# icrdr/3D-UNet-Renal-Anatomy-Extraction

Measured on AMD Instinct MI355X. Metric: train voxels/sec (128^3 patch, bs=2 per GPU), whole job, higher is better.
Workload: dtype bf16; 1 GPU; ResUnet3D(num_pool=4, num_features=32, in=1, out=3) train step (fwd+HybirdLoss+bwd+Adam), 2x1x128^3 per GPU, dropout on; global_batch=2, parallelism=dp1, optimizer=optim.Adam (fused multi-tensor)

## Files before the change

3d-unet-renal-anatomy-extraction_amd/_native.py:

```python
import ctypes
import os
import threading

import torch

_HERE = os.path.dirname(os.path.abspath(__file__))
LIB_PATH = os.environ.get("RU3D_LIB", os.path.join(_HERE, "libru3d.so"))

F32, BF16, F16 = 0, 1, 2
PREDICT_MAX_BATCH = 16
LABEL_I64, LABEL_U8 = 0, 1
ROLE_CONV_FWD, ROLE_CONV_DGRAD, ROLE_CONVT_FWD, ROLE_CONVT_DGRAD, ROLE_BIAS = 0, 1, 2, 3, 4
LOSS_HYBIRD, LOSS_DICELOSS, LOSS_FOCAL, LOSS_DICE = 0, 1, 2, 3
MAX_CLASSES = 8


class Tensor(ctypes.Structure):
    _fields_ = [("ptr", ctypes.c_void_p), ("n", ctypes.c_int32), ("d", ctypes.c_int32), ("h", ctypes.c_int32),
                ("w", ctypes.c_int32), ("c", ctypes.c_int32), ("ld", ctypes.c_int32), ("cseg", ctypes.c_int32),
                ("seg_stride", ctypes.c_int64)]


class PackItem(ctypes.Structure):
    _fields_ = [("src", ctypes.c_void_p), ("dst", ctypes.c_void_p), ("cout", ctypes.c_int32), ("cin", ctypes.c_int32),
                ("k", ctypes.c_int32), ("stride", ctypes.c_int32), ("role", ctypes.c_int32),
                ("cout_seg", ctypes.c_int32), ("cin_seg", ctypes.c_int32)]


class PatchParams(ctypes.Structure):
    _fields_ = [("lo", ctypes.c_int32 * 3), ("before", ctypes.c_int32 * 3), ("patch", ctypes.c_int32 * 3),
                ("flip", ctypes.c_int32 * 3), ("image_cval", ctypes.c_float), ("label_cval", ctypes.c_int32),
                ("do_contrast", ctypes.c_int32), ("do_brightness", ctypes.c_int32), ("do_gamma", ctypes.c_int32),
                ("contrast", ctypes.c_float), ("brightness", ctypes.c_float), ("gamma", ctypes.c_float),
                ("gamma_eps", ctypes.c_float)]


class SpatialParams(ctypes.Structure):
    _fields_ = [("centre", ctypes.c_double * 3), ("matrix", ctypes.c_double * 9), ("lattice", ctypes.c_int32 * 3),
                ("spacing", ctypes.c_int32 * 3)]


class DegradeParams(ctypes.Structure):
    _fields_ = [("do_noise", ctypes.c_int32), ("do_blur", ctypes.c_int32), ("do_low_res", ctypes.c_int32),
                ("noise_key", ctypes.c_uint32 * 2), ("reserved", ctypes.c_int32), ("noise_variance", ctypes.c_double),
                ("blur_sigma", ctypes.c_double), ("low_res_zoom", ctypes.c_double)]


class MorphRow(ctypes.Structure):
    _fields_ = [("dx", ctypes.c_int8), ("dy", ctypes.c_int8), ("zmask", ctypes.c_uint16)]


class RenderTile(ctypes.Structure):
    _fields_ = [("volume", ctypes.c_void_p), ("table", ctypes.c_void_p), ("overlay", ctypes.c_void_p * 2),
                ("overlay_table", ctypes.c_void_p * 2), ("vmin", ctypes.c_double), ("vmax", ctypes.c_double),
                ("origin", ctypes.c_double * 2), ("step", ctypes.c_double * 2), ("x0", ctypes.c_int32),
                ("y0", ctypes.c_int32), ("w", ctypes.c_int32), ("h", ctypes.c_int32), ("X", ctypes.c_int32),
                ("Y", ctypes.c_int32), ("Z", ctypes.c_int32), ("C", ctypes.c_int32), ("channel", ctypes.c_int32),
                ("kind", ctypes.c_int32), ("axis", ctypes.c_int32), ("index", ctypes.c_int32),
                ("overlay_mode", ctypes.c_int32 * 2)]


class RenderView(ctypes.Structure):
    _fields_ = [("o", ctypes.c_double * 3), ("du", ctypes.c_double * 3), ("dv", ctypes.c_double * 3),
                ("dw", ctypes.c_double * 3), ("spacing", ctypes.c_double * 3), ("light", ctypes.c_double * 3),
                ("ambient", ctypes.c_double), ("diffuse", ctypes.c_double), ("background", ctypes.c_double * 3),
                ("num_steps", ctypes.c_int32), ("reserved", ctypes.c_int32)]


class DsLevel(ctypes.Structure):
    _fields_ = [("logits", ctypes.c_void_p), ("stride_n", ctypes.c_int64), ("stride_c", ctypes.c_int64),
                ("stride_v", ctypes.c_int64), ("d", ctypes.c_int32), ("h", ctypes.c_int32), ("w", ctypes.c_int32),
                ("shift", ctypes.c_int32)]


DS_MAX_LEVELS = 8
MASK_NE, MASK_EQ, MASK_GT, MASK_GE = 0, 1, 2, 3
TILE_F32, TILE_U8 = 0, 1
OVERLAY_FILL, OVERLAY_OUTLINE = 0, 1
RENDER_MAX_TILES = 256
MORPH_ERODE, MORPH_DILATE = 0, 1
MORPH_MAX_EXTENT, MORPH_MAX_ROWS = 15, 225
CONFUSION_MAX_CLASSES = 32
ORDER_STATS_MAX_RANKS = 8
EDT_MAX_AXIS = 4096
SPATIAL_MAX_YZ = 2560
BOUNDARY_MAX_AXIS = 2048
DEGRADE_MAX_RADIUS = 16
PACK_MAX = 40
_P = ctypes.POINTER(Tensor)
_vp, _i, _i64, _f, _sz, _u64 = (ctypes.c_void_p, ctypes.c_int, ctypes.c_int64, ctypes.c_float, ctypes.c_size_t,
                                ctypes.c_uint64)
_dbl = ctypes.c_double

_LOSS_VIEW = [_vp, _i64, _i64, _i64, _vp, _i, _i]

SIGNATURES = {
    "ru3d_version": (_i, []),
    "ru3d_last_error": (ctypes.c_char_p, []),
    "ru3d_launch_log_begin": (None, []),
    "ru3d_launch_log_end": (ctypes.c_char_p, []),
    "ru3d_packed_weight_bytes": (_sz, [_i, _i, _i, _i, _i, _i]),
    "ru3d_pack_weight": (_i, [_vp, _vp, _i, _i, _i, _i, _i, _i, _vp]),
    "ru3d_pack_weights": (_i, [ctypes.POINTER(PackItem), _i, _i, _vp]),
    "ru3d_unpad_weight_grad": (_i, [_vp, _vp, _i, _i, _i, _i, _i, _vp]),
    "ru3d_conv3d_workspace_bytes": (_sz, [_P, _P, _i, _i, _i]),
    "ru3d_conv3d_fwd": (_i, [_P, _vp, _vp, _P, _P, _i, _i, _i, _i, _vp, _sz, _vp]),
    "ru3d_conv3d_fwd_in_workspace_bytes": (_sz, [_P, _P, _i, _i, _i]),
    "ru3d_conv3d_fwd_in": (_i, [_P, _vp, _vp, _P, _i, _i, _i, _vp, _vp, _vp, _vp, _sz, _f, _vp]),
    "ru3d_conv3d_fwd_in_lrelu_workspace_bytes": (_sz, [_P, _P, _i, _i, _i]),
    "ru3d_conv3d_fwd_in_lrelu": (_i, [_P, _vp, _vp, _P, _i, _i, _i, _vp, _vp, _vp, _P, _P, _f, _vp, _sz, _f, _vp]),
    "ru3d_planar_concat_supported": (_i, [_i, _i, _i, _i, _i, _i, _i]),
    "ru3d_conv3d_dgrad": (_i, [_P, _vp, _P, _P, _i, _i, _i, _vp, _sz, _vp]),
    "ru3d_conv3d_s2_pair_fwd_in_supported": (_i, [_P, _P, _P, _i]),
    "ru3d_conv3d_s2_pair_fwd_in_workspace_bytes": (_sz, [_P, _P, _i]),
    "ru3d_conv3d_s2_pair_fwd_in": (_i, [_P, _vp, _vp, _P, _vp, _vp, _P, _vp, _vp, _vp, _vp, _sz, _f, _i, _vp]),
    "ru3d_conv3d_s1_dgrad_pair_supported": (_i, [_P, _P, _P, _i]),
    "ru3d_conv3d_s1_dgrad_pair": (_i, [_P, _vp, _P, _vp, _P, _i, _vp]),
    "ru3d_conv3d_s2_dgrad_pair_supported": (_i, [_P, _P, _P, _P, _i]),
    "ru3d_conv3d_s2_dgrad_pair": (_i, [_P, _vp, _P, _vp, _P, _P, _i, _vp]),
    "ru3d_conv3d_wgrad_workspace_bytes": (_sz, [_P, _P, _i, _i, _i]),
    "ru3d_conv3d_wgrad": (_i, [_P, _P, _vp, _vp, _sz, _i, _i, _i, _vp]),
    "ru3d_conv3d_wgrad_bias_workspace_bytes": (_sz, [_P, _P, _i, _i, _i]),
    "ru3d_conv3d_wgrad_bias": (_i, [_P, _P, _vp, _vp, _vp, _sz, _i, _i, _i, _vp]),
    "ru3d_conv3d_wgrad_pair_supported": (_i, [_P, _P, _P, _i, _i]),
    "ru3d_conv3d_wgrad_pair_workspace_bytes": (_sz, [_P, _P, _P, _i, _i]),
    "ru3d_conv3d_wgrad_pair": (_i, [_P, _P, _P, _vp, _vp, _vp, _sz, _i, _i, _vp]),
    "ru3d_head_bwd_supported": (_i, [_P, _P, _P, _i]),
    "ru3d_head_bwd_workspace_bytes": (_sz, [_P, _i]),
    "ru3d_head_bwd": (_i, [_P, _P, _vp, _i, _P, _vp, _vp, _vp, _sz, _i, _vp]),
    "ru3d_convtranspose3d_k3s2p1_fwd": (_i, [_P, _vp, _vp, _P, _i, _vp]),
    "ru3d_convtranspose3d_k3s2p1_fwd_in_workspace_bytes": (_sz, [_P, _P, _i]),
    "ru3d_convtranspose3d_k3s2p1_fwd_in": (_i, [_P, _vp, _vp, _P, _vp, _vp, _vp, _sz, _f, _i, _vp]),
    "ru3d_convtranspose3d_k3s2p1_dgrad": (_i, [_P, _vp, _P, _i, _vp]),
    "ru3d_convtranspose3d_k3s2p1_wgrad_workspace_bytes": (_sz, [_P, _P, _i]),
    "ru3d_convtranspose3d_k3s2p1_wgrad": (_i, [_P, _P, _vp, _vp, _sz, _i, _vp]),
    "ru3d_reduce_workspace_bytes": (_sz, [_P]),
    "ru3d_instnorm_stats": (_i, [_P, _vp, _vp, _vp, _vp, _sz, _f, _i, _vp]),
    "ru3d_in_lrelu_fwd": (_i, [_P, _vp, _vp, _P, _P, _f, _i, _vp]),
    "ru3d_skip1x1_in_lrelu_fwd_supported": (_i, [_P, _P, _P, _i]),
    "ru3d_skip1x1_in_lrelu_fwd": (_i, [_P, _vp, _vp, _P, _vp, _vp, _P, _f, _i, _vp]),
    "ru3d_skip1x1_in_lrelu_head_fwd_supported": (_i, [_P, _P, _P, _P, _i]),
    "ru3d_skip1x1_in_lrelu_head_fwd": (_i, [_P, _vp, _vp, _P, _vp, _vp, _P, _vp, _vp, _P, _f, _i, _vp]),
    "ru3d_head_in_bwd_supported": (_i, [_P, _P, _P, _P, _P, _i]),
    "ru3d_head_in_bwd_workspace_bytes": (_sz, [_P, _i]),
    "ru3d_head_in_bwd": (_i, [_P, _P, _vp, _i, _P, _vp, _vp, _P, _P, _vp, _vp, _vp, _vp, _sz, _f, _i, _vp]),
    "ru3d_in_lrelu_bwd": (_i, [_P, _P, _P, _vp, _vp, _P, _P, _vp, _sz, _f, _i, _vp, _vp, _i, _vp]),
    "ru3d_in_lrelu_bwd_apply": (_i, [_P, _P, _vp, _vp, _vp, _P, _f, _i, _i, _vp]),
    "ru3d_conv3d_dgrad_in_bwd_workspace_bytes": (_sz, [_P, _P, _i, _i, _i]),
    "ru3d_conv3d_dgrad_in_bwd": (_i, [_P, _vp, _P, _vp, _vp, _P, _P, _i, _i, _f, _i, _vp, _sz, _vp]),
    "ru3d_channel_sum": (_i, [_P, _vp, _vp, _sz, _i, _vp]),
    "ru3d_batchnorm_stats_pool": (_i, [_P, _vp, _vp, _vp, _sz, _i, _vp]),
    "ru3d_batchnorm_stats_finalize": (_i, [_vp, _i, _i, _i, _dbl, _vp, _vp, _vp, _f, _f, _vp, _vp, _vp, _vp, _vp, _vp, _vp]),
    "ru3d_affine_lrelu_fwd": (_i, [_P, _vp, _vp, _P, _P, _f, _i, _vp]),
    "ru3d_batchnorm_bwd_pool": (_i, [_P, _P, _P, _vp, _vp, _P, _vp, _vp, _sz, _f, _i, _vp]),
    "ru3d_batchnorm_bwd_apply": (_i, [_P, _P, _vp, _vp, _vp, _vp, _dbl, _P, _vp, _sz, _i, _i, _vp]),
    "ru3d_dropout3d_scale": (_i, [_vp, _i, _f, _u64, _u64, _vp]),
    "ru3d_dropout3d_scale_dev": (_i, [_vp, _i, _f, _u64, _u64, _vp, _vp]),
    "ru3d_pointwise": (_i, [_i, _P, _P, _P, _P, _P, _f, _i, _vp]),
    "ru3d_copy_channels": (_i, [_P, _P, _i, _vp]),
    "ru3d_add": (_i, [_P, _P, _P, _i, _vp]),
    "ru3d_cast_f32": (_i, [_P, _P, _i, _vp]),
    "ru3d_ncdhw_to_ndhwc": (_i, [_vp, _P, _i, _vp]),
    "ru3d_ndhwc_to_ncdhw": (_i, [_P, _vp, _i, _vp]),
    "ru3d_loss_state_bytes": (_sz, [_i]),
    "ru3d_loss_state_bad_labels_offset": (_sz, []),
    "ru3d_loss_workspace_bytes": (_sz, [_i, _i64, _i]),
    "ru3d_loss_fwd": (_i, _LOSS_VIEW + [_i64, _i, _i, _f, _vp, _f, _f, _f, _vp, _vp, _vp, _sz, _vp]),
    "ru3d_loss_bwd": (_i, _LOSS_VIEW + [_i64, _i, _f, _vp, _vp, _vp, _i, _vp]),
    "ru3d_tversky": (_i, [_vp, _vp, _i64, _f, _f, _f, _vp, _vp, _sz, _vp]),
    "ru3d_predict_accumulate": (_i, [_P, _i, _i, _vp, _vp, _i, _i, _i, _i, _i, _i, _vp]),
    "ru3d_predict_merge": (_i, [_vp, _vp, _i, _i, _i, _i, _i, _i, _i, _i, _i, _i, _i, _vp, _vp]),
    "ru3d_predict_gather": (_i, [_vp, _i, _i, _i, _i, _vp, _i, _P, _vp]),
    "ru3d_predict_accumulate_weighted": (_i, [_P, _i, _i, _i, _vp, _vp, _vp, _vp, _vp, _i, _i, _i, _i, _i, _i, _vp]),
    "ru3d_group_loss_state_bytes": (_sz, []),
    "ru3d_group_loss_workspace_bytes": (_sz, [_i, _i64, _i]),
    "ru3d_group_loss_fwd": (_i, _LOSS_VIEW + [_i64, _i, _vp, _i, _i, _i, _i, _f, _vp, _f, _f, _f, _vp, _vp, _vp, _sz,
                                              _vp]),
    "ru3d_group_loss_bwd": (_i, _LOSS_VIEW + [_i64, _i, _vp, _i, _i, _i, _f, _vp, _vp, _vp, _i, _vp]),
    "ru3d_topk_select_workspace_bytes": (_sz, [_i64]),
    "ru3d_topk_select_trip_elements": (_i64, []),
    "ru3d_topk_select": (_i, [_vp, _i64, _i64, _vp, _vp, _sz, _vp]),
    "ru3d_topk_loss_state_bytes": (_sz, []),
    "ru3d_topk_loss_workspace_bytes": (_sz, [_i, _i64, _i]),
    "ru3d_topk_loss_fwd": (_i, _LOSS_VIEW + [_i64, _i, _i64, _i, _vp, _f, _f, _f, _f, _vp, _vp, _vp, _vp, _sz, _vp]),
    "ru3d_topk_loss_fwd_launches": (_i, []),
    "ru3d_topk_loss_fwd_timed": (_i, _LOSS_VIEW + [_i64, _i, _i64, _i, _vp, _f, _f, _f, _f, _vp, _vp, _vp, _vp, _sz,
                                                   _vp, _vp]),
    "ru3d_topk_loss_bwd": (_i, _LOSS_VIEW + [_i64, _i, _i, _vp, _vp, _vp, _vp, _i, _vp]),
    "ru3d_predict_accumulate_groups": (_i, [_P, _i, _i, _i, _vp, _vp, _vp, _vp, _vp, _i, _i, _i, _i, _i, _i, _vp]),
    "ru3d_predict_merge_groups": (_i, [_vp, _vp, _i, _i, _i, _i, _vp, _vp, _i, _i, _i, _i, _i, _i, _vp, _vp]),
    "ru3d_components_workspace_bytes": (_sz, [_i, _i, _i]),
    "ru3d_label_components": (_i, [_vp, _i, _i, _i, _vp, _vp, _vp, _sz, _vp]),
    "ru3d_component_stats": (_i, [_vp, _i, _i, _i, _i, _vp, _vp, _vp]),
    "ru3d_filter_components_workspace_bytes": (_sz, [_i]),
    "ru3d_filter_components": (_i, [_vp, _i, _i, _i, _i, _vp, _i, _vp, _vp, _vp, _vp, _sz, _vp]),
    "ru3d_region_accumulate": (_i, [_vp, _i, _i, _i, _i, _i, _i, _i, _vp, _vp, _i, _i, _i, _vp]),
    "ru3d_cascade_merge": (_i, [_vp, _vp, _i, _i, _i, _i, _vp, _vp]),
    "ru3d_mask_bytes": (_sz, [_i, _i, _i]),
    "ru3d_mask_pack": (_i, [_vp, _i, _i, _i, _i, _i, _vp, _vp]),
    "ru3d_mask_unpack": (_i, [_vp, _i, _i, _i, _i, _i, _vp, _vp]),
    "ru3d_binary_morph": (_i, [_vp, _vp, _i, _i, _i, _i, ctypes.POINTER(MorphRow), _i, _i, _vp]),
    "ru3d_confusion_counts": (_i, [_vp, _vp, _i64, _i, _vp, _vp]),
    "ru3d_threshold_bbox": (_i, [_vp, _i, _i, _i, _i, _f, _vp, _vp, _vp]),
    "ru3d_masked_sample_workspace_bytes": (_sz, [_i, _i, _i]),
    "ru3d_masked_sample": (_i, [_vp, _i, _i, _i, _i, _i, _vp, _i, _i, _vp, _i64, _vp, _vp, _sz, _vp]),
    "ru3d_order_stats_workspace_bytes": (_sz, []),
    "ru3d_order_stats": (_i, [_vp, _i64, ctypes.POINTER(ctypes.c_int64), _i, _vp, _vp, _sz, _vp]),
    "ru3d_moments_workspace_bytes": (_sz, []),
    "ru3d_moments": (_i, [_vp, _i64, _vp, _vp, _sz, _vp]),
    "ru3d_edt_workspace_bytes": (_sz, [_i, _i, _i]),
    "ru3d_edt_squared": (_i, [_vp, _i, _i, _i, ctypes.POINTER(_dbl), _vp, _vp, _sz, _vp]),
    "ru3d_mask_surface": (_i, [_vp, _vp, _i, _i, _i, _vp]),
    "ru3d_edt_gather_workspace_bytes": (_sz, [_i, _i, _i]),
    "ru3d_edt_gather": (_i, [_vp, _vp, _i, _i, _i, _vp, _i64, _vp, _vp, _sz, _vp]),
    "ru3d_edt_reduce_workspace_bytes": (_sz, [_i64]),
    "ru3d_edt_reduce": (_i, [_vp, _vp, _i64, _dbl, _vp, _vp, _sz, _vp]),
    "ru3d_skeleton_workspace_bytes": (_sz, [_i, _i, _i]),
    "ru3d_skeleton_thin": (_i, [_vp, _i, _i, _i, _i, _vp, _sz, _vp]),
    "ru3d_skeleton_classify": (_i, [_vp, _i, _i, _i, _vp, _vp, _vp, _vp]),
    "ru3d_skeleton_length": (_i, [_vp, _i, _i, _i, ctypes.POINTER(_dbl), _vp, _vp, _sz, _vp]),
    "ru3d_skeleton_overlap": (_i, [_vp, _vp, _i, _i, _i, _vp, _vp]),
    "ru3d_skeleton_radius_stats": (_i, [_vp, _i64, _vp, _vp]),
    "ru3d_cldice_workspace_bytes": (_sz, [_i, _i, _i, _i, _i]),
    "ru3d_cldice_state_bytes": (_sz, []),
    "ru3d_soft_skeleton_fwd": (_i, [_vp, _i, _i, _i, _i, _i, _vp, _vp, _vp, _vp, _vp, _sz, _vp]),
    "ru3d_soft_skeleton_bwd": (_i, [_vp, _i, _i, _i, _i, _i, _vp, _vp, _vp, _vp, _vp, _vp, _sz, _vp]),
    "ru3d_cldice_fwd": (_i, _LOSS_VIEW + [_i, _i, _i, _i, _vp, _i, _i, _vp, _f, _vp, _vp, _vp, _vp, _vp, _vp, _vp, _vp,
                                          _sz, _vp]),
    "ru3d_cldice_bwd": (_i, _LOSS_VIEW + [_i, _i, _i, _i, _vp, _i, _i, _vp, _vp, _vp, _vp, _vp, _vp, _vp, _f, _i, _vp,
                                          _vp, _sz, _vp]),
    "ru3d_boundary_workspace_bytes": (_sz, [_i, _i, _i, _i]),
    "ru3d_boundary_state_bytes": (_sz, []),
    "ru3d_signed_distance": (_i, [_vp, _i, _i, _i, _i, _i, _i, _vp, _i, _vp, _vp, _vp, _sz, _vp]),
    "ru3d_boundary_fwd": (_i, _LOSS_VIEW + [_i, _i, _i, _i, _vp, _i, _vp, _vp, _vp, _vp, _vp, _sz, _vp]),
    "ru3d_boundary_bwd": (_i, [_vp, _i64, _i64, _i64, _i, _i, _i, _i, _i, _vp, _i, _vp, _vp, _vp, _f, _i, _vp, _vp]),
    "ru3d_ds_state_bytes": (_sz, []),
    "ru3d_ds_state_bad_labels_offset": (_sz, []),
    "ru3d_ds_block_bytes": (_sz, []),
    "ru3d_ds_loss_workspace_bytes": (_sz, [ctypes.POINTER(DsLevel), _i, _i]),
    "ru3d_ds_loss_fwd": (_i, [ctypes.POINTER(DsLevel), _i, _vp, _i, _i, _i, _i, _i, _i, _i, _f, _vp, _f, _f, _f, _vp, _vp,
                              _vp, _vp, _sz, _vp]),
    "ru3d_ds_loss_bwd": (_i, [ctypes.POINTER(DsLevel), ctypes.POINTER(_vp), _i, _vp, _i, _i, _i, _i, _i, _i, _f, _vp, _vp,
                              _vp]),
    "ru3d_mesh_workspace_bytes": (_sz, [_i, _i, _i]),
    "ru3d_mesh_count": (_i, [_vp, _i, _i, _i, _vp, _vp, _sz, _vp]),
    "ru3d_mesh_emit": (_i, [_vp, _i, _i, _i, _vp, _vp, _i64, _vp, _i64, _vp, _vp, _sz, _vp]),
    "ru3d_mesh_smooth": (_i, [_vp, _vp, _vp, _i64, _dbl, _vp]),
    "ru3d_mesh_measure_workspace_bytes": (_sz, [_i64]),
    "ru3d_mesh_measure": (_i, [_vp, _i64, _vp, _i64, _vp, _vp, _sz, _vp]),
    "ru3d_render_tiles": (_i, [_vp, _i, _vp, _i, _i, _vp]),
    "ru3d_render_surface_workspace_bytes": (_sz, [_i, _i, _i]),
    "ru3d_render_surface_prepare": (_i, [_vp, _i, _i, _i, _vp, _vp, _sz, _vp]),
    "ru3d_render_surface": (_i, [_vp, _i, _i, _i, _vp, ctypes.POINTER(RenderView), _vp, _vp, _i, _i, _vp, _sz, _vp]),
    "ru3d_adam_multi": (_i, [_vp, _vp, _i, _i, _f, _f, _f, _f, _f, _f, _f, _vp]),
    "ru3d_adam_multi_dev": (_i, [_vp, _vp, _i, _i, _vp, _vp]),
    "ru3d_adam_multi_amp": (_i, [_vp, _vp, _i, _i, _vp, _vp, _vp]),
    "ru3d_amp_update": (_i, [_vp, _f, _f, _i, _f, _f, _vp]),
    "ru3d_grad_sumsq": (_i, [_vp, _vp, _i, _i, _vp, _vp]),
    "ru3d_grad_norm_finish": (_i, [_vp, _i, _f, _vp, _f, _vp, _vp]),
    "ru3d_grad_norm": (_i, [_vp, _vp, _i, _i, _vp, _f, _f, _vp, _vp]),
    "ru3d_grad_scale_dev": (_i, [_vp, _vp, _i, _i, _vp, _vp]),
    "ru3d_sgd_multi": (_i, [_vp, _vp, _i, _i, _f, _f, _f, _i, _f, _vp, _vp]),
    "ru3d_sgd_multi_dev": (_i, [_vp, _vp, _i, _i, _vp, _vp, _vp]),
    "ru3d_adamw_multi": (_i, [_vp, _vp, _i, _i, _f, _f, _f, _f, _f, _f, _f, _f, _vp, _vp]),
    "ru3d_adamw_multi_dev": (_i, [_vp, _vp, _i, _i, _vp, _vp, _vp]),
    "ru3d_adam_multi_clip": (_i, [_vp, _vp, _i, _i, _f, _f, _f, _f, _f, _f, _f, _vp, _vp]),
    "ru3d_adam_multi_clip_dev": (_i, [_vp, _vp, _i, _i, _vp, _vp, _vp]),
    "ru3d_adam_step": (_i, [_vp, _vp, _vp, _vp, _i64, _f, _f, _f, _f, _f, _f, _f, _vp]),
    "ru3d_augment_workspace_bytes": (_sz, [_i, _i, _i]),
    "ru3d_augment_label_presence": (_i, [_vp, _i, _i, _i, _i, ctypes.POINTER(ctypes.c_int32),
                                        ctypes.POINTER(ctypes.c_int32), _i, _vp, _vp]),
    "ru3d_augment_patch": (_i, [_vp, _vp, _i, _i, _i, _i, _i, ctypes.POINTER(PatchParams), _vp, _vp, _vp, _vp, _sz,
                               _vp]),
    "ru3d_augment_patch_spatial": (_i, [_vp, _vp, _i, _i, _i, _i, _i, ctypes.POINTER(PatchParams),
                                       ctypes.POINTER(SpatialParams), _vp, _vp, _vp, _vp, _vp, _sz, _vp]),
    "ru3d_augment_degrade_workspace_bytes": (_sz, [_i, _i, _i, _i]),
    "ru3d_augment_degrade": (_i, [_vp, _i, _i, _i, _i, ctypes.POINTER(DegradeParams), _vp, _sz, _vp, _vp]),
    "ru3d_augment_intensity": (_i, [_vp, _i64, _vp, _i, ctypes.POINTER(PatchParams), _vp]),
    "ru3d_grad_scale_check": (_i, [_vp, _vp, _i, _i, _f, _vp, _vp]),
    "ru3d_comm_unique_id": (_i, [_vp]),
    "ru3d_comm_init": (_i, [ctypes.POINTER(_vp), _vp, _i, _i, _i]),
    "ru3d_comm_allreduce": (_i, [_vp, _vp, _i64, _i, _i, _vp]),
    "ru3d_comm_reduce_scatter": (_i, [_vp, _vp, _i64, _i, _i, _vp]),
    "ru3d_comm_all_gather": (_i, [_vp, _vp, _i64, _i, _vp]),
    "ru3d_comm_available": (_i, []),
    "ru3d_comm_destroy": (_i, [_vp]),
    "ru3d_probe_begin": (_i, [_i, _i, _i, _i, _i, _i]),
    "ru3d_probe_end": (_i, [ctypes.POINTER(ctypes.c_int), ctypes.POINTER(ctypes.c_double)]),
# ... 172 lines not shown
```

3d-unet-renal-anatomy-extraction_amd/_ops.py:

```python
import ctypes
import os
import threading
import weakref

import torch

import _native as N
from _native import check, desc, ptr, ref, stream

LRELU_SLOPE = 0.01
IN_EPS = 1e-5


def pack_weight(w, role, dtype, stride=1):
    N.require_device(w, "weight")
    w = w.detach()
    if w.dtype != torch.float32 or not w.is_contiguous():
        w = w.float().contiguous()
    k = w.shape[2]
    if role in (N.ROLE_CONVT_FWD, N.ROLE_CONVT_DGRAD):
        cin, cout = w.shape[0], w.shape[1]
    else:
        cout, cin = w.shape[0], w.shape[1]
    code = N.dtype_code(dtype)
# ... 164 lines not shown
    return b if (b.dtype == torch.float32 and b.is_contiguous()) else b.float().contiguous()


def _conv_out(size, k, s):
    return (size + 2 * (k // 2) - k) // s + 1


class Probe:

    def __init__(self, n, cin, cout, extent):
        self.key = (int(n),) + tuple(int(e) for e in extent) + (int(cin), int(cout))
        self.count = 0
        self.total_ms = 0.0
        self.active = False

    def start(self):
        check(N.lib.ru3d_probe_begin(*self.key), "probe_begin")
        self.active = True

    def stop(self):
        if not self.active:
            return
        n = ctypes.c_int(0)
        ms = ctypes.c_double(0.0)
        check(N.lib.ru3d_probe_end(ctypes.byref(n), ctypes.byref(ms)), "probe_end")
        self.count += n.value
        self.total_ms += ms.value
        self.active = False

    def result(self):
        self.stop()
        return self.count, (self.total_ms / self.count if self.count else 0.0)


def set_probe(p):
    cur = _PROBE[0]
    if cur is not None and cur is not p:
        cur.stop()
    _PROBE[0] = p
    if p is not None:
        p.start()


_PROBE = [None]


class launch_log:

    def __init__(self):
        self.names = []

    def __enter__(self):
        N.lib.ru3d_launch_log_begin()
        return self

    def __exit__(self, *exc):
        s = N.lib.ru3d_launch_log_end().decode("utf-8", "replace")
        self.names = s.split(";") if s else []
        return False


def _conv_ws(dsrc, ddst, k, stride, dtype, device):
    if k != 3 or stride != 1 or dtype == torch.float32:
        return None, 0
    need = N.lib.ru3d_conv3d_workspace_bytes(ref(dsrc), ref(ddst), k, stride, N.dtype_code(dtype))
    if need == 0:
        return None, 0
    buf = N.workspace(need, device)
    return ptr(buf), buf.numel()


def conv_fwd(x, pw, bias, cout, k, stride, res=None, out_dtype=None):
    n, _, d, h, w = x.shape
    out_dtype = out_dtype or x.dtype
    y = N.new_act(n, cout, _conv_out(d, k, stride), _conv_out(h, k, stride), _conv_out(w, k, stride), out_dtype,
                  x.device)
    b = _bias(bias)
    dx, dyy = desc(x), desc(y)
    dr = desc(res) if res is not None else None
    ws, wsn = _conv_ws(dx, dyy, k, stride, x.dtype, x.device)
    check(N.lib.ru3d_conv3d_fwd(ref(dx), ptr(pw), ptr(b), ref(dr), ref(dyy), k, stride, N.dtype_code(x.dtype),
                                N.dtype_code(out_dtype), ws, wsn, stream()), "conv3d_fwd")
    return y


def conv_fwd_in(x, pw, bias, cout, k, stride, drop_scale=None):
    n, _, d, h, w = x.shape
    y = N.new_act(n, cout, _conv_out(d, k, stride), _conv_out(h, k, stride), _conv_out(w, k, stride), x.dtype, x.device)
    mean = torch.empty(n * cout, dtype=torch.float32, device=x.device)
    scale = torch.empty(n * cout, dtype=torch.float32, device=x.device)
    b = _bias(bias)
    dx, dyy = desc(x), desc(y)
    code = N.dtype_code(x.dtype)
    ws = N.workspace(N.lib.ru3d_conv3d_fwd_in_workspace_bytes(ref(dx), ref(dyy), k, stride, code), x.device)
    check(N.lib.ru3d_conv3d_fwd_in(ref(dx), ptr(pw), ptr(b), ref(dyy), k, stride, code, ptr(drop_scale), ptr(mean),
                                   ptr(scale), ptr(ws), ws.numel(), IN_EPS, stream()), "conv3d_fwd_in")
    return y, mean, scale


def conv_fwd_in_act(x, pw, bias, cout, k, stride, drop_scale=None, res=None, out=None):
    n, _, d, h, w = x.shape
    od, oh, ow = _conv_out(d, k, stride), _conv_out(h, k, stride), _conv_out(w, k, stride)
    y = N.new_act(n, cout, od, oh, ow, x.dtype, x.device)
    if out is None:
        out = N.new_act(n, cout, od, oh, ow, x.dtype, x.device)
    mean = torch.empty(n * cout, dtype=torch.float32, device=x.device)
    scale = torch.empty(n * cout, dtype=torch.float32, device=x.device)
    b = _bias(bias)
    dx, dyy, do = desc(x), desc(y), desc(out)
    dr = desc(res) if res is not None else None
    code = N.dtype_code(x.dtype)
    ws = N.workspace(N.lib.ru3d_conv3d_fwd_in_lrelu_workspace_bytes(ref(dx), ref(dyy), k, stride, code), x.device)
    check(N.lib.ru3d_conv3d_fwd_in_lrelu(ref(dx), ptr(pw), ptr(b), ref(dyy), k, stride, code, ptr(drop_scale), ptr(mean),
                                         ptr(scale), ref(dr), ref(do), LRELU_SLOPE, ptr(ws), ws.numel(), IN_EPS, stream()),
          "conv3d_fwd_in_lrelu")
    return y, mean, scale, out


def conv_dgrad(dy, pw, in_shape, k, stride, res=None):
    n, cin, d, h, w = in_shape
    dx = N.new_act(n, cin, d, h, w, dy.dtype, dy.device)
    ddy, ddx = desc(dy), desc(dx)
    dr = desc(res) if res is not None else None
    ws, wsn = _conv_ws(ddy, ddx, k, stride, dy.dtype, dy.device)
    check(N.lib.ru3d_conv3d_dgrad(ref(ddy), ptr(pw), ref(dr), ref(ddx), k, stride, N.dtype_code(dy.dtype), ws, wsn,
                                  stream()), "conv3d_dgrad")
    return dx


def conv_dgrad_in_bwd(dy, pw, act, mean, scale, k=3, stride=1):
    n, c, d, h, w = act.shape
    da = N.new_act(n, c, d, h, w, dy.dtype, dy.device)
    dyn = N.new_act(n, c, d, h, w, dy.dtype, dy.device)
    ddy, dact, dda, ddyn = desc(dy), desc(act), desc(da), desc(dyn)
    code = N.dtype_code(dy.dtype)
    need = N.lib.ru3d_conv3d_dgrad_in_bwd_workspace_bytes(ref(ddy), ref(dda), k, stride, code)
    ws = N.workspace(need, dy.device)
    check(N.lib.ru3d_conv3d_dgrad_in_bwd(ref(ddy), ptr(pw), ref(dact), ptr(mean), ptr(scale), ref(dda), ref(ddyn), k,
                                         stride, LRELU_SLOPE, code, ptr(ws), ws.numel(), stream()),
          "conv3d_dgrad_in_bwd")
    return dyn


GRAD_ARENA = {}


def _grad_out(key, shape, device):
    t = GRAD_ARENA.get(key) if key is not None else None
    if t is not None and tuple(t.shape) == tuple(shape) and t.device == device:
        return t.view(t.shape)
    return torch.empty(shape, dtype=torch.float32, device=device)


def conv_wgrad(x, dy, k, stride, key=None):
    cout, cin = dy.shape[1], x.shape[1]
    dw = _grad_out(key, (cout, cin, k, k, k), x.device)
    dx, ddy = desc(x), desc(dy)
    code = N.dtype_code(x.dtype)
    nbytes = N.lib.ru3d_conv3d_wgrad_workspace_bytes(ref(dx), ref(ddy), k, stride, code)
    ws = N.workspace(nbytes, x.device)
    check(N.lib.ru3d_conv3d_wgrad(ref(dx), ref(ddy), ptr(dw), ptr(ws), ws.numel(), k, stride, code, stream()),
          "conv3d_wgrad")
    return dw


def _wgrad_pair_ok(x, dy, stride=1):
    if x.dtype == torch.float32:
        return False
    dx, ddy = desc(x), desc(dy)
    return bool(N.lib.ru3d_conv3d_wgrad_pair_supported(ref(dx), ref(ddy), ref(ddy), stride, N.dtype_code(x.dtype)))


def conv_wgrad_pair(x, dy, dy2, stride=1, key=None, key2=None):
    if x.dtype == torch.float32 or tuple(dy.shape) != tuple(dy2.shape):
        return None
    dx, ddy, ddy2 = desc(x), desc(dy), desc(dy2)
    code = N.dtype_code(x.dtype)
    if not N.lib.ru3d_conv3d_wgrad_pair_supported(ref(dx), ref(ddy), ref(ddy2), stride, code):
        return None
    cout, cin = dy.shape[1], x.shape[1]
    dw = _grad_out(key, (cout, cin, 3, 3, 3), x.device)
    dw2 = _grad_out(key2, (cout, cin, 1, 1, 1), x.device)
    ws = N.workspace(N.lib.ru3d_conv3d_wgrad_pair_workspace_bytes(ref(dx), ref(ddy), ref(ddy2), stride, code), x.device)
    check(N.lib.ru3d_conv3d_wgrad_pair(ref(dx), ref(ddy), ref(ddy2), ptr(dw), ptr(dw2), ptr(ws), ws.numel(), stride, code,
                                       stream()), "conv3d_wgrad_pair")
    return dw, dw2


def conv_wgrad_bias(x, dy, k, stride, key=None):
    cout, cin = dy.shape[1], x.shape[1]
    dw = _grad_out(key, (cout, cin, k, k, k), x.device)
    db = torch.empty(cout, dtype=torch.float32, device=x.device)
    dx, ddy = desc(x), desc(dy)
    code = N.dtype_code(x.dtype)
    ws = N.workspace(N.lib.ru3d_conv3d_wgrad_bias_workspace_bytes(ref(dx), ref(ddy), k, stride, code), x.device)
    check(N.lib.ru3d_conv3d_wgrad_bias(ref(dx), ref(ddy), ptr(dw), ptr(db), ptr(ws), ws.numel(), k, stride, code, stream()),
          "conv3d_wgrad_bias")
    return dw, db


def head_bwd(x, gy, weight, want_bias, key=None):
    if gy.dtype != torch.float32 or x.dtype == torch.float32 or not N.is_ndhwc(gy) or weight.dtype != torch.float32:
        return None
    n, c, d, h, w = x.shape
    dx = N.new_act(n, c, d, h, w, x.dtype, x.device)
    ddx, dg, dxx = desc(x), desc(gy), desc(dx)
    code = N.dtype_code(x.dtype)
    if not N.lib.ru3d_head_bwd_supported(ref(ddx), ref(dg), ref(dxx), code):
        return None
    cout, cin = weight.shape[0], weight.shape[1]
    dw = _grad_out(key, (cout, cin, 1, 1, 1), x.device)
    db = torch.empty(cout, dtype=torch.float32, device=x.device) if want_bias else None
    ws = N.workspace(N.lib.ru3d_head_bwd_workspace_bytes(ref(ddx), code), x.device)
    wd = weight.detach()
    check(N.lib.ru3d_head_bwd(ref(ddx), ref(dg), ptr(wd if wd.is_contiguous() else wd.contiguous()), cin, ref(dxx), ptr(dw),
                              ptr(db), ptr(ws), ws.numel(), code, stream()), "head_bwd")
    return dx, dw, db


def convt_fwd(x, pw, bias, cout):
    n, _, d, h, w = x.shape
    y = N.new_act(n, cout, 2 * d, 2 * h, 2 * w, x.dtype, x.device)
    b = _bias(bias)
    dx, dyy = desc(x), desc(y)
    check(N.lib.ru3d_convtranspose3d_k3s2p1_fwd(ref(dx), ptr(pw), ptr(b), ref(dyy), N.dtype_code(x.dtype), stream()),
          "convtranspose3d_fwd")
    return y


def convt_fwd_in(x, pw, bias, cout):
    n, _, d, h, w = x.shape
    y = N.new_act(n, cout, 2 * d, 2 * h, 2 * w, x.dtype, x.device)
    mean = torch.empty(n * cout, dtype=torch.float32, device=x.device)
    scale = torch.empty(n * cout, dtype=torch.float32, device=x.device)
    b = _bias(bias)
    dx, dyy = desc(x), desc(y)
    code = N.dtype_code(x.dtype)
    ws = N.workspace(N.lib.ru3d_convtranspose3d_k3s2p1_fwd_in_workspace_bytes(ref(dx), ref(dyy), code), x.device)
    check(N.lib.ru3d_convtranspose3d_k3s2p1_fwd_in(ref(dx), ptr(pw), ptr(b), ref(dyy), ptr(mean), ptr(scale), ptr(ws),
                                                   ws.numel(), IN_EPS, code, stream()), "convtranspose3d_fwd_in")
    return y, mean, scale


def conv_s2_pair_fwd_in(x, pw3, b3, pw1, b1, cout, drop_scale=None):
    code = N.dtype_code(x.dtype)
    if code == N.F32:
        return None
    n, _, d, h, w = x.shape
    od, oh, ow = _conv_out(d, 3, 2), _conv_out(h, 3, 2), _conv_out(w, 3, 2)
    y3 = N.new_act(n, cout, od, oh, ow, x.dtype, x.device)
    y1 = N.new_act(n, cout, od, oh, ow, x.dtype, x.device)
    dx, d3, d1 = desc(x), desc(y3), desc(y1)
    if not N.lib.ru3d_conv3d_s2_pair_fwd_in_supported(ref(dx), ref(d3), ref(d1), code):
        return None
    mean = torch.empty(n * cout, dtype=torch.float32, device=x.device)
    scale = torch.empty(n * cout, dtype=torch.float32, device=x.device)
    ws = N.workspace(N.lib.ru3d_conv3d_s2_pair_fwd_in_workspace_bytes(ref(dx), ref(d3), code), x.device)
    check(N.lib.ru3d_conv3d_s2_pair_fwd_in(ref(dx), ptr(pw3), ptr(_bias(b3)), ref(d3), ptr(pw1), ptr(_bias(b1)), ref(d1),
                                           ptr(drop_scale), ptr(mean), ptr(scale), ptr(ws), ws.numel(), IN_EPS, code,
                                           stream()), "conv3d_s2_pair_fwd_in")
    return y3, mean, scale, y1


def conv_s1_dgrad_pair(dy, pw3, dy2, pw1, in_shape, planar=False):
    n, cin, d, h, w = in_shape
    code = N.dtype_code(dy.dtype)
    if code == N.F32:
        return None
    dx = N.new_act(2 * n, cin // 2, d, h, w, dy.dtype, dy.device) if planar else N.new_act(n, cin, d, h, w, dy.dtype, dy.device)
    ddy, ddy2, ddx = desc(dy), desc(dy2), desc(N.Split(dx) if planar else dx)
    if not N.lib.ru3d_conv3d_s1_dgrad_pair_supported(ref(ddy), ref(ddy2), ref(ddx), code):
        return None
    check(N.lib.ru3d_conv3d_s1_dgrad_pair(ref(ddy), ptr(pw3), ref(ddy2), ptr(pw1), ref(ddx), code, stream()),
          "conv3d_s1_dgrad_pair")
    return dx


def conv_s2_dgrad_pair(dy, pw3, dy2, pw1, in_shape, res=None):
    n, cin, d, h, w = in_shape
    code = N.dtype_code(dy.dtype)
    if code == N.F32:
        return None
    dx = N.new_act(n, cin, d, h, w, dy.dtype, dy.device)
    ddy, ddy2, ddx = desc(dy), desc(dy2), desc(dx)
    dr = desc(res) if res is not None else None
    if not N.lib.ru3d_conv3d_s2_dgrad_pair_supported(ref(ddy), ref(ddy2), ref(dr), ref(ddx), code):
        return None
    check(N.lib.ru3d_conv3d_s2_dgrad_pair(ref(ddy), ptr(pw3), ref(ddy2), ptr(pw1), ref(dr), ref(ddx), code, stream()),
          "conv3d_s2_dgrad_pair")
    return dx


def convt_dgrad(dy, pw, in_shape):
    n, cin, d, h, w = in_shape
    dx = N.new_act(n, cin, d, h, w, dy.dtype, dy.device)
    ddy, ddx = desc(dy), desc(dx)
    check(N.lib.ru3d_convtranspose3d_k3s2p1_dgrad(ref(ddy), ptr(pw), ref(ddx), N.dtype_code(dy.dtype), stream()),
          "convtranspose3d_dgrad")
    return dx


def convt_wgrad(x, dy, key=None):
    cin, cout = x.shape[1], dy.shape[1]
    dw = _grad_out(key, (cin, cout, 3, 3, 3), x.device)
    dx, ddy = desc(x), desc(dy)
    code = N.dtype_code(x.dtype)
    nbytes = N.lib.ru3d_convtranspose3d_k3s2p1_wgrad_workspace_bytes(ref(dx), ref(ddy), code)
    ws = N.workspace(nbytes, x.device)
    check(N.lib.ru3d_convtranspose3d_k3s2p1_wgrad(ref(dx), ref(ddy), ptr(dw), ptr(ws), ws.numel(), code, stream()),
          "convtranspose3d_wgrad")
    return dw


def in_stats(y, drop_scale=None):
    n, c = y.shape[0], y.shape[1]
    mean = torch.empty(n * c, dtype=torch.float32, device=y.device)
    scale = torch.empty(n * c, dtype=torch.float32, device=y.device)
    dy = desc(y)
    ws = N.workspace(N.lib.ru3d_reduce_workspace_bytes(ref(dy)), y.device)
    check(N.lib.ru3d_instnorm_stats(ref(dy), ptr(drop_scale), ptr(mean), ptr(scale), ptr(ws), ws.numel(), IN_EPS,
                                    N.dtype_code(y.dtype), stream()), "instnorm_stats")
    return mean, scale


def in_lrelu_fwd(y, mean, scale, res=None, out=None):
    if out is None:
        n, c, d, h, w = y.shape
        out = N.new_act(n, c, d, h, w, y.dtype, y.device)
    dy, do = desc(y), desc(out)
    dr = desc(res) if res is not None else None
    check(N.lib.ru3d_in_lrelu_fwd(ref(dy), ptr(mean), ptr(scale), ref(dr), ref(do), LRELU_SLOPE,
                                  N.dtype_code(y.dtype), stream()), "in_lrelu_fwd")
    return out


def skip1x1_in_lrelu_fwd(x, pw, bias, y, mean, scale, out=None):
    code = N.dtype_code(y.dtype)
    if code == N.F32:
        return None
    if out is None:
        n, c, d, h, w = y.shape
        out = N.new_act(n, c, d, h, w, y.dtype, y.device)
    dx, dy, do = desc(x), desc(y), desc(out)
    if not N.lib.ru3d_skip1x1_in_lrelu_fwd_supported(ref(dx), ref(dy), ref(do), code):
        return None
    check(N.lib.ru3d_skip1x1_in_lrelu_fwd(ref(dx), ptr(pw), ptr(_bias(bias)), ref(dy), ptr(mean), ptr(scale), ref(do),
                                          LRELU_SLOPE, code, stream()), "skip1x1_in_lrelu_fwd")
    return out


def head_tail_mode():
    return os.environ.get("RU3D_HEAD_TAIL", "1")


def skip1x1_in_lrelu_head_fwd(x, pw, bias, y, mean, scale, head_pw, head_bias, head_cout):
    code = N.dtype_code(y.dtype)
    if code == N.F32 or head_cout > 4:
        return None
    n, c, d, h, w = y.shape
    out = N.new_act(n, c, d, h, w, y.dtype, y.device)
    logits = N.new_act(n, head_cout, d, h, w, torch.float32, y.device)
    dx, dy, do, dl = desc(x), desc(y), desc(out), desc(logits)
    if not N.lib.ru3d_skip1x1_in_lrelu_head_fwd_supported(ref(dx), ref(dy), ref(do), ref(dl), code):
        return None
    check(N.lib.ru3d_skip1x1_in_lrelu_head_fwd(ref(dx), ptr(pw), ptr(_bias(bias)), ref(dy), ptr(mean), ptr(scale), ref(do),
                                               ptr(head_pw), ptr(_bias(head_bias)), ref(dl), LRELU_SLOPE, code, stream()),
          "skip1x1_in_lrelu_head_fwd")
    return out, logits


def head_in_bwd(z, gy, weight, want_bias, y, mean, scale, key=None):
    if gy.dtype != torch.float32 or z.dtype == torch.float32 or not N.is_ndhwc(gy) or weight.dtype != torch.float32:
        return None
    n, c, d, h, w = z.shape
    dy = N.new_act(n, c, d, h, w, z.dtype, z.device)
    gpre = N.new_act(n, c, d, h, w, z.dtype, z.device)
    dz, dg, dyy, dp, ddy = desc(z), desc(gy), desc(y), desc(gpre), desc(dy)
    code = N.dtype_code(z.dtype)
    if not N.lib.ru3d_head_in_bwd_supported(ref(dz), ref(dg), ref(dyy), ref(dp), ref(ddy), code):
        return None
    cout, cin = weight.shape[0], weight.shape[1]
    dw = _grad_out(key, (cout, cin, 1, 1, 1), z.device)
    db = torch.empty(cout, dtype=torch.float32, device=z.device) if want_bias else None
    gsum = torch.empty(c, dtype=torch.float32, device=z.device)
    ws = N.workspace(N.lib.ru3d_head_in_bwd_workspace_bytes(ref(dz), code), z.device)
    wd = weight.detach()
    check(N.lib.ru3d_head_in_bwd(ref(dz), ref(dg), ptr(wd if wd.is_contiguous() else wd.contiguous()), cin, ref(dyy),
                                 ptr(mean), ptr(scale), ref(dp), ref(ddy), ptr(dw), ptr(db), ptr(gsum), ptr(ws), ws.numel(),
                                 LRELU_SLOPE, code, stream()), "head_in_bwd")
    return dy, gpre, gsum, dw, db


def in_lrelu_bwd(gout, out, y, mean, scale, want_gpre=False, zero_far=False, want_gpre_sum=False, dy_sum=None):
    n, c, d, h, w = y.shape
    dy = N.new_act(n, c, d, h, w, y.dtype, y.device)
    gpre = N.new_act(n, c, d, h, w, y.dtype, y.device) if want_gpre else None
    dg, do, dyy, ddy = desc(gout), desc(out), desc(y), desc(dy)
    dp = desc(gpre) if want_gpre else None
    ws = N.workspace(N.lib.ru3d_reduce_workspace_bytes(ref(dyy)), y.device)
    gsum = torch.empty(c, dtype=torch.float32, device=y.device) if (want_gpre and want_gpre_sum) else None
    check(N.lib.ru3d_in_lrelu_bwd(ref(dg), ref(do), ref(dyy), ptr(mean), ptr(scale), ref(ddy), ref(dp), ptr(ws),
                                  ws.numel(), LRELU_SLOPE, 1 if zero_far else 0, ptr(gsum), ptr(dy_sum),
                                  N.dtype_code(y.dtype), stream()), "in_lrelu_bwd")
    if want_gpre_sum:
        return dy, gpre, gsum
    return dy, gpre


_BN_SYNC = [None, 1]


def set_bn_sync(group=None, enable=True):
    import torch.distributed as dist
    if enable and dist.is_available() and dist.is_initialized() and dist.get_world_size(group) > 1:
        _BN_SYNC[0], _BN_SYNC[1] = (group if group is not None else dist.group.WORLD), dist.get_world_size(group)
    else:
        _BN_SYNC[0], _BN_SYNC[1] = None, 1


def _bn_allreduce(pooled):
    if _BN_SYNC[0] is not None:
        import torch.distributed as dist
        dist.all_reduce(pooled, group=_BN_SYNC[0])
    return pooled


def bn_train_stats(y, drop_scale, norm, c_real):
    n, c = y.shape[0], y.shape[1]
    dev = y.device
    dy = desc(y)
    pooled = torch.empty(2 * c, dtype=torch.float64, device=dev)
    ws = N.workspace(N.lib.ru3d_reduce_workspace_bytes(ref(dy)), dev)
    check(N.lib.ru3d_batchnorm_stats_pool(ref(dy), ptr(drop_scale), ptr(pooled), ptr(ws), ws.numel(),
                                          N.dtype_code(y.dtype), stream()), "batchnorm_stats_pool")
    _bn_allreduce(pooled)
    count = float(n * y.shape[2] * y.shape[3] * y.shape[4]) * _BN_SYNC[1]
    track = norm.track_running_stats and norm.running_mean is not None
    momentum = 0.0
    if track:
        norm.num_batches_tracked.add_(1)
        momentum = (1.0 / float(norm.num_batches_tracked)) if norm.momentum is None else float(norm.momentum)
    out = torch.empty(4, n * c, dtype=torch.float32, device=dev)
    gamma = norm.weight.detach() if norm.weight is not None else None
    beta = norm.bias.detach() if norm.bias is not None else None
    for t in (gamma, beta, norm.running_mean if track else None, norm.running_var if track else None):
        if t is not None and (t.dtype != torch.float32 or not t.is_contiguous() or t.device != dev):
            raise N.Ru3dError("BatchNorm3d: parameters / running statistics must be contiguous fp32 on %s" % dev)
    check(N.lib.ru3d_batchnorm_stats_finalize(ptr(pooled), n, c, c_real, count, ptr(drop_scale), ptr(gamma), ptr(beta),
                                              float(norm.eps), momentum, ptr(norm.running_mean if track else None),
                                              ptr(norm.running_var if track else None), ptr(out[0]), ptr(out[1]),
                                              ptr(out[2]), ptr(out[3]), stream()), "batchnorm_stats_finalize")
    return out[0], out[1], out[2], out[3], count


def affine_lrelu_fwd(y, scale, shift, res=None, out=None):
    if out is None:
        n, c, d, h, w = y.shape
        out = N.new_act(n, c, d, h, w, y.dtype, y.device)
    dy, do = desc(y), desc(out)
    dr = desc(res) if res is not None else None
# ... 120 lines not shown
    else:
        check(N.lib.ru3d_dropout3d_scale(ptr(out), n * c, float(p), ctypes.c_uint64(seed), ctypes.c_uint64(offset),
                                         stream()), "dropout3d_scale")
    return out


_DROP_POOL = []


def prefill_dropout(specs, device):
    _DROP_POOL.clear()
    if len(specs) < 2 or any(sp[2] != specs[0][2] for sp in specs):
        return
    flat = dropout_scale(1, sum(n * c for n, c, _ in specs), specs[0][2], device)
    off = 0
    for n, c, p in specs:
        _DROP_POOL.append((flat[off:off + n * c], n, c, p))
        off += n * c


def take_dropout(n, c, p):
    if not _DROP_POOL:
        return None
    t, n0, c0, p0 = _DROP_POOL[0]
    if (n0, c0, p0) != (n, c, p):
        _DROP_POOL.clear()
        return None
    _DROP_POOL.pop(0)
    return t


def as_input(x, dtype):
    N.require_device(x, "input")
    if x.dim() != 5:
        raise N.Ru3dError("ru3d: expected a 5-D [N,C,D,H,W] tensor, got %s" % (tuple(x.shape),))
    if x.dtype == dtype and N.is_ndhwc(x):
        return x
    if N.is_ndhwc(x) and x.dtype == torch.float32:
        return cast_f32(x, dtype)
    if x.is_contiguous() or x.dtype != torch.float32:
        return ncdhw_to_ndhwc(x, dtype)
    return ncdhw_to_ndhwc(x.contiguous(), dtype)


def as_grad(g, like_dtype):
    if g.dtype != like_dtype:
        if g.dtype == torch.float32 and N.is_ndhwc(g):
            return cast_f32(g, like_dtype)
        g = g.to(like_dtype)
    return N.to_ndhwc(g)


_SIDE_MODE = os.environ.get("RU3D_WGRAD_STREAM", "0")
_SIDE_MAXVOX = int(os.environ.get("RU3D_SIDE_MAXVOX", "65536"))
_SIDE = {}
_SIDE_BUSY = {}


def _side_stream(device):
    s = _SIDE.get(device)
    if s is None:
        s = _SIDE[device] = torch.cuda.Stream(device=device)
    return s


class _OnSide:

    def __init__(self, device, nvox=0, keep=()):
        self.device = device
        self.ctx = None
        self.on = _SIDE_MODE == "1" or (_SIDE_MODE == "auto" and 0 < nvox <= _SIDE_MAXVOX)
        self.keep = keep

    def __enter__(self):
        if self.on:
            side = _side_stream(self.device)
            side.wait_stream(torch.cuda.current_stream(self.device))
            _SIDE_BUSY.setdefault(self.device, []).extend(t for t in self.keep if t is not None)
            self.ctx = torch.cuda.stream(side)
            self.ctx.__enter__()
        return self

    def __exit__(self, *exc):
        if self.ctx is not None:
            self.ctx.__exit__(*exc)
            self.ctx = None
        return False


def _join(device, *outs):
    busy = _SIDE_BUSY.get(device)
    if busy is None:
        return
    cur = torch.cuda.current_stream(device)
    cur.wait_stream(_side_stream(device))
    for t in outs:
        if t is not None:
            t.record_stream(cur)
    del _SIDE_BUSY[device]


class SkipLink:

    def __init__(self, up_channels, dec_channels=0):
        self.up_channels = up_channels
        self.dec_channels = dec_channels
        self.buf = None
        self.grad = None
        self.planar = False

    def skip_view(self, n, c, d, h, w, dtype, device):
        self.planar = False
        self.buf = N.new_act(n, self.up_channels + c, d, h, w, dtype, device)
        return self.buf[:, self.up_channels:]

    def planar_view(self, n, c, d, h, w, dtype, device):
        if (c != self.up_channels or dtype == torch.float32 or not self.dec_channels
                or not N.lib.ru3d_planar_concat_supported(n, d, h, w, c, self.dec_channels, N.dtype_code(dtype))):
            return None
        self.planar = True
        self.buf = N.new_act(2 * n, c, d, h, w, dtype, device)
        return self.buf[n:]


def _f32_view(pack, count):
    return pack[:4 * count].view(torch.float32)


class ConvFn(torch.autograd.Function):

    @staticmethod
    def forward(ctx, x, weight, bias, stride, storage_dtype, out_dtype, pad_in=False, pad_out=False):
        xin = as_input(x, storage_dtype)
        k = weight.shape[2]
        cout, cin = weight.shape[0], weight.shape[1]
        cin_seg = seg_of(cin, xin.shape[1]) if pad_in else 0
        cout_seg = cout if pad_out else 0
        if not pad_in and xin.shape[1] != cin:
            raise N.Ru3dError("conv: input has %d channels, weight expects %d" % (xin.shape[1], cin))
        cout_p = padded_dim(cout, cout_seg)
        specs = [(weight, N.ROLE_CONV_FWD, stride, cout_seg, cin_seg)]
        if ctx.needs_input_grad[0]:
            specs.append((weight, N.ROLE_CONV_DGRAD, stride, cout_seg, cin_seg))
        if cout_seg and bias is not None:
            specs.append((bias, N.ROLE_BIAS, 1, cout_seg, 0))
        packs = pack_weights(specs, storage_dtype)
        b = _f32_view(packs[-1], cout_p) if (cout_seg and bias is not None) else bias
        y = conv_fwd(xin, packs[0], b, cout_p, k, stride, out_dtype=out_dtype)
        ctx.save_for_backward(xin, packs[1] if ctx.needs_input_grad[0] else None)
        ctx.dims = (cout, cin, cout_seg, cin_seg)
        ctx.stride, ctx.k, ctx.has_bias = stride, k, bias is not None
        ctx.storage_dtype = storage_dtype
        ctx.in_dtype = x.dtype
        ctx.wkey = weight.data_ptr() if not (cout_seg or cin_seg) else None
        ctx.weight_ref = weight if (k == 1 and cout <= 4) else None
        return y

    @staticmethod
    def backward(ctx, gy):
        xin, pwd = ctx.saved_tensors
        sd = ctx.storage_dtype
        cout, cin, cout_seg, cin_seg = ctx.dims
        if (ctx.k == 1 and ctx.stride == 1 and cout <= 4 and not cout_seg and all(ctx.needs_input_grad[:2])
                and ctx.weight_ref is not None):
            fused = head_bwd(xin, gy, ctx.weight_ref, ctx.has_bias and ctx.needs_input_grad[2],
                             key=None if cin_seg else ctx.wkey)
            if fused is not None:
                gx, gw, gb = fused
                if gx.dtype != ctx.in_dtype:
                    gx = gx.to(ctx.in_dtype)
                return gx, gw, gb, None, None, None, None, None
        gy = as_grad(gy, sd)
        gx = gw = gb = None
        with _OnSide(gy.device):
            if ctx.needs_input_grad[1] and ctx.has_bias and ctx.needs_input_grad[2] and not (cout_seg or cin_seg) \
                    and sd != torch.float32:
                gw, gb = conv_wgrad_bias(xin, gy, ctx.k, ctx.stride, key=ctx.wkey)
            elif ctx.needs_input_grad[1]:
                gw = unpad_wgrad(conv_wgrad(xin, gy, ctx.k, ctx.stride, key=ctx.wkey), cout, cin, cout_seg, cin_seg)
            if gb is None and ctx.has_bias and ctx.needs_input_grad[2]:
                gb = channel_sum(gy)[:cout]
        if ctx.needs_input_grad[0]:
            gx = conv_dgrad(gy, pwd, tuple(xin.shape), ctx.k, ctx.stride)
            if gx.dtype != ctx.in_dtype:
                gx = gx.to(ctx.in_dtype)
        _join(gy.device, gw, gb)
        return gx, gw, gb, None, None, None, None, None


class ResBlockFn(torch.autograd.Function):

    @staticmethod
    def forward(ctx, x, w1, b1, w2, b2, ws, bs, stride, drop_scale, pad=0, checkpoint=False, in_link=None,
                out_link=None, planar=False, head_w=None, head_b=None):
        sd = x.dtype
        x = N.to_ndhwc(x)
        xt = x
        if planar:
            x = N.Split(x)
        cout, cin = w1.shape[0], w1.shape[1]
        cin_seg = seg_of(cin, x.shape[1], int(pad)) if pad else 0
        cout_seg = cout if pad else 0
        if not pad and x.shape[1] != cin:
            raise N.Ru3dError("ResBlock: input has %d channels, conv1 expects %d" % (x.shape[1], cin))
        cout_p = padded_dim(cout, cout_seg)
        train = any(ctx.needs_input_grad)
        need_gx = ctx.needs_input_grad[0]
        specs = [(w1, N.ROLE_CONV_FWD, stride, cout_seg, cin_seg), (w2, N.ROLE_CONV_FWD, 1, cout_seg, cout_seg)]
        if ws is not None:
            specs.append((ws, N.ROLE_CONV_FWD, stride, cout_seg, cin_seg))
        nfwd = len(specs)
        if train:
            specs.append((w2, N.ROLE_CONV_DGRAD, 1, cout_seg, cout_seg))
            if need_gx:
                specs.append((w1, N.ROLE_CONV_DGRAD, stride, cout_seg, cin_seg))
                if ws is not None:
                    specs.append((ws, N.ROLE_CONV_DGRAD, stride, cout_seg, cin_seg))
        nw = len(specs)
        if cout_seg:
            specs += [(b, N.ROLE_BIAS, 1, cout_seg, 0) for b in (b1, b2, bs) if b is not None]
        packs = pack_weights(specs, sd)
        if cout_seg:
            it = iter(packs[nw:])
            b1, b2, bs = [(_f32_view(next(it), cout_p) if b is not None else None) for b in (b1, b2, bs)]
        pw1, pw2 = packs[0], packs[1]
        fused = conv_s2_pair_fwd_in(x, pw1, b1, packs[2], bs, cout_p, drop_scale) if (ws is not None and stride == 2) else None
        if fused is not None:
            y1, mean1, scale1, skip = fused
            a1 = in_lrelu_fwd(y1, mean1, scale1)
        else:
            y1, mean1, scale1, a1 = conv_fwd_in_act(x, pw1, b1, cout_p, 3, stride, drop_scale)
        n_, _, d_, h_, w_ = a1.shape
        zout = None
        if out_link is not None and cout_p * a1.element_size() >= 128:
            zout = out_link.skip_view(n_, cout_p, d_, h_, w_, sd, x.device)
        elif out_link is not None:
            zout = out_link.planar_view(n_, cout_p, d_, h_, w_, sd, x.device)
        z = None
        tail = (fused is None and ws is not None and stride == 1 and out_link is None and sd != torch.float32
                and (x.shape[1], cout_p) in ((64, 32), (128, 64)) and n_ * d_ * h_ * w_ >= 65536)
        logits = head_pack = None
        if head_w is not None:
            if head_w.shape[1] != cout or head_w.shape[2] != 1 or out_link is not None:
                raise N.Ru3dError("ResBlock: the head must be a 1x1x1 conv on the block's %d output channels" % cout)
            head_pack = pack_weights([(head_w, N.ROLE_CONV_FWD, 1, 0, cout_seg)], sd)[0]
        if tail:
            y2, mean2, scale2 = conv_fwd_in(a1, pw2, b2, cout_p, 3, 1)
            both = (skip1x1_in_lrelu_head_fwd(x, packs[2], bs, y2, mean2, scale2, head_pack, head_b, head_w.shape[0])
                    if (head_w is not None and head_tail_mode() != "bwd") else None)
            if both is not None:
                z, logits = both
            else:
                z = skip1x1_in_lrelu_fwd(x, packs[2], bs, y2, mean2, scale2)
            if z is None:
                z = in_lrelu_fwd(y2, mean2, scale2, res=conv_fwd(x, packs[2], bs, cout_p, 1, stride), out=zout)
        else:
            if fused is not None:
                pass
            elif ws is not None:
                skip = conv_fwd(x, packs[2], bs, cout_p, 1, stride)
            else:
                skip = x
            y2, mean2, scale2, z = conv_fwd_in_act(a1, pw2, b2, cout_p, 3, 1, res=skip, out=zout)
        if head_w is not None and logits is None:
            logits = conv_fwd(z, head_pack, head_b, head_w.shape[0], 1, 1, out_dtype=torch.float32)
        bwd = packs[nfwd:nw] + [None] * 3
        hsave = head_w if train else None
        if checkpoint and train:
            ctx.save_for_backward(xt, None, None, None, z, mean1, scale1, mean2, scale2, bwd[0], bwd[1], bwd[2],
                                  pw1, pw2, b1, b2, hsave)
        else:
            ctx.save_for_backward(xt, y1, a1, y2, z, mean1, scale1, mean2, scale2, bwd[0], bwd[1], bwd[2],
                                  None, None, None, None, hsave)
        ctx.head = head_w is not None
        ctx.head_bias = head_b is not None
        ctx.hkey = head_w.data_ptr() if (head_w is not None and not cout_seg) else None
        ctx.planar = bool(planar)
        ctx.dims = (cout, cin, cout_seg, cin_seg)
        ctx.stride = stride
        plain = not (cout_seg or cin_seg)
        ctx.wkeys = (w1.data_ptr() if plain else None, w2.data_ptr() if plain else None,
                     ws.data_ptr() if (plain and ws is not None) else None)
        ctx.has_skip_conv = ws is not None
        ctx.in_link = in_link if (in_link is not None and ws is not None) else None
        if in_link is not None:
            in_link.fused_grad = ctx.in_link is not None and need_gx
        return logits if head_w is not None else z

    @staticmethod
    def _head_backward(ctx, gy, z, head_w, y2, mean2, scale2):
        cout, cin, cout_seg, cin_seg = ctx.dims
        sd = z.dtype
        want_b = ctx.head_bias and ctx.needs_input_grad[15]
        fused = head_in_bwd(z, gy, head_w, want_b, y2, mean2, scale2, key=ctx.hkey) if head_tail_mode() != "fwd" else None
        if fused is not None:
            return fused
        hb = head_bwd(z, gy, head_w, want_b, key=ctx.hkey)
        if hb is not None:
            gz, ghw, ghb = hb
        else:
            gy = as_grad(gy, sd)
            hcout = head_w.shape[0]
            ghw = unpad_wgrad(conv_wgrad(z, gy, 1, 1, key=ctx.hkey), hcout, cout, 0, cout_seg)
            ghb = channel_sum(gy)[:hcout] if want_b else None
            pwd = pack_weights([(head_w, N.ROLE_CONV_DGRAD, 1, 0, cout_seg)], sd)[0]
            gz = conv_dgrad(gy, pwd, tuple(z.shape), 1, 1)
        dy2, gpre, gbs_sum = in_lrelu_bwd(gz, z, y2, mean2, scale2, want_gpre=True, want_gpre_sum=True)
        return dy2, gpre, gbs_sum, ghw, ghb

    @staticmethod
    def backward(ctx, gz):
        (x, y1, a1, y2, z, mean1, scale1, mean2, scale2, pw2d, pw1d, pwsd, pw1, pw2, b1, b2, head_w) = ctx.saved_tensors
        cout, cin, cout_seg, cin_seg = ctx.dims
        cout_p = padded_dim(cout, cout_seg)
        sd = x.dtype
        dev = x.device
        stride = ctx.stride
        if not ctx.head:
            gz = as_grad(gz, sd)
        if ctx.planar:
            x = N.Split(x)
        if y1 is None:
            y1 = conv_fwd(x, pw1, b1, cout_p, 3, stride)
            a1 = in_lrelu_fwd(y1, mean1, scale1)
            y2 = conv_fwd(a1, pw2, b2, cout_p, 3, 1)
        ghw = ghb = None
        if ctx.head:
            dy2, gpre, gbs_sum, ghw, ghb = ResBlockFn._head_backward(ctx, gz, z, head_w, y2, mean2, scale2)
        else:
            dy2, gpre, gbs_sum = in_lrelu_bwd(gz, z, y2, mean2, scale2, want_gpre=True, want_gpre_sum=True)
        del y2
        return ResBlockFn._backward_tail(ctx, x, a1, y1, dy2, gpre, gbs_sum, mean1, scale1, pw2d, pw1d, pwsd) + (ghw, ghb)

    @staticmethod
    def _backward_tail(ctx, x, a1, y1, dy2, gpre, gbs_sum, mean1, scale1, pw2d, pw1d, pwsd):
        cout, cin, cout_seg, cin_seg = ctx.dims
        dev = x.device
        stride = ctx.stride
        gws = gbs = None
        nvox = dy2.shape[0] * dy2.shape[2] * dy2.shape[3] * dy2.shape[4]
        xk = x.t if ctx.planar else x
        pair_later = ctx.has_skip_conv and _wgrad_pair_ok(x, gpre, stride)
        with _OnSide(dev, nvox, (a1, dy2, xk, gpre)):
            gw2 = unpad_wgrad(conv_wgrad(a1, dy2, 3, 1, key=ctx.wkeys[1]), cout, cout, cout_seg, cout_seg)
            if ctx.has_skip_conv:
                if not pair_later:
                    gws = unpad_wgrad(conv_wgrad(x, gpre, 1, stride, key=ctx.wkeys[2]), cout, cin, cout_seg, cin_seg)
                gbs = gbs_sum[:cout]
        gb2 = None
        dy1 = conv_dgrad_in_bwd(dy2, pw2d, a1, mean1, scale1)
        del dy2, a1, y1
        with _OnSide(dev, nvox, (xk, dy1, gpre)):
            both = conv_wgrad_pair(x, dy1, gpre, stride, key=ctx.wkeys[0], key2=ctx.wkeys[2]) if pair_later else None
            if both is not None:
                gw1 = unpad_wgrad(both[0], cout, cin, cout_seg, cin_seg)
                gws = unpad_wgrad(both[1], cout, cin, cout_seg, cin_seg)
            else:
                gw1 = unpad_wgrad(conv_wgrad(x, dy1, 3, stride, key=ctx.wkeys[0]), cout, cin, cout_seg, cin_seg)
                if pair_later:
                    gws = unpad_wgrad(conv_wgrad(x, gpre, 1, stride, key=ctx.wkeys[2]), cout, cin, cout_seg, cin_seg)
        gb1 = None
        gx = None
        need_gx = ctx.needs_input_grad[0]
        if ctx.has_skip_conv:
            if need_gx:
                parked = None
                if ctx.in_link is not None:
                    parked, ctx.in_link.grad = ctx.in_link.grad, None
                if stride == 2:
                    gx = conv_s2_dgrad_pair(dy1, pw1d, gpre, pwsd, tuple(x.shape), res=parked)
                elif parked is None:
                    gx = conv_s1_dgrad_pair(dy1, pw1d, gpre, pwsd, tuple(x.shape), planar=ctx.planar)
                if gx is None and ctx.planar:
                    raise N.Ru3dError("ResBlock: the split concat input has no fused input-gradient kernel for this shape")
                if gx is None:
                    gx0 = conv_dgrad(gpre, pwsd, tuple(x.shape), 1, stride, res=parked)
                    gx = conv_dgrad(dy1, pw1d, tuple(x.shape), 3, stride, res=gx0)
        elif need_gx:
            gx = conv_dgrad(dy1, pw1d, tuple(x.shape), 3, stride, res=gpre)
        _join(dev, gw1, gw2, gws, gbs)
        return gx, gw1, gb1, gw2, gb2, gws, gbs, None, None, None, None, None, None, None


class UpFn(torch.autograd.Function):

    @staticmethod
    def forward(ctx, x, wt, bt, skip, pad=False, link=None):
        sd = x.dtype
        x = N.to_ndhwc(x)
        cin, cout = wt.shape[0], wt.shape[1]
        cin_seg = seg_of(cin, x.shape[1]) if pad else 0
        cout_seg = cout if pad else 0
        if not pad and x.shape[1] != cin:
            raise N.Ru3dError("ConvTrans3D: input has %d channels, weight expects %d" % (x.shape[1], cin))
        cout_p = padded_dim(cout, cout_seg)
        specs = [(wt, N.ROLE_CONVT_FWD, 2, cout_seg, cin_seg)]
        if ctx.needs_input_grad[0]:
            specs.append((wt, N.ROLE_CONVT_DGRAD, 2, cout_seg, cin_seg))
        if cout_seg and bt is not None:
            specs.append((bt, N.ROLE_BIAS, 1, cout_seg, 0))
        packs = pack_weights(specs, sd)
        btp = _f32_view(packs[-1], cout_p) if (cout_seg and bt is not None) else bt
        y, mean, scale = convt_fwd_in(x, packs[0], btp, cout_p)
        n, _, d, h, w = y.shape
        if skip is not None:
            skip = as_grad(skip, sd)
            cs = skip.shape[1]
            if tuple(skip.shape[2:]) != (d, h, w) or skip.shape[0] != n:
                raise N.Ru3dError("UpConcat: skip %s does not match up-sampled %s" % (tuple(skip.shape), tuple(y.shape)))
            planar = (link is not None and link.planar and link.buf is not None and link.up_channels == cout_p == cs
                      and tuple(link.buf.shape) == (2 * n, cs, d, h, w) and link.buf.dtype == sd
                      and skip.data_ptr() == link.buf[n:].data_ptr())
            in_place = (not planar and link is not None and not link.planar and link.buf is not None
                        and link.up_channels == cout_p
                        and tuple(link.buf.shape) == (n, cout_p + cs, d, h, w) and link.buf.dtype == sd
                        and skip.data_ptr() == link.buf[:, cout_p:].data_ptr())
            if planar:
                buf = link.buf
                in_lrelu_fwd(y, mean, scale, out=buf[:n])
            else:
                buf = link.buf if in_place else N.new_act(n, cout_p + cs, d, h, w, sd, x.device)
                u = buf[:, :cout_p]
                in_lrelu_fwd(y, mean, scale, out=u)
                if not in_place:
                    copy_channels(skip, buf[:, cout_p:])
            if link is not None:
                link.buf = None
                link.planar_out = planar
            out = buf
        else:
            u = in_lrelu_fwd(y, mean, scale)
            out = u
        ctx.save_for_backward(x, y, out, mean, scale, packs[1] if ctx.needs_input_grad[0] else None)
        ctx.dims = (cout, cin, cout_seg, cin_seg)
        ctx.has_skip = skip is not None
        ctx.planar = bool(skip is not None and link is not None and getattr(link, "planar_out", False))
        ctx.wkey = wt.data_ptr() if not (cout_seg or cin_seg) else None
        ctx.link = link if (link is not None and getattr(link, "fused_grad", False)) else None
        return out

    @staticmethod
    def backward(ctx, g):
        x, y, out, mean, scale, pwd = ctx.saved_tensors
        cout, cin, cout_seg, cin_seg = ctx.dims
        cout_p = padded_dim(cout, cout_seg)
        sd = x.dtype
        g = as_grad(g, sd)
        if ctx.planar:
            n = out.shape[0] // 2
            u, gu, gskip = out[:n], g[:n], g[n:]
        else:
            u = out[:, :cout_p] if ctx.has_skip else out
            gu = g[:, :cout_p] if ctx.has_skip else g
            gskip = g[:, cout_p:] if ctx.has_skip else None
        gb = torch.empty(y.shape[1], dtype=torch.float32, device=y.device)
        dy, _ = in_lrelu_bwd(gu, u, y, mean, scale, zero_far=True, dy_sum=gb)
        gb = gb[:cout]
        nvox = x.shape[0] * x.shape[2] * x.shape[3] * x.shape[4]
        with _OnSide(x.device, nvox, (x, dy)):
            gw = unpad_wgrad(convt_wgrad(x, dy, key=ctx.wkey), cin, cout, cin_seg, cout_seg)
        gx = None
        if ctx.needs_input_grad[0]:
            gx = convt_dgrad(dy, pwd, tuple(x.shape))
        _join(x.device, gw, gb)
        if ctx.link is not None and gskip is not None:
            ctx.link.grad, gskip = gskip, None
        return gx, gw, gb, gskip, None, None


class ResBlockBNFn(torch.autograd.Function):

    @staticmethod
    def forward(ctx, x, w1, b1, w2, b2, ws, bs, gamma, beta, stride, drop_scale, pad, norm):
        sd = x.dtype
        x = N.to_ndhwc(x)
        cout, cin = w1.shape[0], w1.shape[1]
        cin_seg = seg_of(cin, x.shape[1], int(pad)) if pad else 0
        cout_seg = cout if pad else 0
        if not pad and x.shape[1] != cin:
            raise N.Ru3dError("ResBlock: input has %d channels, conv1 expects %d" % (x.shape[1], cin))
        cout_p = padded_dim(cout, cout_seg)
        need_gx = ctx.needs_input_grad[0]
        specs = [(w1, N.ROLE_CONV_FWD, stride, cout_seg, cin_seg), (w2, N.ROLE_CONV_FWD, 1, cout_seg, cout_seg)]
        if ws is not None:
            specs.append((ws, N.ROLE_CONV_FWD, stride, cout_seg, cin_seg))
        nfwd = len(specs)
        specs.append((w2, N.ROLE_CONV_DGRAD, 1, cout_seg, cout_seg))
        if need_gx:
            specs.append((w1, N.ROLE_CONV_DGRAD, stride, cout_seg, cin_seg))
            if ws is not None:
                specs.append((ws, N.ROLE_CONV_DGRAD, stride, cout_seg, cin_seg))
        nw = len(specs)
        if cout_seg:
            specs += [(b, N.ROLE_BIAS, 1, cout_seg, 0) for b in (b1, b2, bs) if b is not None]
        packs = pack_weights(specs, sd)
        has_b = (b1 is not None, b2 is not None, bs is not None)
        if cout_seg:
            it = iter(packs[nw:])
            b1, b2, bs = [(_f32_view(next(it), cout_p) if b is not None else None) for b in (b1, b2, bs)]
        y1 = conv_fwd(x, packs[0], b1, cout_p, 3, stride)
        fs1, fh1, a1s, b1s, cnt1 = bn_train_stats(y1, drop_scale, norm, cout)
        a1 = affine_lrelu_fwd(y1, fs1, fh1)
        y2 = conv_fwd(a1, packs[1], b2, cout_p, 3, 1)
        fs2, fh2, a2s, b2s, cnt2 = bn_train_stats(y2, None, norm, cout)
        skip = conv_fwd(x, packs[2], bs, cout_p, 1, stride) if ws is not None else x
        z = affine_lrelu_fwd(y2, fs2, fh2, res=skip)
        bwd = packs[nfwd:nw] + [None] * 3
        ctx.save_for_backward(x, y1, a1, y2, z, fs1, a1s, b1s, fs2, a2s, b2s, bwd[0], bwd[1], bwd[2])
        ctx.dims = (cout, cin, cout_seg, cin_seg)
        ctx.counts = (cnt1, cnt2)
        ctx.stride = stride
        ctx.has_skip_conv = ws is not None
        ctx.has_b = has_b
        return z

    @staticmethod
    def backward(ctx, gz):
        x, y1, a1, y2, z, fs1, a1s, b1s, fs2, a2s, b2s, pw2d, pw1d, pwsd = ctx.saved_tensors
        cout, cin, cout_seg, cin_seg = ctx.dims
        stride = ctx.stride
        gz = as_grad(gz, x.dtype)
        dy2, gpre, dg2, db2 = bn_lrelu_bwd(gz, z, y2, a2s, b2s, fs2, ctx.counts[1])
        gw2 = unpad_wgrad(conv_wgrad(a1, dy2, 3, 1), cout, cout, cout_seg, cout_seg)
        gb2 = channel_sum(dy2)[:cout] if ctx.has_b[1] else None
        gws = gbs = None
        if ctx.has_skip_conv:
            gws = unpad_wgrad(conv_wgrad(x, gpre, 1, stride), cout, cin, cout_seg, cin_seg)
            gbs = db2[:cout].clone() if ctx.has_b[2] else None
        da1 = conv_dgrad(dy2, pw2d, tuple(a1.shape), 3, 1)
        del dy2
        dy1, _, dg1, db1 = bn_lrelu_bwd(da1, a1, y1, a1s, b1s, fs1, ctx.counts[0])
        del da1
        gw1 = unpad_wgrad(conv_wgrad(x, dy1, 3, stride), cout, cin, cout_seg, cin_seg)
        gb1 = channel_sum(dy1)[:cout] if ctx.has_b[0] else None
        gx = None
        if ctx.needs_input_grad[0]:
            if ctx.has_skip_conv:
                gx0 = conv_dgrad(gpre, pwsd, tuple(x.shape), 1, stride)
                gx = conv_dgrad(dy1, pw1d, tuple(x.shape), 3, stride, res=gx0)
            else:
                gx = conv_dgrad(dy1, pw1d, tuple(x.shape), 3, stride, res=gpre)
        ggamma = (dg1 + dg2)[:cout] if ctx.needs_input_grad[7] else None
        gbeta = (db1 + db2)[:cout] if ctx.needs_input_grad[8] else None
        return gx, gw1, gb1, gw2, gb2, gws, gbs, ggamma, gbeta, None, None, None, None


class UpBNFn(torch.autograd.Function):

    @staticmethod
    def forward(ctx, x, wt, bt, gamma, beta, skip, pad, norm):
        sd = x.dtype
        x = N.to_ndhwc(x)
        cin, cout = wt.shape[0], wt.shape[1]
        cin_seg = seg_of(cin, x.shape[1]) if pad else 0
        cout_seg = cout if pad else 0
        if not pad and x.shape[1] != cin:
            raise N.Ru3dError("ConvTrans3D: input has %d channels, weight expects %d" % (x.shape[1], cin))
        cout_p = padded_dim(cout, cout_seg)
        specs = [(wt, N.ROLE_CONVT_FWD, 2, cout_seg, cin_seg)]
        if ctx.needs_input_grad[0]:
            specs.append((wt, N.ROLE_CONVT_DGRAD, 2, cout_seg, cin_seg))
        if cout_seg and bt is not None:
            specs.append((bt, N.ROLE_BIAS, 1, cout_seg, 0))
        packs = pack_weights(specs, sd)
        btp = _f32_view(packs[-1], cout_p) if (cout_seg and bt is not None) else bt
        y = convt_fwd(x, packs[0], btp, cout_p)
        fs, fh, a_s, b_s, cnt = bn_train_stats(y, None, norm, cout)
        n, _, d, h, w = y.shape
        if skip is not None:
            skip = as_grad(skip, sd)
            cs = skip.shape[1]
            if tuple(skip.shape[2:]) != (d, h, w) or skip.shape[0] != n:
                raise N.Ru3dError("UpConcat: skip %s does not match up-sampled %s" % (tuple(skip.shape), tuple(y.shape)))
            out = N.new_act(n, cout_p + cs, d, h, w, sd, x.device)
            affine_lrelu_fwd(y, fs, fh, out=out[:, :cout_p])
            copy_channels(skip, out[:, cout_p:])
        else:
            out = affine_lrelu_fwd(y, fs, fh)
        ctx.save_for_backward(x, y, out, fs, a_s, b_s, packs[1] if ctx.needs_input_grad[0] else None)
        ctx.dims = (cout, cin, cout_seg, cin_seg)
        ctx.count = cnt
        ctx.has_skip = skip is not None
        ctx.has_b = bt is not None
        return out

    @staticmethod
    def backward(ctx, g):
        x, y, out, fs, a_s, b_s, pwd = ctx.saved_tensors
        cout, cin, cout_seg, cin_seg = ctx.dims
        cout_p = padded_dim(cout, cout_seg)
# ... 62 lines not shown
```

3d-unet-renal-anatomy-extraction_amd/csrc/api.hip:

```cpp
#include "common.h"
#include "conv.h"
#include <string>

#ifndef RU3D_STORAGE_F16

static thread_local std::string g_last_error;

int ru3d_fail(int code, const char* fmt, ...) {
    char buf[512];
    va_list ap;
    va_start(ap, fmt);
    vsnprintf(buf, sizeof(buf), fmt, ap);
    va_end(ap);
    g_last_error = buf;
    return code;
}

static thread_local std::string g_launch_log;
static thread_local bool g_launch_log_armed = false;

int ru3d_check_launch(const char* what) {
    if (g_launch_log_armed) {
        if (!g_launch_log.empty()) g_launch_log += ';';
        g_launch_log += what;
    }
    hipError_t e = hipGetLastError();
    if (e != hipSuccess) {
        ru3d_fail((int)e, "%s: %s", what, hipGetErrorString(e));
        return (int)e > 0 ? (int)e : 1;
    }
    return 0;
}

extern "C" int ru3d_version(void) { return RU3D_VERSION; }
extern "C" const char* ru3d_last_error(void) { return g_last_error.c_str(); }
extern "C" void ru3d_launch_log_begin(void) {
    g_launch_log.clear();
    g_launch_log_armed = true;
}
extern "C" const char* ru3d_launch_log_end(void) {
    g_launch_log_armed = false;
    return g_launch_log.c_str();
}
#endif

namespace RU3D_NS {

static bool dtype_ok(int d) { return d == RU3D_F32 || d == RU3D_BF16; }
static int conv_out(int in, int k, int s) { return (in + 2 * (k / 2) - k) / s + 1; }

static void role_channels(int cout, int cin, int role, int* kin, int* kout, int64_t* s_o, int64_t* s_i, int taps) {
    switch (role) {
        case RU3D_ROLE_CONV_FWD:
            *kin = cin; *kout = cout; *s_o = (int64_t)cin * taps; *s_i = taps; break;
        case RU3D_ROLE_CONV_DGRAD:
            *kin = cout; *kout = cin; *s_o = taps; *s_i = (int64_t)cin * taps; break;
        case RU3D_ROLE_CONVT_FWD:
            *kin = cin; *kout = cout; *s_o = taps; *s_i = (int64_t)cout * taps; break;
        default:
            *kin = cout; *kout = cin; *s_o = (int64_t)cout * taps; *s_i = taps; break;
    }
}

static bool role_uses_mfma(int kin, int kout, int k, int stride, int role, int dtype) {
    (void)stride;
    (void)role;
    return mfma_conv_eligible(kin, kout, k, dtype, dtype);
}

extern "C" size_t ru3d_packed_weight_bytes(int cout, int cin, int k, int stride, int role, int dtype) {
    RU3D_FWD_F16(dtype, ru3d_packed_weight_bytes_f16(cout, cin, k, stride, role, dtype));
    if (cout <= 0 || cin <= 0 || (k != 1 && k != 3) || (stride != 1 && stride != 2) || role < 0 || role > 3 ||
        !dtype_ok(dtype))
        return 0;
    const int taps = k * k * k;
    int kin, kout;
    int64_t s_o, s_i;
    role_channels(cout, cin, role, &kin, &kout, &s_o, &s_i, taps);
    if (role_uses_mfma(kin, kout, k, stride, role, dtype)) return mfma_packed_bytes(kin, kout, taps);
    return (size_t)taps * kin * generic_cout_pad(kout) * (dtype == RU3D_F32 ? 4 : 2);
}

extern "C" int ru3d_pack_weight(const float* src, void* dst, int cout, int cin, int k, int stride, int role, int dtype,
                                void* stream) {
    RU3D_FWD_F16(dtype, ru3d_pack_weight_f16(src, dst, cout, cin, k, stride, role, dtype, stream));
    Ru3dDeviceGuard dev_guard(stream);
    RU3D_REQUIRE(src && dst, "pack_weight: null pointer");
    RU3D_REQUIRE(cout > 0 && cin > 0 && (k == 1 || k == 3) && (stride == 1 || stride == 2),
                 "pack_weight: bad shape cout=%d cin=%d k=%d stride=%d", cout, cin, k, stride);
    RU3D_REQUIRE(role >= 0 && role <= 3 && dtype_ok(dtype), "pack_weight: bad role/dtype");
    const int taps = k * k * k;
    int kin, kout;
    int64_t s_o, s_i;
    role_channels(cout, cin, role, &kin, &kout, &s_o, &s_i, taps);
    if (role_uses_mfma(kin, kout, k, stride, role, dtype))
        return pack_mfma_launch(src, dst, kin, kout, taps, s_o, s_i, 0, as_stream(stream));
    return pack_generic_launch(src, dst, kin, kout, taps, s_o, s_i, 0, dtype, as_stream(stream));
}

static int pad32(int c) { return (c + 31) / 32 * 32; }
static int padded_dim(int real, int seg) { return seg > 0 ? (real / seg) * pad32(seg) : real; }

extern "C" int ru3d_pack_weights(const ru3d_pack_item* items, int count, int dtype, void* stream) {
    RU3D_FWD_F16(dtype, ru3d_pack_weights_f16(items, count, dtype, stream));
    Ru3dDeviceGuard dev_guard(stream);
    RU3D_REQUIRE(items && count > 0 && count <= RU3D_PACK_MAX, "pack_weights: count must be 1..%d", RU3D_PACK_MAX);
    RU3D_REQUIRE(dtype_ok(dtype), "pack_weights: bad dtype");
    PackBatch b;
    b.count = count;
    for (int i = 0; i < count; i++) {
        const ru3d_pack_item& it = items[i];
        RU3D_REQUIRE(it.src && it.dst && it.cout > 0 && it.cin > 0 && (it.k == 1 || it.k == 3) &&
                         (it.stride == 1 || it.stride == 2) && it.role >= 0 && it.role <= RU3D_ROLE_BIAS,
                     "pack_weights: bad item %d", i);
        RU3D_REQUIRE(it.cout_seg >= 0 && it.cin_seg >= 0 && (it.cout_seg == 0 || it.cout % it.cout_seg == 0) &&
                         (it.cin_seg == 0 || it.cin % it.cin_seg == 0),
                     "pack_weights: item %d: segments (%d, %d) do not divide (%d, %d)", i, it.cout_seg, it.cin_seg,
                     it.cout, it.cin);
        PackOne& p = b.item[i];
        p.src = it.src;
        p.dst = it.dst;
        if (it.role == RU3D_ROLE_BIAS) {
            p.mfma = 2;
            p.cout = padded_dim(it.cout, it.cout_seg);
            p.cin = 1; p.taps = 1; p.cout_pad = p.cout; p.s_o = 1; p.s_i = 1;
            p.co_real = it.cout_seg; p.co_pad = it.cout_seg ? pad32(it.cout_seg) : 0;
            p.ci_real = 0; p.ci_pad = 0;
            p.total = p.cout;
            continue;
        }
        const int taps = it.k * it.k * it.k;
        int kin, kout;
        int64_t s_o, s_i;
        role_channels(it.cout, it.cin, it.role, &kin, &kout, &s_o, &s_i, taps);
        const bool in_is_cin = (it.role == RU3D_ROLE_CONV_FWD || it.role == RU3D_ROLE_CONVT_FWD);
        const int kin_seg = in_is_cin ? it.cin_seg : it.cout_seg, kout_seg = in_is_cin ? it.cout_seg : it.cin_seg;
        const int kin_p = padded_dim(kin, kin_seg), kout_p = padded_dim(kout, kout_seg);
        p.cin = kin_p; p.cout = kout_p; p.taps = taps; p.s_o = s_o; p.s_i = s_i;
        p.ci_real = kin_seg; p.ci_pad = kin_seg ? pad32(kin_seg) : 0;
        p.co_real = kout_seg; p.co_pad = kout_seg ? pad32(kout_seg) : 0;
        p.mfma = role_uses_mfma(kin_p, kout_p, it.k, it.stride, it.role, dtype) ? 1 : 0;
        p.cout_pad = generic_cout_pad(kout_p);
        p.total = p.mfma ? (int64_t)taps * kin_p * kout_p : (int64_t)taps * kin_p * p.cout_pad;
    }
    PackPairBatch pairs;
    pairs.count = 0;
    if (dtype == RU3D_BF16) {
        for (int i = 0; i < count; i++) {
            PackOne& p = b.item[i];
            const ru3d_pack_item& it = items[i];
            if (p.mfma != 1 || (p.cin % 32) || (p.cout % 32) || (p.taps != 27 && p.taps != 1)) continue;
            const bool is_t = it.role == RU3D_ROLE_CONVT_FWD || it.role == RU3D_ROLE_CONVT_DGRAD;
            const bool a_major = it.role == RU3D_ROLE_CONV_FWD || it.role == RU3D_ROLE_CONVT_DGRAD;
            const int a_seg = is_t ? it.cin_seg : it.cout_seg, b_seg = is_t ? it.cout_seg : it.cin_seg;
            const int a_realdim = is_t ? it.cin : it.cout, b_realdim = is_t ? it.cout : it.cin;
            int slot = -1;
            for (int j = 0; j < pairs.count; j++)
                if (pairs.item[j].src == it.src && pairs.item[j].taps == p.taps &&
                    pairs.item[j].adim == padded_dim(a_realdim, a_seg) && pairs.item[j].bdim == padded_dim(b_realdim, b_seg) &&
                    pairs.item[j].a_real == a_seg && pairs.item[j].b_real == b_seg &&
                    (a_major ? !pairs.item[j].dst_a : !pairs.item[j].dst_b))
                    slot = j;
            if (slot < 0) {
                slot = pairs.count++;
                PackPair& q = pairs.item[slot];
                q.src = it.src; q.dst_a = nullptr; q.dst_b = nullptr;
                q.adim = padded_dim(a_realdim, a_seg); q.bdim = padded_dim(b_realdim, b_seg); q.taps = p.taps;
                q.a_real = a_seg; q.a_pad = a_seg ? pad32(a_seg) : 0;
                q.b_real = b_seg; q.b_pad = b_seg ? pad32(b_seg) : 0;
                q.s_a = (int64_t)b_realdim * p.taps;
            }
            (a_major ? pairs.item[slot].dst_a : pairs.item[slot].dst_b) = p.dst;
            p.mfma = 3;
        }
    }
    bool rest = false;
    for (int i = 0; i < count; i++) rest = rest || b.item[i].mfma != 3;
    if (pairs.count) {
        int rc = pack_pair_launch(pairs, as_stream(stream));
        if (rc || !rest) return rc;
    }
    return pack_batch_launch(b, dtype, as_stream(stream));
}

// ... 469 lines not shown
    RU3D_REQUIRE(x && dy && dy2 && wgrad_pair_ok(x, dy, dy2, stride, dtype),
                 "conv3d_wgrad_pair: shapes have no fused kernel (ask ru3d_conv3d_wgrad_pair_supported first)");
    RU3D_REQUIRE(dw && dw2 && ws, "conv3d_wgrad_pair: null output / workspace");
    WgradGeom g = make_wgrad(x, dy, 3, stride);
    if (stride == 2) {
        RU3D_REQUIRE(ws_bytes >= wgrad_s2_pair_ws_bytes(g), "conv3d_wgrad_pair: workspace too small");
        return wgrad_s2_pair_launch(x->ptr, dy->ptr, dy2->ptr, dy2->ld, dw, dw2, ws, g, as_stream(stream));
    }
    RU3D_REQUIRE(ws_bytes >= wgrad_slide_pair_ws_bytes(g), "conv3d_wgrad_pair: workspace too small");
    return wgrad_slide_pair_launch(x->ptr, dy->ptr, dy2->ptr, dy2->ld, dw, dw2, ws, g, as_stream(stream));
}

extern "C" size_t ru3d_conv3d_wgrad_bias_workspace_bytes(const ru3d_tensor* x, const ru3d_tensor* dy, int k, int stride,
                                                         int dtype) {
    RU3D_FWD_F16(dtype, ru3d_conv3d_wgrad_bias_workspace_bytes_f16(x, dy, k, stride, dtype));
    if (!wgrad_shapes_ok(x, dy, k, stride)) return 0;
    const size_t a = ru3d_conv3d_wgrad_workspace_bytes(x, dy, k, stride, dtype), b = ru3d_reduce_workspace_bytes(dy);
    return a > b ? a : b;
}

extern "C" int ru3d_conv3d_wgrad_bias(const ru3d_tensor* x, const ru3d_tensor* dy, float* dw, float* db, void* ws,
                                      size_t ws_bytes, int k, int stride, int dtype, void* stream) {
    RU3D_FWD_F16(dtype, ru3d_conv3d_wgrad_bias_f16(x, dy, dw, db, ws, ws_bytes, k, stride, dtype, stream));
    Ru3dDeviceGuard dev_guard(stream);
    RU3D_REQUIRE((k == 1 || k == 3) && (stride == 1 || stride == 2), "conv3d_wgrad_bias: k=%d stride=%d unsupported", k, stride);
    RU3D_REQUIRE(wgrad_shapes_ok(x, dy, k, stride) && tensor_ok(x), "conv3d_wgrad_bias: x/dy shape mismatch");
    RU3D_REQUIRE(dw && db && dtype_ok(dtype), "conv3d_wgrad_bias: bad argument");
    RU3D_REQUIRE(ws && ws_bytes >= ru3d_conv3d_wgrad_bias_workspace_bytes(x, dy, k, stride, dtype),
                 "conv3d_wgrad_bias: workspace too small");
    WgradGeom g = make_wgrad(x, dy, k, stride);
    if (stem_wgrad_gives_bias(g, dtype))
        return stem_wgrad_launch(x->ptr, dy->ptr, dw, ws, ws_bytes, g, dtype, as_stream(stream), db);
    int rc = ru3d_conv3d_wgrad(x, dy, dw, ws, ws_bytes, k, stride, dtype, stream);
    if (rc) return rc;
    return ru3d_channel_sum(dy, db, ws, ws_bytes, dtype, stream);
}

extern "C" int ru3d_head_bwd_supported(const ru3d_tensor* x, const ru3d_tensor* dlogits, const ru3d_tensor* dx, int dtype) {
    RU3D_FWD_F16(dtype, ru3d_head_bwd_supported_f16(x, dlogits, dx, dtype));
    if (!tensor_ok(x) || !tensor_ok(dlogits) || !tensor_ok(dx)) return 0;
    if (x->n != dlogits->n || x->d != dlogits->d || x->h != dlogits->h || x->w != dlogits->w) return 0;
    if (dx->n != x->n || dx->d != x->d || dx->h != x->h || dx->w != x->w || dx->c != x->c) return 0;
    if ((x->ld % 8) || (dx->ld % 8) || ((((uintptr_t)x->ptr) | ((uintptr_t)dx->ptr)) % 16) || (((uintptr_t)dlogits->ptr) % 4)) return 0;
    return head_bwd_eligible(x->c, dlogits->c, dtype) ? 1 : 0;
}

extern "C" size_t ru3d_head_bwd_workspace_bytes(const ru3d_tensor* x, int dtype) {
    RU3D_FWD_F16(dtype, ru3d_head_bwd_workspace_bytes_f16(x, dtype));
    return tensor_ok(x) ? head_bwd_ws_bytes(nvox(x), x->c) : 0;
}

extern "C" int ru3d_head_bwd(const ru3d_tensor* x, const ru3d_tensor* dlogits, const float* weight, int cin_real,
                             const ru3d_tensor* dx, float* dw, float* db, void* ws, size_t ws_bytes, int dtype, void* stream) {
    RU3D_FWD_F16(dtype, ru3d_head_bwd_f16(x, dlogits, weight, cin_real, dx, dw, db, ws, ws_bytes, dtype, stream));
    Ru3dDeviceGuard dev_guard(stream);
    RU3D_REQUIRE(ru3d_head_bwd_supported(x, dlogits, dx, dtype), "head_bwd: shapes have no fused kernel (ask ru3d_head_bwd_supported first)");
    RU3D_REQUIRE(weight && dw && ws && cin_real > 0 && cin_real <= x->c, "head_bwd: bad argument");
    RU3D_REQUIRE(ws_bytes >= head_bwd_ws_bytes(nvox(x), x->c), "head_bwd: workspace too small");
    return head_bwd_launch(x->ptr, x->ld, (const float*)dlogits->ptr, dlogits->ld, weight, cin_real, x->c, dlogits->c, dx->ptr,
                           dx->ld, dw, db, ws, nvox(x), as_stream(stream));
}

static bool convt_shapes_ok(const ru3d_tensor* x, const ru3d_tensor* y) {
    return tensor_ok(x) && tensor_ok(y) && x->n == y->n && y->d == 2 * x->d && y->h == 2 * x->h && y->w == 2 * x->w;
}

extern "C" int ru3d_convtranspose3d_k3s2p1_fwd(const ru3d_tensor* x, const void* w_packed, const float* bias,
                                               const ru3d_tensor* y, int dtype, void* stream) {
    RU3D_FWD_F16(dtype, ru3d_convtranspose3d_k3s2p1_fwd_f16(x, w_packed, bias, y, dtype, stream));
    Ru3dDeviceGuard dev_guard(stream);
    RU3D_REQUIRE(convt_shapes_ok(x, y) && w_packed, "convtranspose3d_fwd: y must have extents 2*x");
    RU3D_REQUIRE(dtype_ok(dtype), "convtranspose3d_fwd: bad dtype");
    return run_conv(x, w_packed, bias, nullptr, y, 3, 2, 1, 0, 1, dtype, dtype, as_stream(stream));
}

static ConvGeom convt_fwd_geom(const ru3d_tensor* x, const ru3d_tensor* y) {
    return conv_geom(x, y, nullptr, 3, 2, 1, 0, 1);
}

static bool convt_fwd_in_fused(const ru3d_tensor* x, const ru3d_tensor* y, int dtype) {
    return dtype == RU3D_BF16 && convt_shapes_ok(x, y) && mfma_conv_eligible(x->c, y->c, 3, dtype, dtype) &&
           ((((uintptr_t)x->ptr) | ((uintptr_t)y->ptr)) % 16) == 0 && convt_s2_tile_eligible(convt_fwd_geom(x, y));
}

extern "C" size_t ru3d_convtranspose3d_k3s2p1_fwd_in_workspace_bytes(const ru3d_tensor* x, const ru3d_tensor* y, int dtype) {
    RU3D_FWD_F16(dtype, ru3d_convtranspose3d_k3s2p1_fwd_in_workspace_bytes_f16(x, y, dtype));
    if (!tensor_ok(x) || !tensor_ok(y)) return 0;
    size_t need = ru3d_reduce_workspace_bytes(y);
    if (convt_fwd_in_fused(x, y, dtype)) {
        const size_t slab = convt_s2_tile_slab_bytes(convt_fwd_geom(x, y));
        if (slab > need) need = slab;
    }
    return need;
}

extern "C" int ru3d_convtranspose3d_k3s2p1_fwd_in(const ru3d_tensor* x, const void* w_packed, const float* bias,
                                                  const ru3d_tensor* y, float* mean, float* scale, void* ws,
                                                  size_t ws_bytes, float eps, int dtype, void* stream) {
    RU3D_FWD_F16(dtype, ru3d_convtranspose3d_k3s2p1_fwd_in_f16(x, w_packed, bias, y, mean, scale, ws, ws_bytes, eps, dtype, stream));
    Ru3dDeviceGuard dev_guard(stream);
    RU3D_REQUIRE(convt_shapes_ok(x, y) && w_packed && mean && scale && ws, "convtranspose3d_fwd_in: bad argument");
    RU3D_REQUIRE(ws_bytes >= ru3d_convtranspose3d_k3s2p1_fwd_in_workspace_bytes(x, y, dtype),
                 "convtranspose3d_fwd_in: workspace too small");
    if (convt_fwd_in_fused(x, y, dtype)) {
        const ConvGeom g = convt_fwd_geom(x, y);
        int rc = convt_s2_tile_launch(x->ptr, w_packed, bias, nullptr, y->ptr, g, (float*)ws, nullptr, 0, nullptr, as_stream(stream));
        if (rc) return rc;
        int gx, cb;
        if (convt_s2_tile_slab_geom(g, &gx, &cb)) return ru3d_fail(-1, "convtranspose3d_fwd_in: no slab geometry");
        return stats_slab_finalize_launch((const float*)ws, gx, cb, g.N, g.Cout, 1.0 / ((double)g.Do * g.Ho * g.Wo), nullptr, eps,
                                          mean, scale, as_stream(stream));
    }
    int rc = ru3d_convtranspose3d_k3s2p1_fwd(x, w_packed, bias, y, dtype, stream);
    if (rc) return rc;
    return ru3d_instnorm_stats(y, nullptr, mean, scale, ws, ws_bytes, eps, dtype, stream);
}

extern "C" int ru3d_convtranspose3d_k3s2p1_dgrad(const ru3d_tensor* dy, const void* w_packed, const ru3d_tensor* dx,
                                                 int dtype, void* stream) {
    RU3D_FWD_F16(dtype, ru3d_convtranspose3d_k3s2p1_dgrad_f16(dy, w_packed, dx, dtype, stream));
    Ru3dDeviceGuard dev_guard(stream);
    RU3D_REQUIRE(convt_shapes_ok(dx, dy) && w_packed, "convtranspose3d_dgrad: dy must have extents 2*dx");
    RU3D_REQUIRE(dtype_ok(dtype), "convtranspose3d_dgrad: bad dtype");
    return run_conv(dy, w_packed, nullptr, nullptr, dx, 3, 2, 0, 0, 0, dtype, dtype, as_stream(stream));
}

static WgradGeom make_convt_wgrad(const ru3d_tensor* x, const ru3d_tensor* dy) {
    WgradGeom g = make_wgrad(dy, x, 3, 2);
    g.s_o = (int64_t)dy->c * 27;
    g.s_i = 27;
    return g;
}

extern "C" size_t ru3d_convtranspose3d_k3s2p1_wgrad_workspace_bytes(const ru3d_tensor* x, const ru3d_tensor* dy,
                                                                    int dtype) {
    RU3D_FWD_F16(dtype, ru3d_convtranspose3d_k3s2p1_wgrad_workspace_bytes_f16(x, dy, dtype));
    if (!convt_shapes_ok(x, dy)) return 0;
    WgradGeom g = make_convt_wgrad(x, dy);
    if (mfma_wgrad_eligible(g, dtype)) return wgrad_mfma_ws_bytes(g);
    return wgrad_generic_ws_bytes(g);
}

extern "C" int ru3d_convtranspose3d_k3s2p1_wgrad(const ru3d_tensor* x, const ru3d_tensor* dy, float* dw, void* ws,
                                                 size_t ws_bytes, int dtype, void* stream) {
    RU3D_FWD_F16(dtype, ru3d_convtranspose3d_k3s2p1_wgrad_f16(x, dy, dw, ws, ws_bytes, dtype, stream));
    Ru3dDeviceGuard dev_guard(stream);
    RU3D_REQUIRE(convt_shapes_ok(x, dy), "convtranspose3d_wgrad: dy must have extents 2*x");
    RU3D_REQUIRE(dw && dtype_ok(dtype), "convtranspose3d_wgrad: bad argument");
    WgradGeom g = make_convt_wgrad(x, dy);
    if (mfma_wgrad_eligible(g, dtype)) return wgrad_mfma_launch(dy->ptr, x->ptr, dw, ws, ws_bytes, g, as_stream(stream));
    return wgrad_generic_launch(dy->ptr, x->ptr, dw, ws, ws_bytes, g, dtype, as_stream(stream));
}

}
```

3d-unet-renal-anatomy-extraction_amd/csrc/common.h:

```cpp
#pragma once
#include <hip/hip_runtime.h>
#include <stdint.h>
#include <stdio.h>
#include <stdarg.h>
#include <stdlib.h>
#include "f16_names.h"
#include "../../include/ru3d.h"

#ifdef RU3D_STORAGE_F16
typedef _Float16 bf16;
#define RU3D_BF16 RU3D_F16
#define RU3D_NS ru3d_f16
#define RU3D_MFMA_32X32X16 __builtin_amdgcn_mfma_f32_32x32x16_f16
#define RU3D_MFMA_ASM "v_mfma_f32_32x32x16_f16"
#define RU3D_FWD_F16(dt, call)
#else
typedef __bf16 bf16;
#define RU3D_NS ru3d_bf16
#define RU3D_MFMA_32X32X16 __builtin_amdgcn_mfma_f32_32x32x16_bf16
#define RU3D_MFMA_ASM "v_mfma_f32_32x32x16_bf16"
#define RU3D_DECL_F16(name) extern "C" decltype(name) name##_f16;
RU3D_F16_APIS(RU3D_DECL_F16)
#define RU3D_FWD_F16(dt, call) \
    if ((dt) == RU3D_F16) return call
#endif
typedef __attribute__((ext_vector_type(8))) bf16 bf16x8;
typedef __attribute__((ext_vector_type(4))) bf16 bf16x4;
typedef __attribute__((ext_vector_type(4))) short i16x4;
typedef __attribute__((address_space(3))) i16x4 lds_i16x4;
#define RU3D_DS_READ_TR16(p) __builtin_bit_cast(bf16x4, __builtin_amdgcn_ds_read_tr16_b64_v4i16((lds_i16x4*)(p)))
typedef __attribute__((ext_vector_type(4))) float f32x4;
typedef __attribute__((ext_vector_type(16))) float f32x16;

#define RU3D_WAVE 64

typedef __attribute__((ext_vector_type(4))) int ru3d_i32x4;
__device__ __forceinline__ ru3d_i32x4 ru3d_buffer_rsrc(const void* base, int num_bytes) {
    const uint64_t p = (uint64_t)base;
    ru3d_i32x4 r = {(int)(uint32_t)p, (int)((uint32_t)(p >> 32) & 0xffffu), num_bytes, 0x00020000};
    return r;
}
__device__ __forceinline__ void ru3d_lds_dma16(const ru3d_i32x4& rsrc, const void* lds_dst, int byte_offset) {
    const uint32_t dst = (uint32_t)(uintptr_t)lds_dst;
    asm volatile("s_mov_b32 m0, %0\n\ts_nop 0\n\tbuffer_load_dwordx4 %1, %2, 0 offen lds"
                 :
                 : "s"(dst), "v"(byte_offset), "s"(rsrc)
                 : "memory", "m0");
}
__device__ __forceinline__ void ru3d_dma_landed_barrier() {
    asm volatile("s_waitcnt vmcnt(0) lgkmcnt(0)\n\ts_barrier" ::: "memory");
}

int ru3d_fail(int code, const char* fmt, ...);
int ru3d_check_launch(const char* what);

static inline hipStream_t as_stream(void* s) { return (hipStream_t)s; }

static inline int ru3d_env_int(const char* name, int dflt) {
    const char* v = getenv(name);
    return v ? atoi(v) : dflt;
}

void* ru3d_probe_start(int n, int d, int h, int w, int cin, int cout, hipStream_t st);
void ru3d_probe_stop(void* ev, hipStream_t st);

struct Ru3dDeviceGuard {
    int prev, want;
    explicit Ru3dDeviceGuard(void* stream) : prev(-1), want(-1) {
        if (!stream) return;
        hipDevice_t dev;
        if (hipStreamGetDevice((hipStream_t)stream, &dev) != hipSuccess) { (void)hipGetLastError(); return; }
        want = (int)dev;
        if (hipGetDevice(&prev) != hipSuccess) { prev = -1; return; }
        if (prev != want) (void)hipSetDevice(want);
    }
    ~Ru3dDeviceGuard() {
        if (prev >= 0 && want >= 0 && prev != want) (void)hipSetDevice(prev);
    }
};

static inline int64_t nvox(const ru3d_tensor* t) { return (int64_t)t->n * t->d * t->h * t->w; }

static inline int tensor_ok(const ru3d_tensor* t) {
    return t && t->ptr && t->n > 0 && t->d > 0 && t->h > 0 && t->w > 0 && t->c > 0 && t->ld >= t->c && t->cseg == 0;
}
static inline int tensor_ok_split(const ru3d_tensor* t) {
    if (t && t->cseg == 0) return tensor_ok(t);
    return t && t->ptr && t->n > 0 && t->d > 0 && t->h > 0 && t->w > 0 && t->c > 0 && t->cseg > 0 && (t->c % t->cseg) == 0 &&
           t->ld >= t->cseg && t->seg_stride >= (int64_t)t->n * t->d * t->h * t->w * t->ld;
}

#define RU3D_REQUIRE(cond, ...)                        \
    do {                                               \
        if (!(cond)) return ru3d_fail(-1, __VA_ARGS__); \
    } while (0)

template <typename T> __device__ __forceinline__ float to_f32(T v);
template <> __device__ __forceinline__ float to_f32<float>(float v) { return v; }
template <> __device__ __forceinline__ float to_f32<bf16>(bf16 v) { return (float)v; }

template <typename T> __device__ __forceinline__ T from_f32(float v);
template <> __device__ __forceinline__ float from_f32<float>(float v) { return v; }
template <> __device__ __forceinline__ bf16 from_f32<bf16>(float v) { return (bf16)v; }

template <typename T, int VEC> struct vec_t {
    T v[VEC];
};
template <typename T, int VEC>
__device__ __forceinline__ void load_vec(const T* p, float (&out)[VEC]) {
    typedef __attribute__((ext_vector_type(VEC))) T VT;
    VT x = *reinterpret_cast<const VT*>(p);
#pragma unroll
    for (int i = 0; i < VEC; i++) out[i] = to_f32<T>(x[i]);
}
template <typename T, int VEC>
__device__ __forceinline__ void store_vec(T* p, const float (&in)[VEC]) {
    typedef __attribute__((ext_vector_type(VEC))) T VT;
    VT x;
#pragma unroll
    for (int i = 0; i < VEC; i++) x[i] = from_f32<T>(in[i]);
    *reinterpret_cast<VT*>(p) = x;
}

__device__ __forceinline__ void ru3d_clear_own_slab_rows(float* slab, int64_t wave_row, int N, int row_floats) {
    float* base = slab + wave_row * (int64_t)N * row_floats;
    for (int i = threadIdx.x & 63; i < N * row_floats; i += 64) base[i] = 0.f;
    __builtin_amdgcn_s_waitcnt(0x0f70);
}

__device__ __forceinline__ float wave_sum(float v) {
#pragma unroll
    for (int o = 32; o > 0; o >>= 1) v += __shfl_xor(v, o, 64);
    return v;
}
__device__ __forceinline__ double wave_sum_d(double v) {
#pragma unroll
    for (int o = 32; o > 0; o >>= 1) v += __shfl_xor(v, o, 64);
    return v;
}

__device__ __forceinline__ float lrelu_f(float x, float slope) { return x > 0.f ? x : x * slope; }
```

3d-unet-renal-anatomy-extraction_amd/csrc/conv.h:

```cpp
#pragma once
#include "common.h"

namespace RU3D_NS {

struct ConvGeom {
    int N;
    int Di, Hi, Wi, Cin, ldx;
    int Do, Ho, Wo, Cout, ldy;
    int CoutPad;
    int ldr;
    int k, stride, pad;
    int transposed;
    int zero_far;
    int flip;
    int x_cseg = 0, y_cseg = 0;
    int64_t x_segstride = 0, y_segstride = 0;
};

struct WgradGeom {
    int N;
    int Di, Hi, Wi, Cin, ldx;
    int Do, Ho, Wo, Cout, lddy;
    int k, taps, stride, pad;
    int64_t s_o, s_i;
    int64_t chunk_len;
    int x_cseg = 0;
    int64_t x_segstride = 0;
};

struct PackOne {
    const float* src;
    void* dst;
    int cin, cout, taps, mfma, cout_pad;
    int co_real, co_pad, ci_real, ci_pad;
    int64_t s_o, s_i, total;
};
struct PackBatch {
    int count;
    PackOne item[RU3D_PACK_MAX];
};
int pack_batch_launch(const PackBatch& b, int dtype, hipStream_t st);

struct PackPair {
    const float* src;
    void* dst_a;
    void* dst_b;
    int adim, bdim, taps;
    int a_real, a_pad, b_real, b_pad;
    int64_t s_a;
};
struct PackPairBatch {
    int count;
    PackPair item[RU3D_PACK_MAX];
};
int pack_pair_launch(const PackPairBatch& b, hipStream_t st);
int unpad_weight_launch(const float* src, float* dst, int cout, int cin, int taps, int co_real, int co_pad, int ci_real,
                        int ci_pad, int cin_p, hipStream_t st);

int generic_cot(int cout);
int generic_cout_pad(int cout);
int conv_generic_launch(const void* x, const void* w, const float* bias, const void* res, void* y,
                        const ConvGeom& g, int dtype, int y_dtype, hipStream_t st);
int pack_generic_launch(const float* src, void* dst, int cin, int cout, int taps, int64_t s_o, int64_t s_i,
                        int flip, int dtype, hipStream_t st);
size_t wgrad_generic_ws_bytes(const WgradGeom& g);
int wgrad_reduce_launch(const float* part, float* dw, int chunks, int taps, int cin, int cout, int64_t s_o, int64_t s_i,
                        hipStream_t st);
int wgrad_generic_launch(const void* x, const void* dy, float* dw, void* ws, size_t ws_bytes, WgradGeom g, int dtype,
                         hipStream_t st);

bool mfma_conv_eligible(int cin, int cout, int k, int dtype, int y_dtype);
bool mfma_conv_geometry_ok(const ConvGeom& g);
size_t mfma_packed_bytes(int cin, int cout, int taps);
int pack_mfma_launch(const float* src, void* dst, int cin, int cout, int taps, int64_t s_o, int64_t s_i, int flip,
                     hipStream_t st);
enum { S1_SLIDE32 = 1, S1_SLIDE64, S1_WS, S1_PC4, S1_PC, S1_SK, S1_TILE };
struct SlidePlan {
    int dsplit, DL, tiles_h, tiles_w, units, grid, ny;
};
struct Conv3S1Choice {
    int family;
    int td, th, tw, mt, nt;
    int ks;
    char name[40];
};
struct Conv3S1Plan {
    int count = 0;
    Conv3S1Choice choice[5];
    SlidePlan slide;
    int pc_gx = 0, pc_gy = 0;
    size_t ws_bytes = 0;
    bool can_stats = false, can_bwd_sums = false, can_partner = false;
    int gx = 0, gy = 0, cb = 0;
    size_t slab_bytes = 0;
};
Conv3S1Plan conv3_s1_plan(const ConvGeom& g);
int conv_mfma_launch(const void* x, const void* w, const float* bias, const void* res, void* y, const ConvGeom& g,
                     hipStream_t st, float* stat_slab = nullptr, void* ws = nullptr, size_t ws_bytes = 0,
                     const void* bst_act = nullptr, int bst_ld = 0, float slope = 0.f, const void* x2 = nullptr,
                     int ldx2 = 0, const void* w2 = nullptr, int* defer_ks = nullptr, const Conv3S1Plan* plan = nullptr);
int stats_slab_finalize_launch(const float* slab, int gx, int cb, int N, int C, double invV, const float* drop, float eps,
                               float* mean, float* scale, hipStream_t st);
bool mfma_wgrad_eligible(const WgradGeom& g, int dtype);
size_t wgrad_mfma_ws_bytes(const WgradGeom& g);
int wgrad_mfma_launch(const void* x, const void* dy, float* dw, void* ws, size_t ws_bytes, WgradGeom g,
                      hipStream_t st);

bool slide_conv_plan(int N, int D, int H, int W, int Cin, int Cout, SlidePlan* out);
int conv_slide_launch(const void* x, const void* w, const float* bias, const void* res, void* y, const ConvGeom& g,
                      const SlidePlan& p, float* stat_slab, hipStream_t st, const void* bst_act = nullptr, int bst_ld = 0,
                      float slope = 0.f, const void* x2 = nullptr, int ldx2 = 0, const void* w2 = nullptr);

bool slide64_conv_plan(int N, int D, int H, int W, int Cin, int Cout, bool edge, SlidePlan* out);
int conv_ws_slices(int N, int D, int H, int W, int Cin, int Cout, int mode);
int conv_ws_launch(const void* x, const void* w, float* part, int N, int D, int H, int W, int Cin, int Cout, int ldx,
                   int flip, int slices, hipStream_t st);
int conv_slide64_launch(const void* x, const void* w, const float* bias, const void* res, void* y, const ConvGeom& g,
                        const SlidePlan& p, float* stat_slab, hipStream_t st);

bool convt_s2_tile_eligible(const ConvGeom& g);
size_t convt_s2_tile_slab_bytes(const ConvGeom& g);
int convt_s2_tile_slab_geom(const ConvGeom& g, int* gx, int* cb);
int convt_s2_tile_launch(const void* x, const void* w, const float* bias, const void* res, void* y, const ConvGeom& g,
                         float* stat_slab, const void* x2, int ldx2, const void* w2, hipStream_t st);

bool conv_s2_tile_eligible(const ConvGeom& g);
size_t conv_s2_tile_slab_bytes(const ConvGeom& g);
int conv_s2_tile_slab_geom(const ConvGeom& g, int* gx, int* cb);
int conv_s2_tile_launch(const void* x, const void* w, const float* bias, void* y, const ConvGeom& g, float* stat_slab,
                        const void* w2, const float* bias2, void* y2, int ldy2, hipStream_t st);

bool skip1x1_fused_eligible(const ru3d_tensor* x, const ru3d_tensor* y2, const ru3d_tensor* out, int dtype);
bool skip1x1_head_fused_eligible(const ru3d_tensor* x, const ru3d_tensor* y2, const ru3d_tensor* out,
                                 const ru3d_tensor* logits, int dtype);
int skip1x1_fused_launch(const ru3d_tensor* x, const void* w, const float* bias, const ru3d_tensor* y2, const float* mean,
                         const float* scale, const ru3d_tensor* out, float slope, hipStream_t st,
                         const void* head_w = nullptr, const float* head_bias = nullptr, const ru3d_tensor* logits = nullptr);

int in_small_mode(const ru3d_tensor* y, bool all_samples, const ru3d_tensor* a = nullptr, const ru3d_tensor* b = nullptr,
                  const ru3d_tensor* c = nullptr, const ru3d_tensor* d = nullptr);
size_t in_small_ws_bytes(const ru3d_tensor* y);
int in_small_fwd_launch(const ru3d_tensor* y, const float* part, int ksplit, const float* bias, const float* drop,
                        float* mean, float* scale, const ru3d_tensor* res, const ru3d_tensor* out, void* ws, float eps,
                        float slope, hipStream_t st);
int in_small_bwd_launch(const ru3d_tensor* gout, const float* part, int ksplit, const ru3d_tensor* outp,
                        const ru3d_tensor* y, const float* mean, const float* scale, const ru3d_tensor* dy,
                        const ru3d_tensor* gpre, void* ws, float slope, int zero_far, float* gpre_sum, hipStream_t st);

struct WgradSlidePlan {
    int dsplit, DL, tiles_h, tiles_w, units, G, pairs;
};
bool wgrad_slide_plan(const WgradGeom& g, WgradSlidePlan* out);
size_t wgrad_slide_ws_bytes(const WgradGeom& g);
int wgrad_slide_launch(const void* x, const void* dy, float* dw, void* ws, const WgradGeom& g, hipStream_t st);
size_t wgrad_slide_pair_ws_bytes(const WgradGeom& g);
int wgrad_slide_pair_launch(const void* x, const void* dy, const void* dy2, int lddy2, float* dw, float* dw2, void* ws,
                            const WgradGeom& g, hipStream_t st);

bool wgrad_s2_eligible(const WgradGeom& g);
size_t wgrad_s2_ws_bytes(const WgradGeom& g);
int wgrad_s2_launch(const void* x, const void* dy, float* dw, void* ws, const WgradGeom& g, hipStream_t st);
bool wgrad_s2_pair_eligible(const WgradGeom& g);
size_t wgrad_s2_pair_ws_bytes(const WgradGeom& g);
int wgrad_s2_pair_launch(const void* x, const void* dy, const void* dy2, int lddy2, float* dw, float* dw2, void* ws,
                         const WgradGeom& g, hipStream_t st);

bool stem_fwd_eligible(const ConvGeom& g, int dtype, int y_dtype, const void* res);
int stem_fwd_launch(const void* x, const void* w, const float* bias, void* y, const ConvGeom& g, int dtype,
                    hipStream_t st);
bool head_fwd_eligible(const ConvGeom& g, int dtype, const void* res);
int head_fwd_launch(const void* x, const void* w, const float* bias, void* y, const ConvGeom& g, int dtype,
                    int y_dtype, hipStream_t st);
bool head_dgrad_eligible(const ConvGeom& g, int dtype, int y_dtype, const void* res);
int head_dgrad_launch(const void* dy, const void* w, void* dx, const ConvGeom& g, int dtype, hipStream_t st);
bool stem_wgrad_eligible(const WgradGeom& g);
size_t stem_wgrad_ws_bytes(const WgradGeom& g);
int stem_wgrad_launch(const void* x, const void* dy, float* dw, void* ws, size_t ws_bytes, const WgradGeom& g,
                      int dtype, hipStream_t st, float* db = nullptr);
bool stem_wgrad_gives_bias(const WgradGeom& g, int dtype);
bool head_bwd_eligible(int Cin, int Cout, int dtype);
size_t head_bwd_ws_bytes(int64_t P, int Cin);
int head_bwd_launch(const void* a, int lda, const float* dlog, int ldd, const float* w, int cin_real, int Cin, int Cout,
                    void* dx, int lddx, float* dw, float* db, void* ws, int64_t P, hipStream_t st);
bool head_wgrad_eligible(const WgradGeom& g, int dtype);
size_t head_wgrad_ws_bytes(const WgradGeom& g);
int head_wgrad_launch(const void* x, const void* dy, float* dw, void* ws, size_t ws_bytes, const WgradGeom& g,
                      int dtype, hipStream_t st);

}
using namespace RU3D_NS;
```

3d-unet-renal-anatomy-extraction_amd/csrc/conv_generic.hip:

```cpp
#include "common.h"
#include "conv.h"

namespace RU3D_NS {

template <typename T, typename TO, int CO_T, int VEC, bool TRANSPOSED>
__global__ __launch_bounds__(256) void conv_generic_kernel(const T* __restrict__ x, const T* __restrict__ w,
                                                           const float* __restrict__ bias,
                                                           const TO* __restrict__ res, TO* __restrict__ y,
                                                           ConvGeom g) {
    const int64_t total = (int64_t)g.N * g.Do * g.Ho * g.Wo;
    const int64_t vo = (int64_t)blockIdx.x * 256 + threadIdx.x;
    if (vo >= total) return;
    const int co0 = blockIdx.y * CO_T;
    int ow = (int)(vo % g.Wo);
    int64_t t = vo / g.Wo;
    int oh = (int)(t % g.Ho);
    t /= g.Ho;
    int od = (int)(t % g.Do);
    int n = (int)(t / g.Do);

    float acc[CO_T];
#pragma unroll
    for (int j = 0; j < CO_T; j++) acc[j] = 0.f;

    const int k = g.k, s = g.stride, p = g.pad;
    for (int kd = 0; kd < k; kd++) {
        int id;
        if (!TRANSPOSED) {
            id = od * s + kd - p;
            if (id < 0 || id >= g.Di) continue;
        } else {
            int q = od + p - kd;
            if (q < 0 || (q % s) != 0) continue;
            id = q / s;
            if (id >= g.Di) continue;
        }
        for (int kh = 0; kh < k; kh++) {
            int ih;
            if (!TRANSPOSED) {
                ih = oh * s + kh - p;
                if (ih < 0 || ih >= g.Hi) continue;
            } else {
                int q = oh + p - kh;
                if (q < 0 || (q % s) != 0) continue;
                ih = q / s;
                if (ih >= g.Hi) continue;
            }
            for (int kw = 0; kw < k; kw++) {
                int iw;
                if (!TRANSPOSED) {
                    iw = ow * s + kw - p;
                    if (iw < 0 || iw >= g.Wi) continue;
                } else {
                    int q = ow + p - kw;
                    if (q < 0 || (q % s) != 0) continue;
                    iw = q / s;
                    if (iw >= g.Wi) continue;
                }
                const int tap = (kd * k + kh) * k + kw;
                const T* xp = x + ((((int64_t)n * g.Di + id) * g.Hi + ih) * g.Wi + iw) * g.ldx;
                const int wtap = g.flip ? (k * k * k - 1 - tap) : tap;
                const T* wp = w + (int64_t)wtap * g.Cin * g.CoutPad + co0;
                for (int ci = 0; ci < g.Cin; ci += VEC) {
                    float xv[VEC];
                    load_vec<T, VEC>(xp + ci, xv);
#pragma unroll
                    for (int u = 0; u < VEC; u++) {
                        const T* wr = wp + (int64_t)(ci + u) * g.CoutPad;
#pragma unroll
                        for (int j = 0; j < CO_T; j++) acc[j] = fmaf(xv[u], to_f32<T>(wr[j]), acc[j]);
                    }
                }
            }
        }
    }
    const bool far = g.zero_far && (od == g.Do - 1 || oh == g.Ho - 1 || ow == g.Wo - 1);
#pragma unroll
    for (int j = 0; j < CO_T; j++) {
        const int co = co0 + j;
        if (co < g.Cout) {
            float v = acc[j];
            if (bias) v += bias[co];
            if (far) v = 0.f;
            if (res) v += to_f32<TO>(res[vo * g.ldr + co]);
            y[vo * g.ldy + co] = from_f32<TO>(v);
        }
    }
}

int generic_cot(int cout) { return cout <= 4 ? 4 : (cout % 16 == 0 ? 16 : 8); }
int generic_cout_pad(int cout) {
    int t = generic_cot(cout);
    return (cout + t - 1) / t * t;
}

template <typename T, typename TO, int CO_T, int VEC>
static int launch_generic2(const void* x, const void* w, const float* bias, const void* res, void* y,
                           const ConvGeom& g, hipStream_t st) {
    const int64_t total = (int64_t)g.N * g.Do * g.Ho * g.Wo;
    dim3 grid((unsigned)((total + 255) / 256), (unsigned)(g.CoutPad / CO_T));
    if (g.transposed)
        hipLaunchKernelGGL((conv_generic_kernel<T, TO, CO_T, VEC, true>), grid, dim3(256), 0, st, (const T*)x,
                           (const T*)w, bias, (const TO*)res, (TO*)y, g);
    else
        hipLaunchKernelGGL((conv_generic_kernel<T, TO, CO_T, VEC, false>), grid, dim3(256), 0, st, (const T*)x,
                           (const T*)w, bias, (const TO*)res, (TO*)y, g);
    return ru3d_check_launch("conv_generic");
}

template <typename T, typename TO>
static int launch_generic1(const void* x, const void* w, const float* bias, const void* res, void* y,
                           const ConvGeom& g, hipStream_t st) {
    const bool v4 = (g.Cin % 4 == 0) && (g.ldx % 4 == 0) && (((uintptr_t)x) % (4 * sizeof(T)) == 0);
    const int cot = generic_cot(g.Cout);
#define GO(CO, V) return launch_generic2<T, TO, CO, V>(x, w, bias, res, y, g, st)
    if (cot == 4) { if (v4) GO(4, 4); else GO(4, 1); }
    if (cot == 8) { if (v4) GO(8, 4); else GO(8, 1); }
    if (v4) GO(16, 4); else GO(16, 1);
#undef GO
}

int conv_generic_launch(const void* x, const void* w, const float* bias, const void* res, void* y,
                        const ConvGeom& g, int dtype, int y_dtype, hipStream_t st) {
    if (dtype == RU3D_F32 && y_dtype == RU3D_F32) return launch_generic1<float, float>(x, w, bias, res, y, g, st);
    if (dtype == RU3D_BF16 && y_dtype == RU3D_BF16) return launch_generic1<bf16, bf16>(x, w, bias, res, y, g, st);
    if (dtype == RU3D_BF16 && y_dtype == RU3D_F32) return launch_generic1<bf16, float>(x, w, bias, res, y, g, st);
    return ru3d_fail(-1, "conv_generic: unsupported dtype pair (%d -> %d)", dtype, y_dtype);
}

template <typename T>
__global__ void pack_generic_kernel(const float* __restrict__ src, T* __restrict__ dst, int cin, int cout,
                                    int cout_pad, int taps, int64_t s_o, int64_t s_i, int flip) {
    const int64_t total = (int64_t)taps * cin * cout_pad;
    for (int64_t i = (int64_t)blockIdx.x * blockDim.x + threadIdx.x; i < total; i += (int64_t)gridDim.x * blockDim.x) {
        int co = (int)(i % cout_pad);
        int64_t t = i / cout_pad;
        int ci = (int)(t % cin);
        int tap = (int)(t / cin);
        float v = 0.f;
        if (co < cout) {
            int st = flip ? (taps - 1 - tap) : tap;
            v = src[co * s_o + ci * s_i + st];
        }
        dst[i] = from_f32<T>(v);
    }
}

int pack_generic_launch(const float* src, void* dst, int cin, int cout, int taps, int64_t s_o, int64_t s_i,
                        int flip, int dtype, hipStream_t st) {
    const int cp = generic_cout_pad(cout);
    const int64_t total = (int64_t)taps * cin * cp;
    int blocks = (int)((total + 255) / 256);
    if (blocks > 4096) blocks = 4096;
    if (dtype == RU3D_F32)
// ... 155 lines not shown
        }
        __syncthreads();
        if (p.dst_a) {
            const int KS = p.bdim / 16, NTT = TA;
            for (int f = wave; f < taps * 2; f += 4) {
                const int tap = f >> 1, kc = f & 1;
                const bf16x8 v = *reinterpret_cast<const bf16x8*>(&tile[tap * PP_PLANE + (lane & 31) * PP_PITCH + 16 * kc + 8 * (lane >> 5)]);
                *reinterpret_cast<bf16x8*>((bf16*)p.dst_a + ((((int64_t)tap * KS + 2 * tb + kc) * NTT + ta) * 64 + lane) * 8) = v;
            }
        }
        if (p.dst_b) {
            const int KS = p.adim / 16, NTT = TB;
            for (int f = wave; f < taps * 2; f += 4) {
                const int tap = f >> 1, kc = f & 1;
                const int a0 = 16 * kc + 8 * (lane >> 5);
                bf16x8 v;
#pragma unroll
                for (int j = 0; j < 8; j++) v[j] = tile[tap * PP_PLANE + (a0 + j) * PP_PITCH + (lane & 31)];
                *reinterpret_cast<bf16x8*>((bf16*)p.dst_b + ((((int64_t)tap * KS + 2 * ta + kc) * NTT + tb) * 64 + lane) * 8) = v;
            }
        }
    }
}

int pack_pair_launch(const PackPairBatch& b, hipStream_t st) {
    int64_t mx = 1;
    for (int i = 0; i < b.count; i++) {
        const int64_t units = (int64_t)(b.item[i].adim / 32) * (b.item[i].bdim / 32);
        mx = units > mx ? units : mx;
    }
    if (mx > 1024) mx = 1024;
    bool t27 = false, t1 = false;
    for (int i = 0; i < b.count; i++) {
        t27 = t27 || b.item[i].taps == 27;
        t1 = t1 || b.item[i].taps == 1;
    }
    if (t27) hipLaunchKernelGGL(pack_pair_kernel<27>, dim3((unsigned)mx, b.count), dim3(256), 0, st, b);
    if (t1) hipLaunchKernelGGL(pack_pair_kernel<1>, dim3((unsigned)mx, b.count), dim3(256), 0, st, b);
    return ru3d_check_launch("pack_pair");
}

__global__ __launch_bounds__(256) void unpad_weight_kernel(const float* __restrict__ src, float* __restrict__ dst,
                                                           int cout, int cin, int taps, int co_real, int co_pad,
                                                           int ci_real, int ci_pad, int cin_p) {
    const int64_t total = (int64_t)cout * cin * taps;
    for (int64_t i = (int64_t)blockIdx.x * 256 + threadIdx.x; i < total; i += (int64_t)gridDim.x * 256) {
        const int tap = (int)(i % taps);
        const int64_t t = i / taps;
        const int ci = (int)(t % cin), co = (int)(t / cin);
        const int cop = co_pad ? (co / co_real) * co_pad + co % co_real : co;
        const int cip = ci_pad ? (ci / ci_real) * ci_pad + ci % ci_real : ci;
        dst[i] = src[((int64_t)cop * cin_p + cip) * taps + tap];
    }
}

int unpad_weight_launch(const float* src, float* dst, int cout, int cin, int taps, int co_real, int co_pad, int ci_real,
                        int ci_pad, int cin_p, hipStream_t st) {
    const int64_t total = (int64_t)cout * cin * taps;
    int64_t blocks = (total + 1023) / 1024;
    if (blocks > 2048) blocks = 2048;
    hipLaunchKernelGGL(unpad_weight_kernel, dim3((unsigned)blocks), dim3(256), 0, st, src, dst, cout, cin, taps, co_real,
                       co_pad, ci_real, ci_pad, cin_p);
    return ru3d_check_launch("unpad_weight_grad");
}

int pack_batch_launch(const PackBatch& b, int dtype, hipStream_t st) {
    int64_t mx = 1;
    for (int i = 0; i < b.count; i++) mx = b.item[i].total > mx ? b.item[i].total : mx;
    int64_t blocks = (mx + 1023) / 1024;
    if (blocks > 2048) blocks = 2048;
    dim3 grid((unsigned)blocks, b.count);
    if (dtype == RU3D_F32)
        hipLaunchKernelGGL(pack_batch_kernel<float>, grid, dim3(256), 0, st, b);
    else
        hipLaunchKernelGGL(pack_batch_kernel<bf16>, grid, dim3(256), 0, st, b);
    return ru3d_check_launch("pack_batch");
}

#define WG_PB 16
template <typename T>
__global__ __launch_bounds__(256) void wgrad_generic_kernel(const T* __restrict__ x, const T* __restrict__ dy,
                                                            float* __restrict__ part, WgradGeom g) {
    __shared__ float xs[WG_PB][64 + 4];
    __shared__ float ds[WG_PB][64 + 4];
    const int tid = threadIdx.x;
    const int chunk = blockIdx.x, tap = blockIdx.y;
    const int co_tiles = (g.Cout + 63) / 64;
    const int ci0 = (blockIdx.z / co_tiles) * 64, co0 = (blockIdx.z % co_tiles) * 64;
    const int kw = tap % g.k, kh = (tap / g.k) % g.k, kd = tap / (g.k * g.k);
    const int ty = tid / 16, tx = tid % 16;
    float acc[4][4];
#pragma unroll
    for (int i = 0; i < 4; i++)
#pragma unroll
        for (int j = 0; j < 4; j++) acc[i][j] = 0.f;

    const int64_t P = (int64_t)g.N * g.Do * g.Ho * g.Wo;
    const int64_t p_begin = (int64_t)chunk * g.chunk_len;
    int64_t p_end = p_begin + g.chunk_len;
    if (p_end > P) p_end = P;

    for (int64_t p0 = p_begin; p0 < p_end; p0 += WG_PB) {
#pragma unroll
        for (int r = 0; r < 4; r++) {
            const int e = tid + r * 256;
            const int pl = e / 64, c = e % 64;
            const int64_t pos = p0 + pl;
            float xv = 0.f, dv = 0.f;
            if (pos < p_end) {
                int ow = (int)(pos % g.Wo);
                int64_t t = pos / g.Wo;
                int oh = (int)(t % g.Ho);
                t /= g.Ho;
                int od = (int)(t % g.Do);
                int n = (int)(t / g.Do);
                if (co0 + c < g.Cout) dv = to_f32<T>(dy[pos * g.lddy + co0 + c]);
                const int id = od * g.stride + kd - g.pad, ih = oh * g.stride + kh - g.pad,
                          iw = ow * g.stride + kw - g.pad;
                if (ci0 + c < g.Cin && id >= 0 && id < g.Di && ih >= 0 && ih < g.Hi && iw >= 0 && iw < g.Wi)
                    xv = to_f32<T>(x[((((int64_t)n * g.Di + id) * g.Hi + ih) * g.Wi + iw) * g.ldx + ci0 + c]);
            }
            xs[pl][c] = xv;
            ds[pl][c] = dv;
        }
        __syncthreads();
#pragma unroll
        for (int pl = 0; pl < WG_PB; pl++) {
            float a[4], b[4];
#pragma unroll
            for (int i = 0; i < 4; i++) a[i] = xs[pl][ty * 4 + i];
#pragma unroll
            for (int j = 0; j < 4; j++) b[j] = ds[pl][tx * 4 + j];
#pragma unroll
            for (int i = 0; i < 4; i++)
#pragma unroll
                for (int j = 0; j < 4; j++) acc[i][j] = fmaf(a[i], b[j], acc[i][j]);
        }
        __syncthreads();
    }
    float* pp = part + ((int64_t)chunk * g.taps + tap) * g.Cin * g.Cout;
#pragma unroll
    for (int i = 0; i < 4; i++) {
        const int ci = ci0 + ty * 4 + i;
        if (ci >= g.Cin) continue;
#pragma unroll
        for (int j = 0; j < 4; j++) {
            const int co = co0 + tx * 4 + j;
            if (co < g.Cout) pp[(int64_t)ci * g.Cout + co] = acc[i][j];
        }
    }
}

template <int QX>
__global__ __launch_bounds__(256) void wgrad_reduce_kernel(const float* __restrict__ part, float* __restrict__ dw,
                                                           int chunks, int taps, int cin, int cout, int64_t s_o,
                                                           int64_t s_i) {
    constexpr int KY = 256 / QX;
    __shared__ f32x4 sh[KY][QX];
    const int64_t total = (int64_t)taps * cin * cout;
    const int ox = threadIdx.x % QX, ky = threadIdx.x / QX;
    const int64_t i0 = ((int64_t)blockIdx.x * QX + ox) * 4;
    f32x4 s = {0.f, 0.f, 0.f, 0.f};
    const bool full = (i0 + 3 < total) && ((total & 3) == 0);
    if (full) {
        f32x4 s0 = s, s1 = s, s2 = s, s3 = s;
        int c = ky;
        for (; c + 3 * KY < chunks; c += 4 * KY) {
            s0 += *reinterpret_cast<const f32x4*>(part + (int64_t)c * total + i0);
            s1 += *reinterpret_cast<const f32x4*>(part + (int64_t)(c + KY) * total + i0);
            s2 += *reinterpret_cast<const f32x4*>(part + (int64_t)(c + 2 * KY) * total + i0);
            s3 += *reinterpret_cast<const f32x4*>(part + (int64_t)(c + 3 * KY) * total + i0);
        }
        for (; c < chunks; c += KY) s0 += *reinterpret_cast<const f32x4*>(part + (int64_t)c * total + i0);
        s = (s0 + s1) + (s2 + s3);
    } else {
        for (int j = 0; j < 4; j++)
            if (i0 + j < total)
                for (int c = ky; c < chunks; c += KY) s[j] += part[(int64_t)c * total + i0 + j];
    }
    sh[ky][ox] = s;
    __syncthreads();
    if (ky == 0) {
        s = sh[0][ox];
#pragma unroll
        for (int k = 1; k < KY; k++) s += sh[k][ox];
        for (int j = 0; j < 4; j++) {
            const int64_t i = i0 + j;
            if (i >= total) break;
            const int co = (int)(i % cout);
            const int64_t t = i / cout;
            const int ci = (int)(t % cin);
            const int tap = (int)(t / cin);
            dw[co * s_o + ci * s_i + tap] = s[j];
        }
    }
}

template <bool CO_MAJOR>
__device__ __forceinline__ void wgrad_reduce_tiled_body(const float* __restrict__ part, float* __restrict__ dw, int chunks,
                                                        int taps, int cin, int cout, int64_t s_o, int64_t s_i, int bid,
                                                        float* tile) {
    const int cot = bid % (cout / 32), cit = bid / (cout / 32);
    const int ci0 = cit * 4, co0 = cot * 32;
    const int64_t total = (int64_t)taps * cin * cout;
    const int nquads = taps * 32;
    const int pitch_co = 4 * taps + 1;
    constexpr int QPT = 4;
    const float* src[QPT];
    bool live[QPT];
    f32x4 acc[QPT][4];
#pragma unroll
    for (int k = 0; k < QPT; k++) {
        const int qid = threadIdx.x + 256 * k;
        live[k] = qid < nquads;
        const int qq = live[k] ? qid : 0;
        const int tap = qq >> 5, ci_l = (qq >> 3) & 3, co4 = qq & 7;
        src[k] = part + ((int64_t)tap * cin + ci0 + ci_l) * cout + co0 + co4 * 4;
#pragma unroll
        for (int j = 0; j < 4; j++) acc[k][j] = f32x4{0.f, 0.f, 0.f, 0.f};
    }
    int c = 0;
    for (; c + 3 < chunks; c += 4) {
        f32x4 v[QPT][4];
#pragma unroll
        for (int k = 0; k < QPT; k++)
#pragma unroll
            for (int j = 0; j < 4; j++) v[k][j] = *reinterpret_cast<const f32x4*>(src[k] + (int64_t)(c + j) * total);
#pragma unroll
        for (int k = 0; k < QPT; k++)
#pragma unroll
            for (int j = 0; j < 4; j++) acc[k][j] += v[k][j];
    }
    for (; c < chunks; c++) {
#pragma unroll
        for (int k = 0; k < QPT; k++) acc[k][0] += *reinterpret_cast<const f32x4*>(src[k] + (int64_t)c * total);
    }
#pragma unroll
    for (int k = 0; k < QPT; k++) {
        if (!live[k]) continue;
        const int qid = threadIdx.x + 256 * k;
        const int tap = qid >> 5, ci_l = (qid >> 3) & 3, co4 = qid & 7;
        const f32x4 s = (acc[k][0] + acc[k][1]) + (acc[k][2] + acc[k][3]);
#pragma unroll
        for (int e = 0; e < 4; e++) {
            const int co = co4 * 4 + e;
            if (CO_MAJOR) tile[co * pitch_co + ci_l * taps + tap] = s[e];
            else tile[ci_l * (32 * taps + 1) + co * taps + tap] = s[e];
        }
    }
    __syncthreads();
    if (CO_MAJOR) {
        const int run = 4 * taps;
        for (int e = threadIdx.x; e < 32 * run; e += 256) {
            const int co = e / run, j = e - co * run;
            dw[(int64_t)(co0 + co) * s_o + (int64_t)ci0 * s_i + j] = tile[co * pitch_co + j];
        }
    } else {
        const int run = 32 * taps;
        for (int e = threadIdx.x; e < 4 * run; e += 256) {
            const int ci = e / run, j = e - ci * run;
            dw[(int64_t)(ci0 + ci) * s_i + (int64_t)co0 * s_o + j] = tile[ci * (run + 1) + j];
        }
    }
}

template <bool CO_MAJOR>
__global__ __launch_bounds__(256) void wgrad_reduce_tiled_kernel(const float* __restrict__ part, float* __restrict__ dw,
                                                                 int chunks, int taps, int cin, int cout, int64_t s_o,
                                                                 int64_t s_i) {
    __shared__ float tile[32 * (4 * 27 + 1)];
    wgrad_reduce_tiled_body<CO_MAJOR>(part, dw, chunks, taps, cin, cout, s_o, s_i, blockIdx.x, tile);
}

int wgrad_reduce_launch(const float* part, float* dw, int chunks, int taps, int cin, int cout, int64_t s_o, int64_t s_i,
                        hipStream_t st) {
    const int64_t total = (int64_t)taps * cin * cout;
    const bool tiled = (int64_t)cin * cout >= 128 * 128 && (cin % 4) == 0 && (cout % 32) == 0 && taps <= 27 &&
                       (s_i == taps || s_o == taps);
    if (tiled) {
        const int64_t blocks = (int64_t)(cin / 4) * (cout / 32);
        if (blocks > 0x3fffffff) return ru3d_fail(-1, "wgrad_reduce: grid too large");
        if (s_i == taps)
            hipLaunchKernelGGL(wgrad_reduce_tiled_kernel<true>, dim3((unsigned)blocks), dim3(256), 0, st, part, dw, chunks, taps,
                               cin, cout, s_o, s_i);
        else
            hipLaunchKernelGGL(wgrad_reduce_tiled_kernel<false>, dim3((unsigned)blocks), dim3(256), 0, st, part, dw, chunks, taps,
                               cin, cout, s_o, s_i);
        return ru3d_check_launch(s_i == taps ? "wgrad_reduce_tiled<true>" : "wgrad_reduce_tiled<false>");
    }
    const bool deep = chunks >= 128 && (total + 255) / 256 < 512;
    const int qx = deep ? 8 : 64;
    const int64_t blocks = (total + 4 * qx - 1) / (4 * qx);
    if (blocks > 0x3fffffff) return ru3d_fail(-1, "wgrad_reduce: grid too large");
    if (deep)
        hipLaunchKernelGGL(wgrad_reduce_kernel<8>, dim3((unsigned)blocks), dim3(256), 0, st, part, dw, chunks, taps, cin, cout,
                           s_o, s_i);
    else
        hipLaunchKernelGGL(wgrad_reduce_kernel<64>, dim3((unsigned)blocks), dim3(256), 0, st, part, dw, chunks, taps, cin, cout,
                           s_o, s_i);
    return ru3d_check_launch(deep ? "wgrad_reduce<8>" : "wgrad_reduce<64>");
}

int wgrad_generic_chunks(const WgradGeom& g) {
    const int64_t P = (int64_t)g.N * g.Do * g.Ho * g.Wo;
    const int tiles = ((g.Cin + 63) / 64) * ((g.Cout + 63) / 64);
    int64_t want = 2048 / ((int64_t)g.taps * tiles);
    if (want < 1) want = 1;
    int64_t maxc = (P + WG_PB * 16 - 1) / (WG_PB * 16);
    if (want > maxc) want = maxc;
    if (want < 1) want = 1;
    return (int)want;
}

size_t wgrad_generic_ws_bytes(const WgradGeom& g) {
    return (size_t)wgrad_generic_chunks(g) * g.taps * g.Cin * g.Cout * sizeof(float);
}

int wgrad_generic_launch(const void* x, const void* dy, float* dw, void* ws, size_t ws_bytes, WgradGeom g, int dtype,
                         hipStream_t st) {
    const int chunks = wgrad_generic_chunks(g);
    const size_t need = wgrad_generic_ws_bytes(g);
    if (!ws || ws_bytes < need) return ru3d_fail(-1, "wgrad: workspace too small (%zu < %zu)", ws_bytes, need);
    const int64_t P = (int64_t)g.N * g.Do * g.Ho * g.Wo;
    int64_t len = (P + chunks - 1) / chunks;
    len = (len + WG_PB - 1) / WG_PB * WG_PB;
    g.chunk_len = len;
    const int tiles = ((g.Cin + 63) / 64) * ((g.Cout + 63) / 64);
    dim3 grid(chunks, g.taps, tiles);
    if (dtype == RU3D_F32)
        hipLaunchKernelGGL(wgrad_generic_kernel<float>, grid, dim3(256), 0, st, (const float*)x, (const float*)dy,
                           (float*)ws, g);
    else
        hipLaunchKernelGGL(wgrad_generic_kernel<bf16>, grid, dim3(256), 0, st, (const bf16*)x, (const bf16*)dy,
                           (float*)ws, g);
    int rc = ru3d_check_launch("wgrad_generic");
    if (rc) return rc;
    return wgrad_reduce_launch((const float*)ws, dw, chunks, g.taps, g.Cin, g.Cout, g.s_o, g.s_i, st);
}

}
```

3d-unet-renal-anatomy-extraction_amd/graph.py:

```python
import torch

import _native as N
import _ops
import loss as _loss
import optim as _optim

_RING = 8


class GraphedTrainStep:
    def __init__(self, model, criterion, optimizer, warmup=2, scaler=None):
        if not isinstance(optimizer, _optim._Fused):
            raise TypeError("GraphedTrainStep needs optim.Adam, optim.AdamW or optim.SGD (their update kernels read the "
                            "per-step scalars from device memory)")
        if scaler is not None and not optimizer.captures_with_scaler():
            raise TypeError("GraphedTrainStep: a captured fp16 step (device-side loss scaler) needs optim.Adam without "
                            "max_grad_norm; SGD, AdamW and clipped steps run the eager fp16 loop")
        self.model, self.criterion, self.optimizer = model, criterion, optimizer
        self.scaler = scaler
        self.warmup = max(1, int(warmup))
        self.graph = None
        self.key = None
        self.replays = 0
        self.eager_steps = 0

    def _eager(self, x, y):
        self.optimizer.zero_grad(set_to_none=True)
        logits = self.model(x)
        loss = self.criterion(logits, y)
        stepped = True
        if self.scaler is None:
            loss.backward()
            self.optimizer.step()
        elif self.scaler._dev is not None:
            stepped = self.scaler.eager_step(self.optimizer, loss)
        else:
            self.scaler.scale(loss).backward()
            stepped = self.scaler.step(self.optimizer)
        self.eager_steps += 1 if (stepped or self.graph is not None) else 0
        self.skipped_warmup = getattr(self, "skipped_warmup", 0) + (0 if stepped else 1)
        self.logits = _loss.main_output(logits).detach()
        return loss.detach()

    def _capture(self, x, y):
        dev = x.device
        groups = len(self.optimizer.param_groups)
        self.stream = torch.cuda.Stream(dev)
        drop0 = _ops._drop_counter[0]
        import loss as _loss_mod
        try:
            self.x = torch.empty_like(x)
            self.y = torch.empty_like(y)
            self.x.copy_(x)
            self.y.copy_(y)
            self.block = torch.zeros(8 + groups * 32, dtype=torch.uint8, device=dev)
            self.drop_base = self.block[:8].view(torch.int64)
            self.hyper = self.block[8:].view(torch.float32).view(groups, 8)
            self.host = [torch.zeros(8 + groups * 32, dtype=torch.uint8).pin_memory() for _ in range(_RING)]
            self.host_ev = [None] * _RING
            self.optimizer.begin_capture(self.hyper)
            if self.scaler is not None:
                self.scaler.begin_capture(self.optimizer, dev)
            self.optimizer.zero_grad(set_to_none=True)
            g = torch.cuda.CUDAGraph()
            _ops.DROP_OFFSET_BASE[0] = self.drop_base
            _loss_mod.CAPTURE_SINK[0] = self.label_states = []
            self.stream.wait_stream(torch.cuda.current_stream(dev))
            try:
                with torch.cuda.graph(g, stream=self.stream, capture_error_mode="thread_local"):
                    logits = self.model(self.x)
                    loss = self.criterion(logits, self.y)
                    if self.scaler is None:
                        loss.backward()
                        self.optimizer.step()
                    else:
                        self.scaler.scale(loss).backward()
                        self.scaler.step(self.optimizer)
                    self.loss = loss.detach()
                    self._static_logits = _loss_mod.main_output(logits).detach()
            finally:
                _ops.DROP_OFFSET_BASE[0] = None
                _loss_mod.CAPTURE_SINK[0] = None
        except BaseException:
            _ops._drop_counter[0] = drop0
            cap = self.optimizer._captured
            if cap is not None and cap["steps"]:
                cap["dirty"] = True
            self.release()
            raise
        self.draws = _ops._drop_counter[0] - drop0
        _ops._drop_counter[0] = drop0
        self.drop_origin = drop0
        self.graph = g
        self.key = (tuple(x.shape), x.dtype, tuple(y.shape), y.dtype, dev)

    def __call__(self, x, y):
        key = (tuple(x.shape), x.dtype, tuple(y.shape), y.dtype, x.device)
        if self.graph is None:
            if self.eager_steps < self.warmup:
                return self._eager(x, y)
            self._capture(x, y)
        elif key != self.key:
            return self._eager(x, y)
        else:
            self.x.copy_(x, non_blocking=True)
            self.y.copy_(y, non_blocking=True)
        slot = self.replays % _RING
        if self.host_ev[slot] is not None:
            self.host_ev[slot].synchronize()
        host = self.host[slot]
        host[:8].view(torch.int64)[0] = _ops._drop_counter[0] - self.drop_origin
        self.optimizer.replay_scalars(host[8:].view(torch.float32).view(-1, 8))
        self.block.copy_(host, non_blocking=True)
        ev = torch.cuda.Event()
        ev.record()
        self.host_ev[slot] = ev
        self.graph.replay()
        if self.label_states:
            import loss as _loss_mod
            for st in self.label_states:
                _loss_mod._note_label_flag(st)
        _ops._drop_counter[0] += self.draws
        _ops.WEIGHTS_EPOCH[0] += 1
        self.replays += 1
        self.logits = self._static_logits
        return self.loss

    def release(self):
        self.optimizer.sync_captured_steps()
        if self.scaler is not None and self.scaler._dev is not None:
            self.scaler.end_capture()
        self.optimizer.end_capture()
        if self.graph is not None or hasattr(self, "stream"):
            self.optimizer.zero_grad(set_to_none=True)
            sid = self.stream.cuda_stream
            side = _ops._SIDE.get(self.stream.device)
            sids = (sid,) if side is None else (sid, side.cuda_stream)
            for key in [k for k in N._WS if k[1] in sids]:
                del N._WS[key]
            _ops._PREPACK.clear()
            for name in ("x", "y", "loss", "logits", "_static_logits", "block", "drop_base", "hyper", "host", "host_ev",
                         "stream", "label_states"):
                if hasattr(self, name):
                    delattr(self, name)
        self.graph = None
        self.key = None
```

include/ru3d.h:

```cpp
#ifndef RU3D_H
#define RU3D_H

#include <stddef.h>
#include <stdint.h>

#ifdef __cplusplus
extern "C" {
#endif

#define RU3D_VERSION 201

enum { RU3D_F32 = 0, RU3D_BF16 = 1, RU3D_F16 = 2 };

enum { RU3D_LABEL_I64 = 0, RU3D_LABEL_U8 = 1 };

enum {
    RU3D_ROLE_CONV_FWD = 0,
    RU3D_ROLE_CONV_DGRAD = 1,
    RU3D_ROLE_CONVT_FWD = 2,
    RU3D_ROLE_CONVT_DGRAD = 3,
    RU3D_ROLE_BIAS = 4
};

enum {
    RU3D_LOSS_HYBIRD = 0,
    RU3D_LOSS_DICELOSS = 1,
    RU3D_LOSS_FOCAL = 2,
    RU3D_LOSS_DICE = 3
};

typedef struct ru3d_tensor {
    void* ptr;
    int32_t n, d, h, w;
    int32_t c;
    int32_t ld;
    int32_t cseg;
    int64_t seg_stride;
} ru3d_tensor;

int ru3d_version(void);
const char* ru3d_last_error(void);
void ru3d_launch_log_begin(void);
const char* ru3d_launch_log_end(void);

size_t ru3d_packed_weight_bytes(int cout, int cin, int k, int stride, int role, int dtype);
int ru3d_pack_weight(const float* src, void* dst, int cout, int cin, int k, int stride, int role, int dtype,
                     void* stream);

#define RU3D_PACK_MAX 40
typedef struct ru3d_pack_item {
    const float* src;
    void* dst;
    int32_t cout, cin, k, stride, role;
    int32_t cout_seg, cin_seg;
} ru3d_pack_item;
int ru3d_pack_weights(const ru3d_pack_item* items, int count, int dtype, void* stream);

int ru3d_unpad_weight_grad(const float* src, float* dst, int cout, int cin, int taps, int cout_seg, int cin_seg,
                           void* stream);

size_t ru3d_conv3d_workspace_bytes(const ru3d_tensor* x, const ru3d_tensor* y, int k, int stride, int dtype);
int ru3d_conv3d_fwd(const ru3d_tensor* x, const void* w_packed, const float* bias, const ru3d_tensor* res,
                    const ru3d_tensor* y, int k, int stride, int dtype, int y_dtype, void* ws,
                    size_t ws_bytes, void* stream);
size_t ru3d_conv3d_fwd_in_workspace_bytes(const ru3d_tensor* x, const ru3d_tensor* y, int k, int stride, int dtype);
int ru3d_conv3d_fwd_in(const ru3d_tensor* x, const void* w_packed, const float* bias, const ru3d_tensor* y, int k,
                       int stride, int dtype, const float* drop_scale, float* mean, float* scale, void* ws,
                       size_t ws_bytes, float eps, void* stream);
size_t ru3d_conv3d_fwd_in_lrelu_workspace_bytes(const ru3d_tensor* x, const ru3d_tensor* y, int k, int stride, int dtype);
int ru3d_conv3d_fwd_in_lrelu(const ru3d_tensor* x, const void* w_packed, const float* bias, const ru3d_tensor* y, int k,
                             int stride, int dtype, const float* drop_scale, float* mean, float* scale,
                             const ru3d_tensor* res, const ru3d_tensor* out, float slope, void* ws, size_t ws_bytes,
                             float eps, void* stream);
int ru3d_planar_concat_supported(int n, int d, int h, int w, int cseg, int cout, int dtype);
int ru3d_conv3d_dgrad(const ru3d_tensor* dy, const void* w_packed, const ru3d_tensor* res,
                      const ru3d_tensor* dx, int k, int stride, int dtype, void* ws, size_t ws_bytes,
                      void* stream);
int ru3d_conv3d_s1_dgrad_pair_supported(const ru3d_tensor* dy, const ru3d_tensor* dy2, const ru3d_tensor* dx, int dtype);
int ru3d_conv3d_s1_dgrad_pair(const ru3d_tensor* dy, const void* w3_packed, const ru3d_tensor* dy2, const void* w1_packed,
                              const ru3d_tensor* dx, int dtype, void* stream);
int ru3d_conv3d_s2_pair_fwd_in_supported(const ru3d_tensor* x, const ru3d_tensor* y3, const ru3d_tensor* y1, int dtype);
size_t ru3d_conv3d_s2_pair_fwd_in_workspace_bytes(const ru3d_tensor* x, const ru3d_tensor* y3, int dtype);
int ru3d_conv3d_s2_pair_fwd_in(const ru3d_tensor* x, const void* w3_packed, const float* b3, const ru3d_tensor* y3,
                               const void* w1_packed, const float* b1, const ru3d_tensor* y1, const float* drop_scale,
                               float* mean, float* scale, void* ws, size_t ws_bytes, float eps, int dtype, void* stream);
int ru3d_conv3d_s2_dgrad_pair_supported(const ru3d_tensor* dy, const ru3d_tensor* dy2, const ru3d_tensor* res,
                                        const ru3d_tensor* dx, int dtype);
int ru3d_conv3d_s2_dgrad_pair(const ru3d_tensor* dy, const void* w3_packed, const ru3d_tensor* dy2,
                              const void* w1_packed, const ru3d_tensor* res, const ru3d_tensor* dx, int dtype,
                              void* stream);
size_t ru3d_conv3d_wgrad_workspace_bytes(const ru3d_tensor* x, const ru3d_tensor* dy, int k, int stride, int dtype);
int ru3d_conv3d_wgrad(const ru3d_tensor* x, const ru3d_tensor* dy, float* dw, void* ws, size_t ws_bytes,
                      int k, int stride, int dtype, void* stream);

int ru3d_conv3d_wgrad_pair_supported(const ru3d_tensor* x, const ru3d_tensor* dy, const ru3d_tensor* dy2, int stride, int dtype);
size_t ru3d_conv3d_wgrad_pair_workspace_bytes(const ru3d_tensor* x, const ru3d_tensor* dy, const ru3d_tensor* dy2, int stride,
                                              int dtype);
int ru3d_conv3d_wgrad_pair(const ru3d_tensor* x, const ru3d_tensor* dy, const ru3d_tensor* dy2, float* dw, float* dw2,
                           void* ws, size_t ws_bytes, int stride, int dtype, void* stream);
size_t ru3d_conv3d_wgrad_bias_workspace_bytes(const ru3d_tensor* x, const ru3d_tensor* dy, int k, int stride, int dtype);
int ru3d_conv3d_wgrad_bias(const ru3d_tensor* x, const ru3d_tensor* dy, float* dw, float* db, void* ws, size_t ws_bytes,
                           int k, int stride, int dtype, void* stream);
int ru3d_head_bwd_supported(const ru3d_tensor* x, const ru3d_tensor* dlogits, const ru3d_tensor* dx, int dtype);
size_t ru3d_head_bwd_workspace_bytes(const ru3d_tensor* x, int dtype);
int ru3d_head_bwd(const ru3d_tensor* x, const ru3d_tensor* dlogits, const float* weight, int cin_real, const ru3d_tensor* dx,
                  float* dw, float* db, void* ws, size_t ws_bytes, int dtype, void* stream);
int ru3d_head_in_bwd_supported(const ru3d_tensor* z, const ru3d_tensor* dlogits, const ru3d_tensor* y,
                               const ru3d_tensor* gpre, const ru3d_tensor* dy, int dtype);
size_t ru3d_head_in_bwd_workspace_bytes(const ru3d_tensor* z, int dtype);
int ru3d_head_in_bwd(const ru3d_tensor* z, const ru3d_tensor* dlogits, const float* weight, int cin_real,
                     const ru3d_tensor* y, const float* mean, const float* scale, const ru3d_tensor* gpre,
                     const ru3d_tensor* dy, float* dw, float* db, float* gpre_sum, void* ws, size_t ws_bytes, float slope,
                     int dtype, void* stream);

int ru3d_convtranspose3d_k3s2p1_fwd(const ru3d_tensor* x, const void* w_packed, const float* bias,
                                    const ru3d_tensor* y, int dtype, void* stream);
size_t ru3d_convtranspose3d_k3s2p1_fwd_in_workspace_bytes(const ru3d_tensor* x, const ru3d_tensor* y, int dtype);
int ru3d_convtranspose3d_k3s2p1_fwd_in(const ru3d_tensor* x, const void* w_packed, const float* bias,
                                       const ru3d_tensor* y, float* mean, float* scale, void* ws, size_t ws_bytes,
                                       float eps, int dtype, void* stream);
int ru3d_convtranspose3d_k3s2p1_dgrad(const ru3d_tensor* dy, const void* w_packed, const ru3d_tensor* dx,
                                      int dtype, void* stream);
size_t ru3d_convtranspose3d_k3s2p1_wgrad_workspace_bytes(const ru3d_tensor* x, const ru3d_tensor* dy, int dtype);
int ru3d_convtranspose3d_k3s2p1_wgrad(const ru3d_tensor* x, const ru3d_tensor* dy, float* dw, void* ws,
                                      size_t ws_bytes, int dtype, void* stream);

size_t ru3d_reduce_workspace_bytes(const ru3d_tensor* t);
int ru3d_instnorm_stats(const ru3d_tensor* y, const float* drop_scale, float* mean, float* scale,
                        void* ws, size_t ws_bytes, float eps, int dtype, void* stream);
int ru3d_skip1x1_in_lrelu_fwd_supported(const ru3d_tensor* x, const ru3d_tensor* y, const ru3d_tensor* out, int dtype);
int ru3d_skip1x1_in_lrelu_fwd(const ru3d_tensor* x, const void* w_packed, const float* bias, const ru3d_tensor* y,
                              const float* mean, const float* scale, const ru3d_tensor* out, float slope, int dtype,
                              void* stream);
int ru3d_skip1x1_in_lrelu_head_fwd_supported(const ru3d_tensor* x, const ru3d_tensor* y, const ru3d_tensor* out,
                                             const ru3d_tensor* logits, int dtype);
int ru3d_skip1x1_in_lrelu_head_fwd(const ru3d_tensor* x, const void* w_packed, const float* bias, const ru3d_tensor* y,
                                   const float* mean, const float* scale, const ru3d_tensor* out, const void* head_w_packed,
                                   const float* head_bias, const ru3d_tensor* logits, float slope, int dtype, void* stream);
int ru3d_in_lrelu_fwd(const ru3d_tensor* y, const float* mean, const float* scale, const ru3d_tensor* res,
                      const ru3d_tensor* out, float slope, int dtype, void* stream);
int ru3d_in_lrelu_bwd(const ru3d_tensor* gout, const ru3d_tensor* out, const ru3d_tensor* y, const float* mean,
                      const float* scale, const ru3d_tensor* dy, const ru3d_tensor* gpre, void* ws,
                      size_t ws_bytes, float slope, int zero_far, float* gpre_sum, float* dy_sum, int dtype,
                      void* stream);
int ru3d_channel_sum(const ru3d_tensor* t, float* out, void* ws, size_t ws_bytes, int dtype, void* stream);
int ru3d_dropout3d_scale(float* scale, int count, float p, uint64_t seed, uint64_t offset, void* stream);
int ru3d_dropout3d_scale_dev(float* scale, int count, float p, uint64_t seed, uint64_t offset,
                             const uint64_t* offset_base, void* stream);

int ru3d_pointwise(int op, const ru3d_tensor* a, const ru3d_tensor* b, const ru3d_tensor* c, const ru3d_tensor* o1,
                   const ru3d_tensor* o2, float slope, int dtype, void* stream);

int ru3d_copy_channels(const ru3d_tensor* src, const ru3d_tensor* dst, int dtype, void* stream);
int ru3d_add(const ru3d_tensor* a, const ru3d_tensor* b, const ru3d_tensor* dst, int dtype, void* stream);
int ru3d_cast_f32(const ru3d_tensor* src, const ru3d_tensor* dst, int dst_dtype, void* stream);
int ru3d_ncdhw_to_ndhwc(const float* src, const ru3d_tensor* dst, int dtype, void* stream);
int ru3d_ndhwc_to_ncdhw(const ru3d_tensor* src, float* dst, int dtype, void* stream);

size_t ru3d_loss_state_bytes(int num_classes);
size_t ru3d_loss_state_bad_labels_offset(void);
size_t ru3d_loss_workspace_bytes(int n, int64_t v, int num_classes);
int ru3d_loss_fwd(const float* logits, int64_t stride_n, int64_t stride_c, int64_t stride_v, const void* labels,
                  int label_dtype, int n, int64_t v, int num_classes, int kind, float gamma, const float* weight_v,
                  float alpha, float beta, float smooth, void* state, float* loss_out, void* ws, size_t ws_bytes,
                  void* stream);
int ru3d_loss_bwd(const float* logits, int64_t stride_n, int64_t stride_c, int64_t stride_v, const void* labels,
                  int label_dtype, int n, int64_t v, int num_classes, float gamma, const void* state,
                  const float* grad_out, void* dlogits, int dlogits_dtype, void* stream);
int ru3d_tversky(const float* p, const float* g, int64_t count, float alpha, float beta, float smooth,
                 float* out, void* ws, size_t ws_bytes, void* stream);

int ru3d_predict_accumulate(const ru3d_tensor* logits, int dtype, int sample, float* acc, float* cnt, int X, int Y,
                            int Z, int ox, int oy, int oz, void* stream);
int ru3d_predict_merge(const float* acc, const float* cnt, int X, int Y, int Z, int num_classes, int cx, int cy,
                       int cz, int sx, int sy, int sz, int one_hot, void* out, void* stream);
#define RU3D_PREDICT_MAX_BATCH 16
int ru3d_predict_gather(const float* vol, int X, int Y, int Z, int cin, const int32_t* windows, int count,
                        const ru3d_tensor* dst, void* stream);
int ru3d_predict_accumulate_weighted(const ru3d_tensor* logits, int dtype, int sample, int flip, const float* gx,
                                     const float* gy, const float* gz, float* acc, float* cnt, int X, int Y, int Z,
                                     int ox, int oy, int oz, void* stream);

size_t ru3d_group_loss_state_bytes(void);
size_t ru3d_group_loss_workspace_bytes(int n, int64_t v, int num_groups);
int ru3d_group_loss_fwd(const float* logits, int64_t stride_n, int64_t stride_c, int64_t stride_v, const void* labels,
                        int label_dtype, int n, int64_t v, int num_groups, const uint8_t* table, int num_labels,
                        int has_ignore, int ignore_label, int kind, float gamma, const float* weight_v, float alpha,
                        float beta, float smooth, void* state, float* loss_out, void* ws, size_t ws_bytes, void* stream);
int ru3d_group_loss_bwd(const float* logits, int64_t stride_n, int64_t stride_c, int64_t stride_v, const void* labels,
                        int label_dtype, int n, int64_t v, int num_groups, const uint8_t* table, int num_labels,
                        int has_ignore, int ignore_label, float gamma, const void* state, const float* grad_out,
                        void* dlogits, int dlogits_dtype, void* stream);
typedef struct ru3d_topk_result {
    float tau;
    int64_t count_gt;
    int64_t count_eq;
    double sum_gt;
} ru3d_topk_result;
size_t ru3d_topk_select_workspace_bytes(int64_t n);
int64_t ru3d_topk_select_trip_elements(void);
int ru3d_topk_select(const float* values, int64_t n, int64_t K, ru3d_topk_result* result, void* ws, size_t ws_bytes,
                     void* stream);
size_t ru3d_topk_loss_state_bytes(void);
size_t ru3d_topk_loss_workspace_bytes(int n, int64_t v, int num_classes);
int ru3d_topk_loss_fwd(const float* logits, int64_t stride_n, int64_t stride_c, int64_t stride_v, const void* labels,
                       int label_dtype, int n, int64_t v, int num_classes, int64_t K, int with_dice,
                       const float* weight_v, float alpha, float beta, float smooth, float ce_weight, float* ce,
                       void* state, float* loss_out, void* ws, size_t ws_bytes, void* stream);
int ru3d_topk_loss_fwd_launches(void);
int ru3d_topk_loss_fwd_timed(const float* logits, int64_t stride_n, int64_t stride_c, int64_t stride_v, const void* labels,
                             int label_dtype, int n, int64_t v, int num_classes, int64_t K, int with_dice,
                             const float* weight_v, float alpha, float beta, float smooth, float ce_weight, float* ce,
                             void* state, float* loss_out, void* ws, size_t ws_bytes, float* launch_ms, void* stream);
int ru3d_topk_loss_bwd(const float* logits, int64_t stride_n, int64_t stride_c, int64_t stride_v, const void* labels,
                       int label_dtype, int n, int64_t v, int num_classes, int with_dice, const float* ce,
                       const void* state, const float* grad_out, void* dlogits, int dlogits_dtype, void* stream);
int ru3d_predict_accumulate_groups(const ru3d_tensor* logits, int dtype, int sample, int flip, const float* gx,
                                   const float* gy, const float* gz, float* acc, float* cnt, int X, int Y, int Z,
                                   int ox, int oy, int oz, void* stream);
int ru3d_predict_merge_groups(const float* acc, const float* cnt, int X, int Y, int Z, int num_groups,
                              const int32_t* group_labels, const float* threshold, int cx, int cy, int cz, int sx,
                              int sy, int sz, uint8_t* out, void* stream);

size_t ru3d_components_workspace_bytes(int X, int Y, int Z);
int ru3d_label_components(const uint8_t* mask, int X, int Y, int Z, int32_t* labels, int32_t* count_dev, void* ws,
                          size_t ws_bytes, void* stream);
int ru3d_component_stats(const int32_t* labels, int X, int Y, int Z, int count, int32_t* sizes, int32_t* boxes,
                         void* stream);
size_t ru3d_filter_components_workspace_bytes(int count);
int ru3d_filter_components(const int32_t* labels, int X, int Y, int Z, int count, const int32_t* sizes, int threshold,
                           uint8_t* mask_inout, int32_t* labels_out, int32_t* kept_dev, void* ws, size_t ws_bytes,
                           void* stream);
int ru3d_region_accumulate(const float* prob, int rx, int ry, int rz, int num_classes, int bx, int by, int bz,
                           double* total, int32_t* hits, int X, int Y, int Z, void* stream);
int ru3d_cascade_merge(const double* total, const int32_t* hits, int X, int Y, int Z, int num_classes, uint8_t* out,
                       void* stream);

enum { RU3D_MASK_NE = 0, RU3D_MASK_EQ = 1, RU3D_MASK_GT = 2, RU3D_MASK_GE = 3 };
enum { RU3D_MORPH_ERODE = 0, RU3D_MORPH_DILATE = 1 };
#define RU3D_MORPH_MAX_EXTENT 15
#define RU3D_MORPH_MAX_ROWS 225
typedef struct ru3d_morph_row {
    int8_t dx, dy;
    uint16_t zmask;
} ru3d_morph_row;
size_t ru3d_mask_bytes(int X, int Y, int Z);
int ru3d_mask_pack(const uint8_t* src, int X, int Y, int Z, int op, int value, uint64_t* bits, void* stream);
int ru3d_mask_unpack(const uint64_t* bits, int X, int Y, int Z, int value, int paint, uint8_t* dst, void* stream);
int ru3d_binary_morph(const uint64_t* src, uint64_t* dst, int X, int Y, int Z, int op, const ru3d_morph_row* rows,
                      int num_rows, int border_value, void* stream);
int ru3d_confusion_counts(const uint8_t* pred, const uint8_t* label, int64_t n, int num_classes, int64_t* table,
                          void* stream);

int ru3d_threshold_bbox(const float* image, int X, int Y, int Z, int C, float threshold, int32_t* box, int64_t* count,
                        void* stream);
size_t ru3d_masked_sample_workspace_bytes(int X, int Y, int Z);
int ru3d_masked_sample(const float* image, int X, int Y, int Z, int C, int channel, const void* label, int label_dtype,
                       int stride, float* out, int64_t capacity, int64_t* count, void* ws, size_t ws_bytes, void* stream);
#define RU3D_ORDER_STATS_MAX_RANKS 8
size_t ru3d_order_stats_workspace_bytes(void);
int ru3d_order_stats(const float* values, int64_t n, const int64_t* ranks, int num_ranks, float* out, void* ws,
                     size_t ws_bytes, void* stream);
size_t ru3d_moments_workspace_bytes(void);
int ru3d_moments(const float* values, int64_t n, double* out, void* ws, size_t ws_bytes, void* stream);

#define RU3D_EDT_MAX_AXIS 4096
size_t ru3d_edt_workspace_bytes(int X, int Y, int Z);
int ru3d_edt_squared(const uint64_t* bits, int X, int Y, int Z, const double* spacing, double* out, void* ws,
                     size_t ws_bytes, void* stream);
int ru3d_mask_surface(const uint64_t* src, uint64_t* dst, int X, int Y, int Z, void* stream);
size_t ru3d_edt_gather_workspace_bytes(int X, int Y, int Z);
int ru3d_edt_gather(const double* sq, const uint64_t* query, int X, int Y, int Z, double* values, int64_t capacity,
                    int64_t* count, void* ws, size_t ws_bytes, void* stream);
size_t ru3d_edt_reduce_workspace_bytes(int64_t capacity);
int ru3d_edt_reduce(const double* values, const int64_t* count, int64_t capacity, double tau_sq, double* out, void* ws,
                    size_t ws_bytes, void* stream);

size_t ru3d_skeleton_workspace_bytes(int X, int Y, int Z);
// ... 238 lines not shown
```

Measured before the change: 277.7 million voxels/s.

## Defer weight-gradient partial reductions into one batched multi-item reduce kernel

Weight-gradient kernels now write their per-chunk partials into dedicated slab workspaces and record a pending descriptor instead of launching a reduce kernel each time. At the end of the backward pass, an autograd-engine callback builds a cost-sorted block map on the host, copies it through pinned memory, and launches a single kernel that reduces every pending weight gradient. The goal is to remove many small reduce launches and their tail underutilisation. In exchange it costs extra workspace memory (up to a cap) because slabs cannot be reused, adds host-side bookkeeping and a host-to-device table copy per step, and adds extra handling for graph capture.

```diff
diff --git a/3d-unet-renal-anatomy-extraction_amd/_native.py b/3d-unet-renal-anatomy-extraction_amd/_native.py
--- a/3d-unet-renal-anatomy-extraction_amd/_native.py
+++ b/3d-unet-renal-anatomy-extraction_amd/_native.py
@@ -25,6 +25,12 @@
     _fields_ = [("src", ctypes.c_void_p), ("dst", ctypes.c_void_p), ("cout", ctypes.c_int32), ("cin", ctypes.c_int32),
                 ("k", ctypes.c_int32), ("stride", ctypes.c_int32), ("role", ctypes.c_int32),
                 ("cout_seg", ctypes.c_int32), ("cin_seg", ctypes.c_int32)]
+
+
+class WgradPending(ctypes.Structure):
+    _fields_ = [("part", ctypes.c_void_p), ("dw", ctypes.c_void_p), ("chunks", ctypes.c_int32), ("taps", ctypes.c_int32),
+                ("cin", ctypes.c_int32), ("cout", ctypes.c_int32), ("s_o", ctypes.c_int64), ("s_i", ctypes.c_int64),
+                ("variant", ctypes.c_int32), ("blocks", ctypes.c_int32)]
 
 
 class PatchParams(ctypes.Structure):
@@ -87,6 +93,7 @@
 BOUNDARY_MAX_AXIS = 2048
 DEGRADE_MAX_RADIUS = 16
 PACK_MAX = 40
+WGSUM_TILED_CO, WGSUM_TILED_CI, WGSUM_Q64, WGSUM_Q8 = 0, 1, 2, 3
 _P = ctypes.POINTER(Tensor)
 _vp, _i, _i64, _f, _sz, _u64 = (ctypes.c_void_p, ctypes.c_int, ctypes.c_int64, ctypes.c_float, ctypes.c_size_t,
                                 ctypes.c_uint64)
@@ -134,6 +141,12 @@
     "ru3d_convtranspose3d_k3s2p1_dgrad": (_i, [_P, _vp, _P, _i, _vp]),
     "ru3d_convtranspose3d_k3s2p1_wgrad_workspace_bytes": (_sz, [_P, _P, _i]),
     "ru3d_convtranspose3d_k3s2p1_wgrad": (_i, [_P, _P, _vp, _vp, _sz, _i, _vp]),
+    "ru3d_conv3d_wgrad_deferred": (_i, [_P, _P, _vp, _vp, _sz, _i, _i, _i, _vp, _vp, _i, ctypes.POINTER(_i)]),
+    "ru3d_conv3d_wgrad_pair_deferred": (_i, [_P, _P, _P, _vp, _vp, _vp, _sz, _i, _i, _vp, _vp, _i, ctypes.POINTER(_i)]),
+    "ru3d_conv3d_wgrad_bias_deferred": (_i, [_P, _P, _vp, _vp, _vp, _sz, _i, _i, _i, _vp, _vp, _i, ctypes.POINTER(_i)]),
+    "ru3d_convtranspose3d_k3s2p1_wgrad_deferred": (_i, [_P, _P, _vp, _vp, _sz, _i, _vp, _vp, _i, ctypes.POINTER(_i)]),
+    "ru3d_wgrad_block_map": (_i, [_vp, _i, _vp, _i]),
+    "ru3d_wgrad_reduce_multi": (_i, [_vp, _i, _vp, _i, _vp]),
     "ru3d_reduce_workspace_bytes": (_sz, [_P]),
     "ru3d_instnorm_stats": (_i, [_P, _vp, _vp, _vp, _vp, _sz, _f, _i, _vp]),
     "ru3d_in_lrelu_fwd": (_i, [_P, _vp, _vp, _P, _P, _f, _i, _vp]),
diff --git a/3d-unet-renal-anatomy-extraction_amd/_ops.py b/3d-unet-renal-anatomy-extraction_amd/_ops.py
--- a/3d-unet-renal-anatomy-extraction_amd/_ops.py
+++ b/3d-unet-renal-anatomy-extraction_amd/_ops.py
@@ -340,12 +340,159 @@
     return torch.empty(shape, dtype=torch.float32, device=device)
 
 
+WGRAD_DEFER = [os.environ.get("RU3D_WGRAD_DEFER", "1") != "0"]
+WGRAD_DEFER_CAP = [int(os.environ.get("RU3D_WGRAD_DEFER_CAP", str(3 << 30)))]
+_TABLE_RING = 4
+WGRAD_DEFER_STATS = {"flushes": 0, "items": 0, "blocks": 0, "bytes": 0, "arena": 0}
+_WKEY_PARAM = {}
+_WKEY_USES = {}
+_PENDING = {}
+_CAPTURE_TABLE = {}
+
+
+def reserve_capture_table(device, nbytes=1 << 20):
+    if WGRAD_DEFER[0]:
+        _CAPTURE_TABLE[device] = [torch.empty(int(nbytes), dtype=torch.uint8).pin_memory() for _ in range(_TABLE_RING)]
+
+
+def wkey(weight, ctx):
+    k = weight.data_ptr()
+    _WKEY_PARAM[k] = weakref.ref(weight)
+    if any(ctx.needs_input_grad):
+        _WKEY_USES[k] = _WKEY_USES.get(k, 0) + 1
+    return k
+
+
+class _Pending:
+    def __init__(self):
+        self.items = []
+        self.task = -1
+        self.slabs, self.need = [], 0
+        self.ring = []
+        self.turn = 0
+
+
+def _may_defer(key, dtype, device):
+    if not WGRAD_DEFER[0] or key is None or dtype == torch.float32 or torch.is_grad_enabled() or key in GRAD_ARENA:
+        return None
+    wr = _WKEY_PARAM.get(key)
+    p = wr() if wr is not None else None
+    if p is None or not p.is_leaf or not p.requires_grad or p.grad is not None or p._backward_hooks or \
+            getattr(p, "_post_accumulate_grad_hooks", None):
+        return None
+    task = torch._C._current_graph_task_id()
+    if task < 0 or (not _CAPTURE_TABLE.get(device) and torch.cuda.is_current_stream_capturing()):
+        return None
+    skey = (device, torch.cuda.current_stream(device).cuda_stream)
+    st = _PENDING.get(skey)
+    if st is None:
+        st = _PENDING[skey] = _Pending()
+    if st.task != task:
+        st.items, st.slabs, st.need = [], [], 0
+        try:
+            torch.autograd.Variable._execution_engine.queue_callback(lambda: _flush_pending(skey, task))
+        except RuntimeError:
+            return None
+        st.task = task
+    if _WKEY_USES.get(key, 0) != 1:
+        return None
+    return st, wr, skey
+
+
+def _slab_ws(st, skey, nbytes):
+    nbytes = max(256, (int(nbytes) + 255) // 256 * 256)
+    if st.need + nbytes > WGRAD_DEFER_CAP[0]:
+        return None
+    with torch.cuda.stream(torch.cuda.ExternalStream(skey[1], device=skey[0])):
+        ws = torch.empty(nbytes, dtype=torch.uint8, device=skey[0])
+    st.slabs.append(ws)
+    st.need += nbytes
+    return ws
+
+
+def _note_pending(st, wr, recs, n):
+    for i in range(n):
+        st.items.append((N.WgradPending.from_buffer_copy(recs[i]), wr[i] if isinstance(wr, (list, tuple)) else wr))
+
+
+def _flush_pending(skey, task, final=True):
+    st = _PENDING.get(skey)
+    if st is None or st.task != task:
+        return
+    items, need, slabs = st.items, st.need, st.slabs
+    st.items, st.slabs, st.need = [], [], 0
+    if final:
+        st.task = -1
+        _WKEY_USES.clear()
+    if not items:
+        return
+    dev, sid = skey
+    lost = [rec for rec, wr in items if wr() is None or wr().grad is None or wr().grad.data_ptr() != rec.dw] if final else []
+    if lost:
+        raise N.Ru3dError("ru3d: %d deferred weight gradients are not their parameters' .grad at the flush; run with "
+                          "RU3D_WGRAD_DEFER=0" % len(lost))
+    n = len(items)
+    arr = (N.WgradPending * n)(*[rec for rec, _ in items])
+    nblocks = N.lib.ru3d_wgrad_block_map(arr, n, None, 0)
+    if nblocks <= 0:
+        check(-1, "wgrad_block_map")
+    isz = ctypes.sizeof(N.WgradPending) * n
+    off = (isz + 15) // 16 * 16
+    total = off + 8 * nblocks
+    capturing = torch.cuda.is_current_stream_capturing()
+    with torch.cuda.stream(torch.cuda.ExternalStream(sid, device=dev)):
+        if capturing:
+            host = _CAPTURE_TABLE[dev].pop() if _CAPTURE_TABLE.get(dev) else None
+            if host is None or host.numel() < total:
+                raise N.Ru3dError("ru3d: the captured step's deferred slab sums need a %d-byte table, %d reserved "
+                                  "(ops.reserve_capture_table)" % (total, 0 if host is None else host.numel()))
+            table = torch.empty(total, dtype=torch.uint8, device=dev)
+            N._WS[(dev, sid, "wgrad_tables", len(N._WS))] = (host, table)
+        else:
+            if len(st.ring) < _TABLE_RING:
+                st.ring.append([None, None, None])
+            slot = st.ring[st.turn % len(st.ring)]
+            st.turn += 1
+            if slot[2] is not None:
+                slot[2].synchronize()
+            if slot[0] is None or slot[0].numel() < total:
+                slot[0] = torch.empty(max(total, 1 << 16), dtype=torch.uint8).pin_memory()
+                slot[1] = torch.empty(slot[0].numel(), dtype=torch.uint8, device=dev)
+            host, table = slot[0], slot[1]
+        base = host.data_ptr()
+        ctypes.memmove(base, arr, isz)
+        if N.lib.ru3d_wgrad_block_map(arr, n, ctypes.c_void_p(base + off), nblocks) != nblocks:
+            check(-1, "wgrad_block_map")
+        table[:total].copy_(host[:total], non_blocking=True)
+        N.note_device(dev)
+        check(N.lib.ru3d_wgrad_reduce_multi(ctypes.c_void_p(table.data_ptr()), n, ctypes.c_void_p(table.data_ptr() + off),
+                                            nblocks, ctypes.c_void_p(sid)), "wgrad_reduce_multi")
+        if not capturing:
+            slot[2] = torch.cuda.Event()
+            slot[2].record()
+        del slabs
+    S = WGRAD_DEFER_STATS
+    S["flushes"] += 1
+    S["items"], S["blocks"], S["arena"] = n, nblocks, need
+    S["bytes"] = sum(4 * r.taps * r.cin * r.cout * (r.chunks + 1) for r, _ in items)
+
+
 def conv_wgrad(x, dy, k, stride, key=None):
     cout, cin = dy.shape[1], x.shape[1]
     dw = _grad_out(key, (cout, cin, k, k, k), x.device)
     dx, ddy = desc(x), desc(dy)
     code = N.dtype_code(x.dtype)
     nbytes = N.lib.ru3d_conv3d_wgrad_workspace_bytes(ref(dx), ref(ddy), k, stride, code)
+    defer = _may_defer(key, x.dtype, x.device)
+    if defer is not None:
+        st, wr, skey = defer
+        ws = _slab_ws(st, skey, nbytes)
+    if defer is not None and ws is not None:
+        recs, n = (N.WgradPending * 2)(), ctypes.c_int(0)
+        check(N.lib.ru3d_conv3d_wgrad_deferred(ref(dx), ref(ddy), ptr(dw), ptr(ws), ws.numel(), k, stride, code, stream(),
+                                               recs, 2, ctypes.byref(n)), "conv3d_wgrad_deferred")
+        _note_pending(st, wr, recs, n.value)
+        return dw
     ws = N.workspace(nbytes, x.device)
     check(N.lib.ru3d_conv3d_wgrad(ref(dx), ref(ddy), ptr(dw), ptr(ws), ws.numel(), k, stride, code, stream()),
           "conv3d_wgrad")
@@ -369,19 +516,43 @@
     cout, cin = dy.shape[1], x.shape[1]
     dw = _grad_out(key, (cout, cin, 3, 3, 3), x.device)
     dw2 = _grad_out(key2, (cout, cin, 1, 1, 1), x.device)
-    ws = N.workspace(N.lib.ru3d_conv3d_wgrad_pair_workspace_bytes(ref(dx), ref(ddy), ref(ddy2), stride, code), x.device)
+    nbytes = N.lib.ru3d_conv3d_wgrad_pair_workspace_bytes(ref(dx), ref(ddy), ref(ddy2), stride, code)
+    defer, defer2 = _may_defer(key, x.dtype, x.device), _may_defer(key2, x.dtype, x.device)
+    if defer is not None and defer2 is not None:
+        st, wr, skey = defer
+        ws = _slab_ws(st, skey, nbytes)
+    if defer is not None and defer2 is not None and ws is not None:
+        recs, n = (N.WgradPending * 2)(), ctypes.c_int(0)
+        check(N.lib.ru3d_conv3d_wgrad_pair_deferred(ref(dx), ref(ddy), ref(ddy2), ptr(dw), ptr(dw2), ptr(ws), ws.numel(), stride,
+                                                    code, stream(), recs, 2, ctypes.byref(n)), "conv3d_wgrad_pair_deferred")
+        if n.value != 2 or recs[0].dw != dw.data_ptr() or recs[1].dw != dw2.data_ptr():
+            raise N.Ru3dError("ru3d: conv3d_wgrad_pair_deferred did not describe (dw, dw2) in that order")
+        _note_pending(st, (wr, defer2[1]), recs, 2)
+        return dw, dw2
+    ws = N.workspace(nbytes, x.device)
     check(N.lib.ru3d_conv3d_wgrad_pair(ref(dx), ref(ddy), ref(ddy2), ptr(dw), ptr(dw2), ptr(ws), ws.numel(), stride, code,
                                        stream()), "conv3d_wgrad_pair")
     return dw, dw2
 
 
-def conv_wgrad_bias(x, dy, k, stride, key=None):
+def conv_wgrad_bias(x, dy, k, stride, key=None, bkey=None):
     cout, cin = dy.shape[1], x.shape[1]
     dw = _grad_out(key, (cout, cin, k, k, k), x.device)
     db = torch.empty(cout, dtype=torch.float32, device=x.device)
     dx, ddy = desc(x), desc(dy)
     code = N.dtype_code(x.dtype)
-    ws = N.workspace(N.lib.ru3d_conv3d_wgrad_bias_workspace_bytes(ref(dx), ref(ddy), k, stride, code), x.device)
+    nbytes = N.lib.ru3d_conv3d_wgrad_bias_workspace_bytes(ref(dx), ref(ddy), k, stride, code)
+    defer, defer2 = _may_defer(key, x.dtype, x.device), _may_defer(bkey, x.dtype, x.device)
+    if defer is not None and defer2 is not None:
+        st, wr, skey = defer
+        ws = _slab_ws(st, skey, nbytes)
+    if defer is not None and defer2 is not None and ws is not None:
+        recs, n = (N.WgradPending * 2)(), ctypes.c_int(0)
+        check(N.lib.ru3d_conv3d_wgrad_bias_deferred(ref(dx), ref(ddy), ptr(dw), ptr(db), ptr(ws), ws.numel(), k, stride, code,
+                                                    stream(), recs, 2, ctypes.byref(n)), "conv3d_wgrad_bias_deferred")
+        _note_pending(st, [wr if recs[i].dw == dw.data_ptr() else defer2[1] for i in range(n.value)], recs, n.value)
+        return dw, db
+    ws = N.workspace(nbytes, x.device)
     check(N.lib.ru3d_conv3d_wgrad_bias(ref(dx), ref(ddy), ptr(dw), ptr(db), ptr(ws), ws.numel(), k, stride, code, stream()),
           "conv3d_wgrad_bias")
     return dw, db
@@ -494,6 +665,16 @@
     dx, ddy = desc(x), desc(dy)
     code = N.dtype_code(x.dtype)
     nbytes = N.lib.ru3d_convtranspose3d_k3s2p1_wgrad_workspace_bytes(ref(dx), ref(ddy), code)
+    defer = _may_defer(key, x.dtype, x.device)
+    if defer is not None:
+        st, wr, skey = defer
+        ws = _slab_ws(st, skey, nbytes)
+    if defer is not None and ws is not None:
+        recs, n = (N.WgradPending * 2)(), ctypes.c_int(0)
+        check(N.lib.ru3d_convtranspose3d_k3s2p1_wgrad_deferred(ref(dx), ref(ddy), ptr(dw), ptr(ws), ws.numel(), code, stream(),
+                                                               recs, 2, ctypes.byref(n)), "convtranspose3d_wgrad_deferred")
+        _note_pending(st, wr, recs, n.value)
+        return dw
     ws = N.workspace(nbytes, x.device)
     check(N.lib.ru3d_convtranspose3d_k3s2p1_wgrad(ref(dx), ref(ddy), ptr(dw), ptr(ws), ws.numel(), code, stream()),
           "convtranspose3d_wgrad")
@@ -920,7 +1101,8 @@
         ctx.stride, ctx.k, ctx.has_bias = stride, k, bias is not None
         ctx.storage_dtype = storage_dtype
         ctx.in_dtype = x.dtype
-        ctx.wkey = weight.data_ptr() if not (cout_seg or cin_seg) else None
+        ctx.wkey = wkey(weight, ctx) if not (cout_seg or cin_seg) else None
+        ctx.bkey = wkey(bias, ctx) if (bias is not None and not cout_seg) else None
         ctx.weight_ref = weight if (k == 1 and cout <= 4) else None
         return y
 
@@ -943,7 +1125,7 @@
         with _OnSide(gy.device):
             if ctx.needs_input_grad[1] and ctx.has_bias and ctx.needs_input_grad[2] and not (cout_seg or cin_seg) \
                     and sd != torch.float32:
-                gw, gb = conv_wgrad_bias(xin, gy, ctx.k, ctx.stride, key=ctx.wkey)
+                gw, gb = conv_wgrad_bias(xin, gy, ctx.k, ctx.stride, key=ctx.wkey, bkey=ctx.bkey)
             elif ctx.needs_input_grad[1]:
                 gw = unpad_wgrad(conv_wgrad(xin, gy, ctx.k, ctx.stride, key=ctx.wkey), cout, cin, cout_seg, cin_seg)
             if gb is None and ctx.has_bias and ctx.needs_input_grad[2]:
@@ -1042,13 +1224,13 @@
                                   None, None, None, None, hsave)
         ctx.head = head_w is not None
         ctx.head_bias = head_b is not None
-        ctx.hkey = head_w.data_ptr() if (head_w is not None and not cout_seg) else None
+        ctx.hkey = wkey(head_w, ctx) if (head_w is not None and not cout_seg) else None
         ctx.planar = bool(planar)
         ctx.dims = (cout, cin, cout_seg, cin_seg)
         ctx.stride = stride
         plain = not (cout_seg or cin_seg)
-        ctx.wkeys = (w1.data_ptr() if plain else None, w2.data_ptr() if plain else None,
-                     ws.data_ptr() if (plain and ws is not None) else None)
+        ctx.wkeys = (wkey(w1, ctx) if plain else None, wkey(w2, ctx) if plain else None,
+                     wkey(ws, ctx) if (plain and ws is not None) else None)
         ctx.has_skip_conv = ws is not None
         ctx.in_link = in_link if (in_link is not None and ws is not None) else None
         if in_link is not None:
@@ -1203,7 +1385,7 @@
         ctx.dims = (cout, cin, cout_seg, cin_seg)
         ctx.has_skip = skip is not None
         ctx.planar = bool(skip is not None and link is not None and getattr(link, "planar_out", False))
-        ctx.wkey = wt.data_ptr() if not (cout_seg or cin_seg) else None
+        ctx.wkey = wkey(wt, ctx) if not (cout_seg or cin_seg) else None
         ctx.link = link if (link is not None and getattr(link, "fused_grad", False)) else None
         return out
 
diff --git a/3d-unet-renal-anatomy-extraction_amd/csrc/api.hip b/3d-unet-renal-anatomy-extraction_amd/csrc/api.hip
--- a/3d-unet-renal-anatomy-extraction_amd/csrc/api.hip
+++ b/3d-unet-renal-anatomy-extraction_amd/csrc/api.hip
@@ -30,6 +30,11 @@
         return (int)e > 0 ? (int)e : 1;
     }
     return 0;
+}
+
+Ru3dWgradSink*& ru3d_wgrad_sink() {
+    static thread_local Ru3dWgradSink* sink = nullptr;
+    return sink;
 }
 
 extern "C" int ru3d_version(void) { return RU3D_VERSION; }
@@ -805,4 +810,54 @@
     return wgrad_generic_launch(dy->ptr, x->ptr, dw, ws, ws_bytes, g, dtype, as_stream(stream));
 }
 
-}
+#ifndef RU3D_STORAGE_F16
+namespace {
+struct WgradSinkScope {
+    Ru3dWgradSink sink;
+    int* n_out;
+    WgradSinkScope(ru3d_wgrad_pending* items, int cap, int* n) : sink{items, items && cap > 0 ? cap : 0, 0}, n_out(n) {
+        ru3d_wgrad_sink() = &sink;
+    }
+    ~WgradSinkScope() {
+        ru3d_wgrad_sink() = nullptr;
+        if (n_out) *n_out = sink.count;
+    }
+};
+}
+
+extern "C" int ru3d_conv3d_wgrad_deferred(const ru3d_tensor* x, const ru3d_tensor* dy, float* dw, void* ws, size_t ws_bytes,
+                                          int k, int stride, int dtype, void* stream, ru3d_wgrad_pending* pending, int cap,
+                                          int* n_pending) {
+    RU3D_REQUIRE(n_pending, "conv3d_wgrad_deferred: n_pending is NULL");
+    WgradSinkScope scope(pending, cap, n_pending);
+    return ru3d_conv3d_wgrad(x, dy, dw, ws, ws_bytes, k, stride, dtype, stream);
+}
+
+extern "C" int ru3d_conv3d_wgrad_pair_deferred(const ru3d_tensor* x, const ru3d_tensor* dy, const ru3d_tensor* dy2, float* dw,
+                                               float* dw2, void* ws, size_t ws_bytes, int stride, int dtype, void* stream,
+                                               ru3d_wgrad_pending* pending, int cap, int* n_pending) {
+    RU3D_REQUIRE(n_pending, "conv3d_wgrad_pair_deferred: n_pending is NULL");
+    WgradSinkScope scope(pending, cap, n_pending);
+    return ru3d_conv3d_wgrad_pair(x, dy, dy2, dw, dw2, ws, ws_bytes, stride, dtype, stream);
+}
+
+extern "C" int ru3d_conv3d_wgrad_bias_deferred(const ru3d_tensor* x, const ru3d_tensor* dy, float* dw, float* db, void* ws,
+                                               size_t ws_bytes, int k, int stride, int dtype, void* stream,
+                                               ru3d_wgrad_pending* pending, int cap, int* n_pending) {
+    RU3D_REQUIRE(n_pending, "conv3d_wgrad_bias_deferred: n_pending is NULL");
+    const bool rides = (k == 1 || k == 3) && (stride == 1 || stride == 2) && wgrad_shapes_ok(x, dy, k, stride) &&
+                       tensor_ok(x) && stem_wgrad_gives_bias(make_wgrad(x, dy, k, stride), dtype);
+    WgradSinkScope scope(pending, rides ? cap : 0, n_pending);
+    return ru3d_conv3d_wgrad_bias(x, dy, dw, db, ws, ws_bytes, k, stride, dtype, stream);
+}
+
+extern "C" int ru3d_convtranspose3d_k3s2p1_wgrad_deferred(const ru3d_tensor* x, const ru3d_tensor* dy, float* dw, void* ws,
+                                                          size_t ws_bytes, int dtype, void* stream,
+                                                          ru3d_wgrad_pending* pending, int cap, int* n_pending) {
+    RU3D_REQUIRE(n_pending, "convtranspose3d_wgrad_deferred: n_pending is NULL");
+    WgradSinkScope scope(pending, cap, n_pending);
+    return ru3d_convtranspose3d_k3s2p1_wgrad(x, dy, dw, ws, ws_bytes, dtype, stream);
+}
+#endif
+
+}
diff --git a/3d-unet-renal-anatomy-extraction_amd/csrc/common.h b/3d-unet-renal-anatomy-extraction_amd/csrc/common.h
--- a/3d-unet-renal-anatomy-extraction_amd/csrc/common.h
+++ b/3d-unet-renal-anatomy-extraction_amd/csrc/common.h
@@ -53,6 +53,12 @@
 
 int ru3d_fail(int code, const char* fmt, ...);
 int ru3d_check_launch(const char* what);
+
+struct Ru3dWgradSink {
+    ru3d_wgrad_pending* items;
+    int cap, count;
+};
+Ru3dWgradSink*& ru3d_wgrad_sink();
 
 static inline hipStream_t as_stream(void* s) { return (hipStream_t)s; }
 
diff --git a/3d-unet-renal-anatomy-extraction_amd/csrc/conv.h b/3d-unet-renal-anatomy-extraction_amd/csrc/conv.h
--- a/3d-unet-renal-anatomy-extraction_amd/csrc/conv.h
+++ b/3d-unet-renal-anatomy-extraction_amd/csrc/conv.h
@@ -64,6 +64,7 @@
 int pack_generic_launch(const float* src, void* dst, int cin, int cout, int taps, int64_t s_o, int64_t s_i,
                         int flip, int dtype, hipStream_t st);
 size_t wgrad_generic_ws_bytes(const WgradGeom& g);
+bool wgrad_reduce_pick(int chunks, int taps, int cin, int cout, int64_t s_o, int64_t s_i, int* variant, int* blocks);
 int wgrad_reduce_launch(const float* part, float* dw, int chunks, int taps, int cin, int cout, int64_t s_o, int64_t s_i,
                         hipStream_t st);
 int wgrad_generic_launch(const void* x, const void* dy, float* dw, void* ws, size_t ws_bytes, WgradGeom g, int dtype,
diff --git a/3d-unet-renal-anatomy-extraction_amd/csrc/conv_generic.hip b/3d-unet-renal-anatomy-extraction_amd/csrc/conv_generic.hip
--- a/3d-unet-renal-anatomy-extraction_amd/csrc/conv_generic.hip
+++ b/3d-unet-renal-anatomy-extraction_amd/csrc/conv_generic.hip
@@ -1,5 +1,7 @@
 #include "common.h"
 #include "conv.h"
+#include <algorithm>
+#include <vector>
 
 namespace RU3D_NS {
 
@@ -461,14 +463,13 @@
 }
 
 template <int QX>
-__global__ __launch_bounds__(256) void wgrad_reduce_kernel(const float* __restrict__ part, float* __restrict__ dw,
-                                                           int chunks, int taps, int cin, int cout, int64_t s_o,
-                                                           int64_t s_i) {
+__device__ __forceinline__ void wgrad_reduce_body(const float* __restrict__ part, float* __restrict__ dw, int chunks, int taps,
+                                                  int cin, int cout, int64_t s_o, int64_t s_i, int bid,
+                                                  f32x4 (*sh)[QX]) {
     constexpr int KY = 256 / QX;
-    __shared__ f32x4 sh[KY][QX];
     const int64_t total = (int64_t)taps * cin * cout;
     const int ox = threadIdx.x % QX, ky = threadIdx.x / QX;
-    const int64_t i0 = ((int64_t)blockIdx.x * QX + ox) * 4;
+    const int64_t i0 = ((int64_t)bid * QX + ox) * 4;
     f32x4 s = {0.f, 0.f, 0.f, 0.f};
     const bool full = (i0 + 3 < total) && ((total & 3) == 0);
     if (full) {
@@ -503,6 +504,14 @@
             dw[co * s_o + ci * s_i + tap] = s[j];
         }
     }
+}
+
+template <int QX>
+__global__ __launch_bounds__(256) void wgrad_reduce_kernel(const float* __restrict__ part, float* __restrict__ dw,
+                                                           int chunks, int taps, int cin, int cout, int64_t s_o,
+                                                           int64_t s_i) {
+    __shared__ f32x4 sh[256 / QX][QX];
+    wgrad_reduce_body<QX>(part, dw, chunks, taps, cin, cout, s_o, s_i, blockIdx.x, sh);
 }
 
 template <bool CO_MAJOR>
@@ -581,33 +590,83 @@
     wgrad_reduce_tiled_body<CO_MAJOR>(part, dw, chunks, taps, cin, cout, s_o, s_i, blockIdx.x, tile);
 }
 
-int wgrad_reduce_launch(const float* part, float* dw, int chunks, int taps, int cin, int cout, int64_t s_o, int64_t s_i,
-                        hipStream_t st) {
+#define WGSUM_TILE_FLOATS (32 * (4 * 27 + 1))
+__global__ __launch_bounds__(256) void wgrad_reduce_multi_kernel(const ru3d_wgrad_pending* __restrict__ items, int n,
+                                                                 const int32_t* __restrict__ block_map) {
+    __shared__ __attribute__((aligned(16))) float lds[WGSUM_TILE_FLOATS];
+    const int it = block_map[2 * blockIdx.x], bid = block_map[2 * blockIdx.x + 1];
+    if (it < 0 || it >= n) return;
+    const ru3d_wgrad_pending p = items[it];
+    if (bid < 0 || bid >= p.blocks) return;
+    switch (p.variant) {
+        case RU3D_WGSUM_TILED_CO:
+            wgrad_reduce_tiled_body<true>(p.part, p.dw, p.chunks, p.taps, p.cin, p.cout, p.s_o, p.s_i, bid, lds);
+            break;
+        case RU3D_WGSUM_TILED_CI:
+            wgrad_reduce_tiled_body<false>(p.part, p.dw, p.chunks, p.taps, p.cin, p.cout, p.s_o, p.s_i, bid, lds);
+            break;
+        case RU3D_WGSUM_Q64:
+            wgrad_reduce_body<64>(p.part, p.dw, p.chunks, p.taps, p.cin, p.cout, p.s_o, p.s_i, bid,
+                                  reinterpret_cast<f32x4(*)[64]>(lds));
+            break;
+        case RU3D_WGSUM_Q8:
+            wgrad_reduce_body<8>(p.part, p.dw, p.chunks, p.taps, p.cin, p.cout, p.s_o, p.s_i, bid,
+                                 reinterpret_cast<f32x4(*)[8]>(lds));
+            break;
+        default: break;
+    }
+}
+
+bool wgrad_reduce_pick(int chunks, int taps, int cin, int cout, int64_t s_o, int64_t s_i, int* variant, int* blocks) {
     const int64_t total = (int64_t)taps * cin * cout;
     const bool tiled = (int64_t)cin * cout >= 128 * 128 && (cin % 4) == 0 && (cout % 32) == 0 && taps <= 27 &&
                        (s_i == taps || s_o == taps);
+    int64_t b;
     if (tiled) {
-        const int64_t blocks = (int64_t)(cin / 4) * (cout / 32);
-        if (blocks > 0x3fffffff) return ru3d_fail(-1, "wgrad_reduce: grid too large");
-        if (s_i == taps)
-            hipLaunchKernelGGL(wgrad_reduce_tiled_kernel<true>, dim3((unsigned)blocks), dim3(256), 0, st, part, dw, chunks, taps,
-                               cin, cout, s_o, s_i);
-        else
-            hipLaunchKernelGGL(wgrad_reduce_tiled_kernel<false>, dim3((unsigned)blocks), dim3(256), 0, st, part, dw, chunks, taps,
-                               cin, cout, s_o, s_i);
-        return ru3d_check_launch(s_i == taps ? "wgrad_reduce_tiled<true>" : "wgrad_reduce_tiled<false>");
-    }
-    const bool deep = chunks >= 128 && (total + 255) / 256 < 512;
-    const int qx = deep ? 8 : 64;
-    const int64_t blocks = (total + 4 * qx - 1) / (4 * qx);
-    if (blocks > 0x3fffffff) return ru3d_fail(-1, "wgrad_reduce: grid too large");
-    if (deep)
-        hipLaunchKernelGGL(wgrad_reduce_kernel<8>, dim3((unsigned)blocks), dim3(256), 0, st, part, dw, chunks, taps, cin, cout,
-                           s_o, s_i);
-    else
-        hipLaunchKernelGGL(wgrad_reduce_kernel<64>, dim3((unsigned)blocks), dim3(256), 0, st, part, dw, chunks, taps, cin, cout,
-                           s_o, s_i);
-    return ru3d_check_launch(deep ? "wgrad_reduce<8>" : "wgrad_reduce<64>");
+        b = (int64_t)(cin / 4) * (cout / 32);
+        *variant = s_i == taps ? RU3D_WGSUM_TILED_CO : RU3D_WGSUM_TILED_CI;
+    } else {
+        const bool deep = chunks >= 128 && (total + 255) / 256 < 512;
+        const int qx = deep ? 8 : 64;
+        b = (total + 4 * qx - 1) / (4 * qx);
+        *variant = deep ? RU3D_WGSUM_Q8 : RU3D_WGSUM_Q64;
+    }
+    if (b > 0x3fffffff) return false;
+    *blocks = (int)b;
+    return true;
+}
+
+int wgrad_reduce_launch(const float* part, float* dw, int chunks, int taps, int cin, int cout, int64_t s_o, int64_t s_i,
+                        hipStream_t st) {
+    int variant = 0, blocks = 0;
+    if (!wgrad_reduce_pick(chunks, taps, cin, cout, s_o, s_i, &variant, &blocks))
+        return ru3d_fail(-1, "wgrad_reduce: grid too large");
+    Ru3dWgradSink* sink = ru3d_wgrad_sink();
+    if (sink && sink->count < sink->cap) {
+        ru3d_wgrad_pending& p = sink->items[sink->count++];
+        p.part = part; p.dw = dw;
+        p.chunks = chunks; p.taps = taps; p.cin = cin; p.cout = cout;
+        p.s_o = s_o; p.s_i = s_i;
+        p.variant = variant; p.blocks = blocks;
+        return 0;
+    }
+    const dim3 grid((unsigned)blocks);
+    switch (variant) {
+        case RU3D_WGSUM_TILED_CO:
+            hipLaunchKernelGGL(wgrad_reduce_tiled_kernel<true>, grid, dim3(256), 0, st, part, dw, chunks, taps, cin, cout, s_o,
+                               s_i);
+            return ru3d_check_launch("wgrad_reduce_tiled<true>");
+        case RU3D_WGSUM_TILED_CI:
+            hipLaunchKernelGGL(wgrad_reduce_tiled_kernel<false>, grid, dim3(256), 0, st, part, dw, chunks, taps, cin, cout, s_o,
+                               s_i);
+            return ru3d_check_launch("wgrad_reduce_tiled<false>");
+        case RU3D_WGSUM_Q8:
+            hipLaunchKernelGGL(wgrad_reduce_kernel<8>, grid, dim3(256), 0, st, part, dw, chunks, taps, cin, cout, s_o, s_i);
+            return ru3d_check_launch("wgrad_reduce<8>");
+        default:
+            hipLaunchKernelGGL(wgrad_reduce_kernel<64>, grid, dim3(256), 0, st, part, dw, chunks, taps, cin, cout, s_o, s_i);
+            return ru3d_check_launch("wgrad_reduce<64>");
+    }
 }
 
 int wgrad_generic_chunks(const WgradGeom& g) {
@@ -648,3 +707,47 @@
 }
 
 }
+
+#ifndef RU3D_STORAGE_F16
+extern "C" int ru3d_wgrad_block_map(const ru3d_wgrad_pending* items, int n, int32_t* block_map, int cap_blocks) {
+    if (!items || n <= 0) return ru3d_fail(-1, "wgrad_block_map: no items");
+    std::vector<int> order(n);
+    std::vector<int64_t> cost(n);
+    int64_t nblocks = 0;
+    for (int i = 0; i < n; i++) {
+        const ru3d_wgrad_pending& p = items[i];
+        int variant = -1, blocks = 0;
+        if (!p.part || !p.dw || p.chunks <= 0 || p.taps <= 0 || p.cin <= 0 || p.cout <= 0 ||
+            !wgrad_reduce_pick(p.chunks, p.taps, p.cin, p.cout, p.s_o, p.s_i, &variant, &blocks) || variant != p.variant ||
+            blocks != p.blocks)
+            return ru3d_fail(-1, "wgrad_block_map: record %d is not one a `_deferred` entry point wrote", i);
+        const bool tiled = variant == RU3D_WGSUM_TILED_CO || variant == RU3D_WGSUM_TILED_CI;
+        const int64_t per = tiled ? (int64_t)p.taps * 128 : variant == RU3D_WGSUM_Q64 ? 256 : 32;
+        cost[i] = (int64_t)p.chunks * per + (tiled ? (1ll << 48) : 0);
+        order[i] = i;
+        nblocks += blocks;
+    }
+    if (nblocks > 0x3fffffff) return ru3d_fail(-1, "wgrad_block_map: grid too large");
+    if (!block_map) return (int)nblocks;
+    if (cap_blocks < nblocks) return ru3d_fail(-1, "wgrad_block_map: map holds %d workgroups, %lld needed", cap_blocks,
+                                               (long long)nblocks);
+    std::stable_sort(order.begin(), order.end(), [&](int a, int b) { return cost[a] > cost[b]; });
+    int64_t o = 0;
+    for (int k = 0; k < n; k++)
+        for (int b = 0; b < items[order[k]].blocks; b++) {
+            block_map[2 * o] = order[k];
+            block_map[2 * o + 1] = b;
+            o++;
+        }
+    return (int)nblocks;
+}
+
+extern "C" int ru3d_wgrad_reduce_multi(const ru3d_wgrad_pending* items, int n, const int32_t* block_map, int nblocks,
+                                       void* stream) {
+    Ru3dDeviceGuard dev_guard(stream);
+    RU3D_REQUIRE(items && block_map && n > 0 && nblocks > 0 && nblocks <= 0x3fffffff, "wgrad_reduce_multi: bad argument");
+    hipLaunchKernelGGL(wgrad_reduce_multi_kernel, dim3((unsigned)nblocks), dim3(256), 0, as_stream(stream), items, n,
+                       block_map);
+    return ru3d_check_launch("wgrad_reduce_multi");
+}
+#endif
diff --git a/3d-unet-renal-anatomy-extraction_amd/graph.py b/3d-unet-renal-anatomy-extraction_amd/graph.py
--- a/3d-unet-renal-anatomy-extraction_amd/graph.py
+++ b/3d-unet-renal-anatomy-extraction_amd/graph.py
@@ -62,6 +62,7 @@
             if self.scaler is not None:
                 self.scaler.begin_capture(self.optimizer, dev)
             self.optimizer.zero_grad(set_to_none=True)
+            _ops.reserve_capture_table(dev)
             g = torch.cuda.CUDAGraph()
             _ops.DROP_OFFSET_BASE[0] = self.drop_base
             _loss_mod.CAPTURE_SINK[0] = self.label_states = []
@@ -138,7 +139,10 @@
             sids = (sid,) if side is None else (sid, side.cuda_stream)
             for key in [k for k in N._WS if k[1] in sids]:
                 del N._WS[key]
+            for key in [k for k in _ops._PENDING if k[1] in sids]:
+                del _ops._PENDING[key]
             _ops._PREPACK.clear()
+            _ops._CAPTURE_TABLE.pop(self.stream.device, None)
             for name in ("x", "y", "loss", "logits", "_static_logits", "block", "drop_base", "hyper", "host", "host_ev",
                          "stream", "label_states"):
                 if hasattr(self, name):
diff --git a/include/ru3d.h b/include/ru3d.h
--- a/include/ru3d.h
+++ b/include/ru3d.h
@@ -124,6 +124,29 @@
 size_t ru3d_convtranspose3d_k3s2p1_wgrad_workspace_bytes(const ru3d_tensor* x, const ru3d_tensor* dy, int dtype);
 int ru3d_convtranspose3d_k3s2p1_wgrad(const ru3d_tensor* x, const ru3d_tensor* dy, float* dw, void* ws,
                                       size_t ws_bytes, int dtype, void* stream);
+
+enum { RU3D_WGSUM_TILED_CO = 0, RU3D_WGSUM_TILED_CI = 1, RU3D_WGSUM_Q64 = 2, RU3D_WGSUM_Q8 = 3 };
+typedef struct ru3d_wgrad_pending {
+    const float* part;
+    float* dw;
+    int32_t chunks, taps, cin, cout;
+    int64_t s_o, s_i;
+    int32_t variant;
+    int32_t blocks;
+} ru3d_wgrad_pending;
+int ru3d_conv3d_wgrad_deferred(const ru3d_tensor* x, const ru3d_tensor* dy, float* dw, void* ws, size_t ws_bytes, int k,
+                               int stride, int dtype, void* stream, ru3d_wgrad_pending* pending, int cap, int* n_pending);
+int ru3d_conv3d_wgrad_pair_deferred(const ru3d_tensor* x, const ru3d_tensor* dy, const ru3d_tensor* dy2, float* dw,
+                                    float* dw2, void* ws, size_t ws_bytes, int stride, int dtype, void* stream,
+                                    ru3d_wgrad_pending* pending, int cap, int* n_pending);
+int ru3d_conv3d_wgrad_bias_deferred(const ru3d_tensor* x, const ru3d_tensor* dy, float* dw, float* db, void* ws,
+                                    size_t ws_bytes, int k, int stride, int dtype, void* stream,
+                                    ru3d_wgrad_pending* pending, int cap, int* n_pending);
+int ru3d_convtranspose3d_k3s2p1_wgrad_deferred(const ru3d_tensor* x, const ru3d_tensor* dy, float* dw, void* ws,
+                                               size_t ws_bytes, int dtype, void* stream, ru3d_wgrad_pending* pending,
+                                               int cap, int* n_pending);
+int ru3d_wgrad_block_map(const ru3d_wgrad_pending* items, int n, int32_t* block_map, int cap_blocks);
+int ru3d_wgrad_reduce_multi(const ru3d_wgrad_pending* items, int n, const int32_t* block_map, int nblocks, void* stream);
 
 size_t ru3d_reduce_workspace_bytes(const ru3d_tensor* t);
 int ru3d_instnorm_stats(const ru3d_tensor* y, const float* drop_scale, float* mean, float* scale,
```

After: 279.5 million voxels/s, median of 6. Within noise of the previous version (+0.6%).
